# lhn0323/BEVFUSION-3D_object_detection

Hardware: AMD Instinct MI355X
Metric: nuScenes frames/sec (6-cam+LiDAR BEVFusion fwd+bwd) (higher is better)
Workload: dtype bf16; 1 GPU; full: BEVFusion camera+LiDAR (ResNet-50, LSS 6x256x704, hard voxelize 40k pts, sparse encoder, ConvFuser, SECOND/SECONDFPN, TransFusion head + Hungarian targets + focal/L1/gaussian-focal losses) fwd + bwd + clip + AdamW, bf16 autocast, fp32 index paths; global_batch=4, points_per_frame=40000, parallelism=independent frames per rank, execution=eager launches on 2 HIP queues (camera / BEV chain, LiDAR branch), view_transform_conv_dtype=bf16, head_fp32_conv=three bf16 products per multiply, fp32 accumulation (2^-16 relative per product), dense_weight_gradients=one grouped launch per tile shape at the end of the backward pass, backward_pass_thread=caller, trainable_params=37361053

## Files before the change

bevfusion-3d_object_detection_amd/_lib.py:

```python
import ctypes
import os

import torch

_HERE = os.path.dirname(os.path.abspath(__file__))
LIB_PATH = os.path.join(_HERE, "csrc", "libbevfusion_hip.so")

_c_int = ctypes.c_int
_c_vp = ctypes.c_void_p
_c_sz = ctypes.c_size_t

SIGNATURES = {
    "bfhip_abi_version": (_c_int, []),
    "bfhip_last_error": (ctypes.c_char_p, []),
    "bfhip_profile_enable": (None, [_c_int]),
    "bfhip_profile_read": (_c_int, [_c_int, _c_vp, _c_vp, _c_int]),
    "bfhip_bev_pool_fwd": (_c_int, [_c_vp] * 5 + [_c_int] * 7 + [_c_vp, _c_vp]),
    "bfhip_bev_pool_bwd": (_c_int, [_c_vp] * 5 + [_c_int] * 8 + [_c_vp, _c_vp]),
    "bfhip_dynamic_voxelize": (_c_int, [_c_vp, _c_vp, _c_int, _c_int, _c_vp, _c_vp, _c_vp]),
    "bfhip_hard_voxelize_workspace_bytes": (_c_sz, [_c_int, _c_int, _c_int]),
    "bfhip_hard_voxelize": (_c_int, [_c_vp, _c_int, _c_int, _c_vp, _c_vp, _c_vp, _c_vp, _c_vp,
                                     _c_int, _c_int, _c_vp, _c_sz, _c_vp, _c_vp]),
    "bfhip_bev_plan_workspace_bytes": (_c_sz, [ctypes.c_longlong, ctypes.c_longlong]),
    "bfhip_bev_plan": (_c_int, [_c_vp] * 7 + [_c_int] * 4 + [_c_vp] * 3 + [_c_vp] * 11 + [_c_int, _c_vp, _c_sz, _c_vp]),
    "bfhip_lift_splat_fwd": (_c_int, [_c_vp, _c_int, _c_vp, _c_int, _c_int] + [_c_vp] * 6 + [_c_int, _c_int, ctypes.c_longlong,
                                       _c_vp, _c_int, _c_vp]),
    "bfhip_lift_splat_bwd": (_c_int, [_c_vp, _c_int, _c_vp, _c_int, _c_vp, _c_int, _c_int, _c_vp] + [_c_int] * 4 +
                             [_c_vp, _c_int, _c_vp, _c_int, _c_vp]),
    "bfhip_conv_out_shape": (_c_int, [_c_vp] * 6),
    "bfhip_rulebook_subm_workspace_bytes": (_c_sz, [_c_int]),
    "bfhip_rulebook_subm": (_c_int, [_c_vp, _c_int, _c_int, _c_vp, _c_vp, _c_vp, _c_vp, _c_vp, _c_vp, _c_vp, _c_vp, _c_sz,
                                     _c_vp]),
    "bfhip_rulebook_sparse_workspace_bytes": (_c_sz, [_c_int] + [_c_vp] * 5),
    "bfhip_rulebook_sparse_count": (_c_int, [_c_vp, _c_int, _c_vp, _c_int] + [_c_vp] * 5 + [_c_vp, _c_vp, _c_sz, _c_vp]),
    "bfhip_rulebook_sparse_out_indices": (_c_int, [_c_int] + [_c_vp] * 5 + [_c_int, _c_vp, _c_vp, _c_sz, _c_vp]),
    "bfhip_rulebook_sparse_fill": (_c_int, [_c_vp, _c_int, _c_int] + [_c_vp] * 5 + [_c_int] + [_c_vp] * 4 +
                                   [_c_vp] * 4 + [_c_vp, _c_sz] + [_c_vp, _c_sz, _c_vp]),
    "bfhip_spconv_workspace_bytes": (_c_sz, [_c_int] * 3),
    "bfhip_rulebook_sort_rows_workspace_bytes": (_c_sz, [_c_int, _c_int]),
    "bfhip_rulebook_sort_rows": (_c_int, [_c_vp, _c_int, _c_int, _c_int, _c_vp, _c_vp, _c_vp, _c_sz, _c_vp]),
    "bfhip_rulebook_validate_workspace_bytes": (_c_sz, [_c_int]),
    "bfhip_rulebook_validate": (_c_int, [_c_vp, _c_int, _c_int, _c_int, _c_int, _c_vp, _c_vp, _c_vp, _c_vp, _c_sz, _c_vp]),
    "bfhip_spconv_gemm": (_c_int, [_c_vp] * 3 + [_c_int] * 7 + [_c_vp, _c_vp, _c_vp, _c_vp, _c_sz, _c_vp]),
    "bfhip_spconv_gemm_bf16": (_c_int, [_c_vp] * 3 + [_c_int] * 7 + [_c_vp, _c_vp, _c_vp, _c_int, _c_vp, _c_sz, _c_vp]),
    "bfhip_spconv_wgrad_workspace_bytes": (_c_sz, [_c_int] * 4),
    "bfhip_spconv_wgrad": (_c_int, [_c_vp] * 3 + [_c_int] * 5 + [_c_vp, _c_vp, _c_int, _c_vp, _c_sz, _c_vp]),
    "bfhip_sparse_to_bev": (_c_int, [_c_vp, _c_vp] + [_c_int] * 6 + [_c_vp, _c_vp]),
    "bfhip_bev_to_sparse": (_c_int, [_c_vp, _c_vp] + [_c_int] * 6 + [_c_vp, _c_vp]),
    "bfhip_dynamic_scatter_workspace_bytes": (_c_sz, [_c_int]),
    "bfhip_dynamic_scatter_fwd": (_c_int, [_c_vp, _c_vp, _c_int, _c_int, _c_int] + [_c_vp] * 5 + [_c_vp, _c_sz, _c_vp]),
    "bfhip_dynamic_scatter_bwd_workspace_bytes": (_c_sz, [_c_int, _c_int]),
    "bfhip_dynamic_scatter_bwd": (_c_int, [_c_vp] * 6 + [_c_int] * 4 + [_c_vp, _c_sz, _c_vp]),
    "bfhip_voxel_mean": (_c_int, [_c_vp, _c_vp, _c_int, _c_int, _c_int, _c_vp, _c_vp]),
    "bfhip_voxel_compact_mean": (_c_int, [_c_vp] * 4 + [_c_int] * 5 + [_c_vp] * 4),
    "bfhip_depth_lift_bwd_workspace_bytes": (_c_sz, []),
    "bfhip_depth_lift_bwd": (_c_int, [_c_vp, _c_vp, ctypes.c_longlong, _c_vp, _c_vp, _c_sz, _c_vp]),
    "bfhip_rasterise_depth_workspace_bytes": (_c_sz, [_c_int] * 3),
    "bfhip_rasterise_depth": (_c_int, [_c_vp, _c_int, _c_int] + [_c_vp] * 4 + [_c_int] * 3 + [_c_vp, _c_vp] + [_c_int] * 3 +
                              [_c_vp, _c_vp, _c_sz, _c_vp]),
    "bfhip_depth_histogram": (_c_int, [_c_vp] + [_c_int] * 6 + [_c_vp, _c_vp, _c_vp, _c_vp]),
    "bfhip_bn1d_workspace_bytes": (_c_sz, [_c_int, _c_int]),
    "bfhip_bn1d_fwd": (_c_int, [_c_vp] * 4 + [_c_int, _c_int, ctypes.c_float, ctypes.c_float, _c_int] + [_c_vp] * 5 +
                       [_c_vp, _c_sz, _c_vp]),
    "bfhip_bn1d_bwd": (_c_int, [_c_vp] * 5 + [_c_int] * 3 + [_c_vp] * 4 + [_c_vp, _c_sz, _c_vp]),
    "bfhip_sparse_to_bev_nhwc": (_c_int, [_c_vp, _c_vp] + [_c_int] * 7 + [_c_vp, _c_vp]),
    "bfhip_bev_nhwc_to_sparse": (_c_int, [_c_vp, ctypes.c_longlong, ctypes.c_longlong, ctypes.c_longlong, _c_int, _c_vp, _c_int,
                                          _c_int, _c_int, _c_vp, _c_vp]),
    "bfhip_bn2d_supported": (_c_int, [ctypes.c_longlong, _c_int, _c_int]),
    "bfhip_bn2d_workspace_bytes": (_c_sz, [ctypes.c_longlong, _c_int, _c_int]),
    "bfhip_colsum": (_c_int, [_c_vp, ctypes.c_longlong, _c_int, _c_int, _c_vp, _c_vp, _c_sz, _c_vp]),
    "bfhip_bn2d_fwd": (_c_int, [_c_vp] * 4 + [ctypes.c_longlong, _c_int, _c_int, ctypes.c_float, ctypes.c_float, _c_int] +
                       [_c_vp] * 5 + [_c_vp, _c_sz, _c_vp]),
    "bfhip_bn2d_bwd": (_c_int, [_c_vp] * 5 + [ctypes.c_longlong, _c_int, _c_int, _c_int] + [_c_vp] * 4 + [_c_vp, _c_sz, _c_vp]),
    "bfhip_xty_workspace_bytes": (_c_sz, [ctypes.c_longlong, _c_int, _c_int]),
    "bfhip_xty": (_c_int, [_c_vp, _c_vp, ctypes.c_longlong, _c_int, _c_int, _c_int, _c_vp, _c_vp, _c_sz, _c_vp]),
    "bfhip_attn_max_queries": (_c_int, []),
    "bfhip_attn_workspace_bytes": (_c_sz, [_c_int] * 4),
    "bfhip_attn_fwd": (_c_int, [_c_vp] * 3 + [_c_int] * 4 + [ctypes.c_float, ctypes.c_float, ctypes.c_ulonglong, _c_vp, _c_vp,
                                                             _c_vp, _c_vp, _c_sz, _c_vp]),
    "bfhip_attn_bwd": (_c_int, [_c_vp] * 6 + [_c_int] * 4 + [ctypes.c_float, ctypes.c_float, ctypes.c_ulonglong] + [_c_vp] * 4 +
                       [_c_vp, _c_sz, _c_vp]),
    "bfhip_attn_dropout_mask": (_c_int, [_c_int] * 4 + [ctypes.c_float, ctypes.c_ulonglong, _c_vp, _c_vp, _c_vp]),
    "bfhip_upsample2x_nhwc": (_c_int, [_c_vp, _c_vp] + [_c_int] * 6 + [_c_vp]),
    "bfhip_maxpool3x3s2_fwd": (_c_int, [_c_vp] + [_c_int] * 4 + [_c_vp, _c_vp, _c_vp]),
    "bfhip_maxpool3x3s2_bwd": (_c_int, [_c_vp, _c_vp] + [_c_int] * 4 + [_c_vp, _c_vp]),
    "bfhip_circle_nms": (_c_int, [_c_vp, _c_int, ctypes.c_float, _c_int, _c_vp, _c_vp, _c_vp]),
    "bfhip_rotate_nms_workspace_bytes": (_c_sz, [_c_int, _c_int]),
    "bfhip_rotate_nms": (_c_int, [_c_vp, _c_vp, _c_int, ctypes.c_float, _c_int, _c_int, _c_vp, _c_vp, _c_vp, _c_sz, _c_vp]),
    "bfhip_decode_boxes": (_c_int, [_c_vp] * 5 + [_c_int] * 4 + [_c_vp, _c_vp, _c_vp]),
    "bfhip_predict_compact": (_c_int, [_c_vp] * 3 + [_c_int] * 3 + [_c_vp, _c_int, ctypes.c_float] + [_c_vp] * 5),
    "bfhip_assign_cost": (_c_int, [_c_vp, _c_int, _c_vp, _c_int, _c_int, _c_int, _c_vp, _c_int, _c_vp, _c_vp] + [_c_int] * 3 +
                          [_c_vp] * 4),
    "bfhip_hungarian": (_c_int, [_c_vp, _c_vp, _c_int, _c_int, _c_int, _c_vp, _c_vp, _c_vp]),
    "bfhip_assign_targets": (_c_int, [_c_vp, _c_vp, _c_vp, _c_int, _c_vp] + [_c_int] * 5 + [_c_vp] * 7),
    "bfhip_draw_heatmap": (_c_int, [_c_vp, _c_int, _c_vp, _c_vp] + [_c_int] * 5 + [_c_vp, ctypes.c_double, _c_int, _c_vp, _c_vp]),
    "bfhip_gaussian_focal_loss_workspace_bytes": (_c_sz, [ctypes.c_longlong]),
    "bfhip_gaussian_focal_loss": (_c_int, [_c_vp, _c_vp, ctypes.c_longlong, ctypes.c_float, _c_vp, _c_vp, _c_vp, _c_sz, _c_vp]),
    "bfhip_conv2d_supported": (_c_int, [_c_int] * 10),
    "bfhip_conv2d_stat_rows": (_c_int, [_c_int] * 3),
    "bfhip_conv2d_fwd": (_c_int, [_c_vp, _c_int, _c_vp, _c_vp, _c_vp, _c_int] + [_c_int] * 11 + [_c_vp, _c_vp]),
    "bfhip_conv2d_dgrad_workspace_bytes": (_c_sz, [_c_int] * 4),
    "bfhip_conv2d_dgrad": (_c_int, [_c_vp, _c_int, _c_vp, _c_vp, _c_int] + [_c_int] * 11 + [_c_vp, _c_sz, _c_vp]),
    "bfhip_conv2d_dgrad_wt": (_c_int, [_c_vp, _c_int, _c_vp, _c_vp, _c_int, _c_vp, _c_int] + [_c_int] * 11 + [_c_vp]),
    "bfhip_conv2d_dgrad_fuses_addend": (_c_int, [_c_int] * 5),
    "bfhip_split_bf16x3": (_c_int, [_c_vp, ctypes.c_longlong, _c_int, _c_vp, _c_int, _c_vp, _c_int, _c_vp]),
    "bfhip_conv2d_wt_segment_bytes": (_c_int, []),
    "bfhip_conv2d_weight_transpose_batched": (_c_int, [_c_vp, _c_int, ctypes.c_longlong, _c_vp]),
    "bfhip_conv2d_launch_choice": (_c_int, [_c_int] * 12 + [_c_vp]),
    "bfhip_conv2d_wgrad_choice": (_c_int, [_c_int] * 10 + [_c_vp]),
    "bfhip_conv2d_wgrad_workspace_bytes": (_c_sz, [_c_int] * 7),
    "bfhip_conv2d_wgrad": (_c_int, [_c_vp, _c_int, _c_vp, _c_int, _c_vp] + [_c_int] * 11 + [_c_vp, _c_sz, _c_vp]),
    "bfhip_conv2d_wgrad_group_table_bytes": (_c_sz, [_c_int]),
    "bfhip_conv2d_wgrad_groupable": (_c_int, [_c_int] * 10),
    "bfhip_conv2d_wgrad_group_plan": (_c_int, [_c_vp, _c_int, _c_int, _c_vp, _c_sz, _c_vp]),
    "bfhip_conv2d_wgrad_group_launch": (_c_int, [_c_vp, _c_vp, _c_vp, _c_sz, _c_vp]),
    "bfhip_bn2d_fwd_partials": (_c_int, [_c_vp] * 4 + [ctypes.c_longlong, _c_int, _c_int, ctypes.c_float, ctypes.c_float, _c_int] +
                                [_c_vp] * 4 + [_c_vp, _c_int, _c_vp, _c_vp]),
    "bfhip_bn2d_fwd_partials_mask": (_c_int, [_c_vp] * 4 + [ctypes.c_longlong, _c_int, _c_int, ctypes.c_float, ctypes.c_float, _c_int] +
                                     [_c_vp] * 4 + [_c_vp, _c_int, _c_vp, _c_vp, _c_vp]),
    "bfhip_bn2d_bwd_mask": (_c_int, [_c_vp] * 5 + [ctypes.c_longlong, _c_int, _c_int] + [_c_vp] * 4 + [_c_vp, _c_sz, _c_vp]),
    "bfhip_adamw_segment_bytes": (_c_int, []),
    "bfhip_adamw_chunk_elems": (_c_int, []),
    "bfhip_adamw_step": (_c_int, [_c_vp, _c_vp, _c_vp, _c_int, _c_vp, _c_vp] + [ctypes.c_float] * 6 + [_c_vp]),
    "bfhip_adamw_step_groups": (_c_int, [_c_vp, _c_vp, _c_vp, _c_int, _c_vp, _c_vp, _c_vp, _c_vp, _c_int, ctypes.c_float, _c_vp]),
    "bfhip_query_losses": (_c_int, [_c_vp] * 7 + [_c_int] * 6 + [ctypes.c_float, ctypes.c_float] + [_c_vp] * 4),
    "bfhip_swin_attn_supported": (_c_int, [_c_int] * 7),
    "bfhip_swin_attn_parts": (_c_int, [_c_int] * 4),
    "bfhip_swin_attn_fwd": (_c_int, [_c_vp, ctypes.c_longlong, _c_vp] + [_c_int] * 5 + [ctypes.c_float, _c_vp, _c_vp, _c_vp]),
    "bfhip_swin_attn_bwd": (_c_int, [_c_vp, ctypes.c_longlong, _c_vp, _c_vp, _c_vp, _c_vp] + [_c_int] * 5 +
                            [ctypes.c_float, _c_vp, _c_vp, _c_int, _c_vp]),
    "bfhip_layernorm_supported": (_c_int, [ctypes.c_longlong, _c_int, _c_int, _c_int]),
    "bfhip_layernorm_parts": (_c_int, [ctypes.c_longlong, _c_int]),
    "bfhip_layernorm_fwd": (_c_int, [_c_vp, _c_vp, _c_vp, ctypes.c_longlong, _c_vp, _c_vp, ctypes.c_longlong, _c_int, ctypes.c_float] +
                            [_c_int] * 3 + [_c_vp] * 4),
    "bfhip_layernorm_bwd": (_c_int, [_c_vp] * 6 + [ctypes.c_longlong, ctypes.c_longlong] + [_c_int] * 4 + [_c_vp] * 3 + [_c_int] +
                            [_c_vp] * 3),
    "bfhip_bn_eval_supported": (_c_int, [ctypes.c_longlong, _c_int, _c_int]),
    "bfhip_bn_eval_parts": (_c_int, [ctypes.c_longlong, _c_int, _c_int]),
    "bfhip_bn_eval_fwd": (_c_int, [_c_vp] * 6 + [ctypes.c_longlong, _c_int, _c_int, ctypes.c_float, _c_int, _c_vp, _c_vp]),
    "bfhip_bn_eval_bwd": (_c_int, [_c_vp] * 6 + [ctypes.c_longlong, _c_int, _c_int, ctypes.c_float, _c_int] + [_c_vp] * 5),
    "bfhip_bn_eval_rows_fwd": (_c_int, [_c_vp] * 6 + [ctypes.c_longlong, _c_int, _c_int, ctypes.c_float, _c_int, _c_vp, _c_vp,
                                         _c_vp]),
    "bfhip_bn_eval_rows_bwd": (_c_int, [_c_vp] * 6 + [ctypes.c_longlong, _c_int, _c_int, ctypes.c_float, _c_int] + [_c_vp] * 6),
    "bfhip_img_preprocess_max_samples": (_c_int, []),
    "bfhip_img_preprocess": (_c_int, [_c_vp] + [_c_int] * 5 + [_c_vp, _c_vp, ctypes.c_float, _c_int, _c_int, _c_int, _c_int,
                                      _c_vp, _c_vp]),
    "bfhip_image_aug_max_taps": (_c_int, []),
    "bfhip_image_aug_max_cams": (_c_int, []),
    "bfhip_image_aug_supported": (_c_int, [_c_int] * 8),
    "bfhip_image_aug": (_c_int, [_c_vp, _c_int, _c_int, _c_vp, _c_vp, ctypes.c_longlong, _c_int, _c_int, _c_vp, _c_int, _c_int,
                                 _c_vp, _c_vp, ctypes.c_float] + [_c_int] * 4 + [_c_vp, _c_vp]),
    "bfhip_image_aug_masked": (_c_int, [_c_vp, _c_vp, _c_int, _c_int, _c_vp, _c_vp, ctypes.c_longlong, _c_int, _c_int, _c_vp, _c_int,
                                        _c_int, _c_vp, _c_vp, ctypes.c_float] + [_c_int] * 4 + [_c_vp, _c_vp]),
    "bfhip_points_aug_block": (_c_int, []),
    "bfhip_points_aug_workspace_bytes": (_c_sz, [ctypes.c_longlong, _c_int]),
    "bfhip_points_aug": (_c_int, [_c_vp, _c_int, _c_int, _c_vp, _c_vp, _c_vp, _c_sz, _c_vp]),
    "bfhip_points_aug_max_boxes": (_c_int, []),
    "bfhip_points_aug_paste": (_c_int, [_c_vp, _c_vp, _c_int, _c_int, _c_vp, _c_vp, _c_vp, _c_sz, _c_vp]),
    "bfhip_points_aug_max_sweeps": (_c_int, []),
    "bfhip_points_aug_sweeps": (_c_int, [_c_vp, _c_vp, _c_vp, _c_int, _c_int, _c_vp, _c_vp, _c_vp, _c_sz, _c_vp]),
    "bfhip_query_init_supported": (_c_int, [_c_int] * 8),
    "bfhip_query_init_workspace_bytes": (_c_sz, [_c_int] * 4),
    "bfhip_query_init_fwd": (_c_int, [_c_vp] + [ctypes.c_longlong] * 4 + [_c_int] * 4 + [ctypes.c_uint, _c_vp, ctypes.c_longlong,
                                      ctypes.c_longlong] + [_c_int] * 4 + [_c_vp] * 6 + [_c_sz, _c_vp]),
    "bfhip_query_init_bwd": (_c_int, [_c_vp, _c_vp, _c_int, _c_int, _c_int, ctypes.c_longlong, _c_int, _c_vp, _c_vp]),
    "bfhip_jpeg_parse": (_c_int, [_c_vp, _c_sz, _c_vp]),
    "bfhip_jpeg_entropy_decode": (_c_int, [_c_vp, _c_sz, _c_vp, _c_vp, _c_sz]),
    "bfhip_jpeg_decode": (_c_int, [_c_vp, _c_vp, _c_int, _c_vp, _c_sz, _c_vp, _c_sz, _c_vp, _c_sz, _c_vp]),
    "bfhip_jpeg_entropy_encode": (_c_int, [_c_vp, _c_vp, _c_sz, _c_int, _c_vp, _c_sz, _c_vp]),
    "bfhip_jpeg_encode_supported": (_c_int, [_c_int] * 4),
    "bfhip_jpeg_encode_workspace_bytes": (_c_sz, [_c_int] * 4),
    "bfhip_jpeg_encode_max_frames": (_c_int, []),
    "bfhip_jpeg_forward": (_c_int, [_c_vp, _c_vp, _c_int, _c_vp, _c_sz, _c_vp, _c_sz, _c_vp]),
    "bfhip_jpeg_entropy_encode_device": (_c_int, [_c_vp, _c_vp, _c_int, _c_vp, _c_sz, _c_vp, _c_sz, _c_vp, _c_sz, _c_vp, _c_vp]),
    "bfhip_jpeg_encode": (_c_int, [_c_vp, _c_vp, _c_int, _c_vp, _c_sz, _c_vp, _c_sz, _c_vp, _c_sz, _c_vp, _c_sz, _c_vp, _c_vp]),
    "bfhip_png_encode_supported": (_c_int, [_c_int] * 3),
    "bfhip_png_encode_max_frames": (_c_int, []),
    "bfhip_png_workspace_bytes": (_c_sz, [ctypes.c_int64, ctypes.c_int64, _c_int]),
    "bfhip_png_capacity": (_c_sz, [ctypes.c_int64, ctypes.c_int64]),
    "bfhip_png_result_words": (_c_sz, [ctypes.c_int64, ctypes.c_int64]),
    "bfhip_png_encode": (_c_int, [_c_vp, _c_vp, _c_int, _c_vp, _c_sz, _c_vp, _c_sz, _c_vp, _c_sz, _c_vp, _c_sz, _c_vp]),
    "bfhip_png_deflate": (_c_int, [_c_vp, _c_vp, _c_int, _c_vp, _c_sz, _c_vp, _c_sz, _c_vp, _c_sz, _c_vp, _c_sz, _c_vp]),
    "bfhip_png_filter_host": (_c_int, [_c_vp, _c_int, _c_int, _c_vp, _c_sz]),
    "bfhip_png_huffman_lengths": (_c_int, [_c_vp, _c_int, _c_int, _c_vp]),
    "bfhip_png_deflate_host": (_c_int, [_c_vp, _c_sz, _c_sz, _c_vp, _c_sz, _c_vp, _c_sz, _c_vp]),
    "bfhip_points_in_boxes_block": (_c_int, []),
    "bfhip_points_in_boxes_max_boxes": (_c_int, []),
    "bfhip_points_in_boxes_workspace_bytes": (_c_sz, [ctypes.c_longlong, _c_int]),
    "bfhip_points_in_boxes_count": (_c_int, [_c_vp, ctypes.c_longlong, _c_int, _c_vp, _c_int, _c_vp, _c_vp, _c_vp, _c_sz, _c_vp]),
    "bfhip_points_in_boxes_gather": (_c_int, [_c_vp, ctypes.c_longlong, _c_int, _c_vp, _c_int, _c_vp, _c_vp, ctypes.c_longlong,
                                              _c_vp, ctypes.c_longlong, _c_vp, _c_sz, _c_vp]),
    "bfhip_detection_eval_max_preds": (_c_int, []),
    "bfhip_detection_eval_max_gt": (_c_int, []),
    "bfhip_detection_eval_max_thresholds": (_c_int, []),
    "bfhip_detection_eval_max_classes": (_c_int, []),
    "bfhip_detection_match": (_c_int, [_c_vp] * 4 + [ctypes.c_longlong] + [_c_vp] * 3 + [ctypes.c_longlong, _c_int, _c_int, _c_vp,
                                       _c_int, _c_int, ctypes.c_uint64, ctypes.c_uint64, _c_vp, _c_vp, _c_vp]),
    "bfhip_detection_curves_workspace_bytes": (_c_sz, [ctypes.c_longlong, _c_int]),
    "bfhip_detection_curves": (_c_int, [_c_vp] * 5 + [ctypes.c_longlong, _c_int, _c_int, _c_int, _c_vp, _c_vp, ctypes.c_double,
                                        _c_int, ctypes.c_uint64] + [_c_vp] * 6 + [_c_vp, _c_sz, _c_vp]),
    "bfhip_vis_max_dim": (_c_int, []),
    "bfhip_vis_max_thickness": (_c_int, []),
    "bfhip_vis_max_scale": (_c_int, []),
    "bfhip_vis_workspace_bytes": (_c_sz, [_c_int, _c_int, _c_int]),
    "bfhip_vis_camera_segments": (_c_int, [_c_vp, _c_int, _c_vp, _c_vp, _c_int, ctypes.c_float, _c_int, _c_int, _c_int, _c_vp, _c_sz,
                                           _c_vp]),
    "bfhip_vis_bev_segments": (_c_int, [_c_vp, _c_int, ctypes.c_float, ctypes.c_float, ctypes.c_float, _c_int, _c_int, _c_int, _c_vp,
                                        _c_sz, _c_vp]),
    "bfhip_vis_composite": (_c_int, [_c_vp, _c_int, _c_int, _c_int, _c_vp, _c_sz, _c_int, _c_int, _c_vp, _c_vp, _c_int, _c_int, _c_int,
                                     _c_vp, _c_vp]),
    "bfhip_vis_bev_points": (_c_int, [_c_vp, ctypes.c_longlong, _c_int, ctypes.c_float, ctypes.c_float, ctypes.c_float, _c_int, _c_vp,
                                      _c_int, _c_int, _c_vp]),
}


class ImgDesc(ctypes.Structure):
    _fields_ = [("data", _c_vp), ("h", _c_int), ("w", _c_int)]

_lib = None


def load():
    global _lib
    if _lib is None:
        if not os.path.exists(LIB_PATH):
            raise RuntimeError(
                "libbevfusion_hip.so not found at %s: build it with "
                "`python -c 'import __graft_entry__ as g; g.build()'` (hipcc, gfx950). "
                "There is no CPU fallback." % LIB_PATH)
        lib = ctypes.CDLL(LIB_PATH)
        for name, (res, args) in SIGNATURES.items():
            fn = getattr(lib, name)
            fn.restype = res
            fn.argtypes = args
        _lib = lib
    return _lib


_torch_ext = False


def torch_ext():
    global _torch_ext
    if _torch_ext is False:
        _torch_ext = None
        path = os.path.join(_HERE, "csrc", "bfhip_torch_ext.so")
        if os.environ.get("BFHIP_TORCH_EXT", "1") == "1" and os.path.exists(path):
            import importlib.util
            load()
            try:
                spec = importlib.util.spec_from_file_location("bfhip_torch_ext", path)
                mod = importlib.util.module_from_spec(spec)
                spec.loader.exec_module(mod)
                if mod.abi_version() == load().bfhip_abi_version():
                    _torch_ext = mod
            except (ImportError, OSError) as e:
                import warnings
                warnings.warn("bfhip_torch_ext not usable (%s); using the ctypes binding" % e)
    return _torch_ext


def check(rc, what):
    if rc != 0:
        msg = load().bfhip_last_error().decode("utf-8", "replace")
        raise RuntimeError("%s failed (rc=%d): %s" % (what, rc, msg))


_fn_cache = {}


def call(name, *args):
    fn = _fn_cache.get(name)
    if fn is None:
        fn = _fn_cache[name] = getattr(load(), name)
    rc = fn(*args)
    if rc != 0:
        check(rc, name)


def call_size(name, *args):
    return int(getattr(load(), name)(*args))


def ptr(t):
    return None if t is None else t.data_ptr()


_raw_stream = getattr(torch._C, "_cuda_getCurrentRawStream", None)


def stream_of(t):
    if _raw_stream is not None:
        return _raw_stream(t.device.index if t.device.index is not None else torch.cuda.current_device())
    return ctypes.c_void_p(torch.cuda.current_stream(t.device).cuda_stream)


def host_i32(values):
    return (ctypes.c_int32 * len(values))(*[int(v) for v in values])


def host_f32(values):
    arr = (ctypes.c_float * len(values))(*[float(v) for v in values])
    return arr


def require_cuda(t, name):
    if not t.is_cuda:
        raise RuntimeError("%s must be a CUDA(HIP) tensor; this build has no CPU path" % name)
    if not t.is_contiguous():
        raise RuntimeError("%s must be contiguous" % name)


OPS = dict(bev_pool_fwd=0, bev_pool_bwd=1, hard_voxelize=2, dynamic_voxelize=3, lift_splat_fwd=4, lift_splat_bwd=5,
           spconv_fwd=6, spconv_bwd=7, rulebook=8, bev_aux=9, scatter_fwd=10, scatter_bwd=11, spconv_wgrad=12, raster=13,
           spconv_wgrad_main=14, conv2d_fwd=15, conv2d_dgrad=16, conv2d_wgrad=17, bn2d_fwd=18, bn2d_bwd=19,
           conv2d_pw_fwd=20, conv2d_pw_dgrad=21)


def profile_enable(on=True):
    load().bfhip_profile_enable(int(on))


def profile_read(op, reset=True):
    s = ctypes.c_double(0.0)
    c = ctypes.c_longlong(0)
    check(load().bfhip_profile_read(OPS[op] if isinstance(op, str) else op, ctypes.byref(s), ctypes.byref(c),
                                    1 if reset else 0), "profile_read")
    return s.value, c.value
```

bevfusion-3d_object_detection_amd/conv2d.py:

```python
import os

import torch
import torch.nn.functional as F
from torch import nn

from . import _lib

ENABLED = os.environ.get("BFHIP_CONV2D", "1") == "1"
CONV_EXT = os.environ.get("BFHIP_CONV_EXT", "1") == "1"


def _conv_ext():
    if not CONV_EXT or WGRAD_SIDE_STREAM:
        return None
    ext = _lib.torch_ext()
    if ext is None or not hasattr(ext, "conv2d"):
        return None
    ext.set_wgrad_grouped(bool(WGRAD_GROUPED))
    return ext


def _cached_wt(weight):
    cached = getattr(weight, "_bfhip_wt", None)
    if cached is not None and cached[1] == weight._version and cached[2] == weight.data_ptr():
        return cached[0]
    return None
MIN_PIXELS = int(os.environ.get("BFHIP_CONV2D_MIN_PIXELS", "2048"))
MIN_CIN = int(os.environ.get("BFHIP_CONV2D_MIN_CIN", "16"))
FORK = os.environ.get("BFHIP_CONV_FORK", "1") == "1"
_WS = {}

WGRAD_SIDE_STREAM = os.environ.get("BFHIP_WGRAD_SIDE_STREAM", "0") == "1"
_SIDE = {}
_KEEP = []


def _wgrad_stream(device):
    s = _SIDE.get(device)
    if s is None:
        s = _SIDE[device] = torch.cuda.Stream(device=device)
    return s


def wgrad_join():
    for dev, side in _SIDE.items():
        torch.cuda.current_stream(dev).wait_stream(side)
    _KEEP.clear()


WGRAD_GROUPED = os.environ.get("BFHIP_WGRAD_GROUPED", "1") == "1"
_PENDING = {}
_GROUPABLE = {}
_GROUP_STATE = {}
_LAYER_DT = None


class _WgradGroupState:

    def __init__(self, device):
        self.device = device
        self.host = [None, None]
        self.dev = None
        self.slab = None
        self.flip = 0

    def tables(self, nbytes):
        if self.dev is None or self.dev.numel() < nbytes:
            cap = max(int(nbytes) * 2, 1 << 16)
            self.host = [torch.empty(cap, dtype=torch.uint8).pin_memory() for _ in range(2)]
            self.dev = torch.empty(cap, dtype=torch.uint8, device=self.device)
        self.flip ^= 1
        return self.host[self.flip], self.dev

    def slabs(self, nbytes):
        if self.slab is None or self.slab.numel() < nbytes:
            self.slab = None
            self.slab = torch.empty(int(nbytes * 1.25) + 256, dtype=torch.uint8, device=self.device)
        return self.slab


def _layer_dtype():
    global _LAYER_DT
    if _LAYER_DT is None:
        import numpy as np
        _LAYER_DT = np.dtype([("x", "<u8"), ("dy", "<u8"), ("dw", "<u8")] + [(k, "<i4") for k in (
            "ldx", "ldg", "N", "H", "W", "Cin", "Cout", "KH", "KW", "stride", "pad", "dil", "dw_bf16", "reserved")])
        assert _LAYER_DT.itemsize == 80
    return _LAYER_DT


def _defer_wgrad(x, dy, weight, stride, pad, dil):
    N, Cin, H, W = x.shape
    Cout, _, KH, KW = weight.shape
    key = (N, H, W, Cin, Cout, KH, KW, stride, pad, dil)
    ok = _GROUPABLE.get(key)
    if ok is None:
        ok = _GROUPABLE[key] = bool(_lib.load().bfhip_conv2d_wgrad_groupable(*key))
    if (not ok or not weight.is_leaf or weight._backward_hooks or weight.dtype not in (torch.bfloat16, torch.float32)
            or torch.cuda.is_current_stream_capturing()):
        return False
    ldx, ldg = _nhwc_view(x), _nhwc_view(dy)
    if ldx is None or ldg is None:
        return False
    ext = _conv_ext()
    if ext is not None:
        return bool(ext.defer_wgrad(x, dy, weight, stride, pad, dil))
    tid = torch._C._current_graph_task_id()
    pend = _PENDING.get(tid)
    if pend is None:
        if tid < 0:
            return False
        try:
            torch.autograd.Variable._execution_engine.queue_callback(lambda: _flush_wgrads(tid))
        except RuntimeError:
            return False
        for old in [k for k in _PENDING if k < tid - 8]:
            del _PENDING[old]
        pend = _PENDING[tid] = []
    row = (x.data_ptr(), dy.data_ptr(), 0, ldx, ldg, N, H, W, Cin, Cout, KH, KW, stride, pad, dil,
           1 if weight.dtype == torch.bfloat16 else 0, 0)
    pend.append((x, dy, weight, row, _lib.stream_of(x)))
    return True


def _flush_wgrads(tid):
    import ctypes

    import numpy as np
    pend = _PENDING.pop(tid, None)
    if not pend:
        return
    by_dev = {}
    for e in pend:
        by_dev.setdefault(e[0].device, []).append(e)
    lib = _lib.load()
    with torch.no_grad():
        for dev, entries in by_dev.items():
            st = _GROUP_STATE.get(dev)
            if st is None:
                st = _GROUP_STATE[dev] = _WgradGroupState(dev)
            cur = torch.cuda.current_stream(dev)
            raw = cur.cuda_stream
            n = len(entries)
            dws = []
            for x, dy, weight, row, s in entries:
                if s != raw:
                    x.record_stream(cur)
                    dy.record_stream(cur)
                Cout, Cin, KH, KW = weight.shape
                dws.append(torch.empty((Cout, KH, KW, Cin), dtype=weight.dtype, device=dev).permute(0, 3, 1, 2))
            layers = np.array([e[3] for e in entries], dtype=_layer_dtype())
            layers["dw"] = [d.data_ptr() for d in dws]
            nbytes = int(lib.bfhip_conv2d_wgrad_group_table_bytes(n))
            host, table = st.tables(nbytes)
            slab_bytes = ctypes.c_size_t(0)
            _lib.call("bfhip_conv2d_wgrad_group_plan", layers.ctypes.data, n, 0, host.data_ptr(), nbytes, ctypes.byref(slab_bytes))
            slab = st.slabs(slab_bytes.value)
            with torch.cuda.device(dev):
                table[:nbytes].copy_(host[:nbytes], non_blocking=True)
                _lib.call("bfhip_conv2d_wgrad_group_launch", host.data_ptr(), table.data_ptr(), slab.data_ptr(), slab.numel(), raw)
            for (x, dy, weight, row, s), dw in zip(entries, dws):
                if weight.grad is None:
                    weight.grad = dw
                else:
                    weight.grad.add_(dw)


def _launch_wgrad(x, dy, weight, stride, pad, dil):
    N, Cin, H, W = x.shape
    Cout, _, KH, KW = weight.shape
    OH, OW = dy.shape[2], dy.shape[3]
    if WGRAD_GROUPED and not WGRAD_SIDE_STREAM and _defer_wgrad(x, dy, weight, stride, pad, dil):
        return None, None
    lib = _lib.load()
    out_bf16 = weight.dtype == torch.bfloat16
    side = None
    if WGRAD_SIDE_STREAM and getattr(weight, "grad", None) is None:
        main = torch.cuda.current_stream(x.device)
        side = _wgrad_stream(x.device)
        side.wait_stream(main)
        _KEEP.append((x, dy))
    with torch.cuda.stream(side) if side is not None else _NullCtx():
        stream = _lib.stream_of(x)
        dw = torch.empty((Cout, KH, KW, Cin), dtype=weight.dtype if out_bf16 else torch.float32, device=x.device).permute(0, 3, 1, 2)
        ws = _workspace(x.device, lib.bfhip_conv2d_wgrad_workspace_bytes(N, OH, OW, Cin, Cout, KH, KW), stream)
        _lib.call("bfhip_conv2d_wgrad", x.data_ptr(), _nhwc_view(x), dy.data_ptr(), _nhwc_view(dy), dw.data_ptr(), N, H, W, Cin,
                  Cout, KH, KW, stride, pad, dil, 1 if out_bf16 else 0, ws.data_ptr(), ws.numel(), stream)
        if dw.dtype != weight.dtype:
            dw = dw.to(weight.dtype)
    return dw, side


class _NullCtx:
    def __enter__(self):
        return None

    def __exit__(self, *a):
        return False


def _workspace(device, nbytes, stream):
    key = (device, stream)
    buf = _WS.get(key)
    if buf is None or buf.numel() < nbytes:
        buf = _WS[key] = torch.empty(max(int(nbytes), 1 << 24), dtype=torch.uint8, device=device)
    return buf


def _nhwc_view(t):
    N, C, H, W = t.shape
    sn, sc, sh, sw = t.stride()
    if sc == 1 and sw >= C and sh == W * sw and (sn == H * W * sw or N == 1) and sw % 8 == 0 and t.data_ptr() % 16 == 0:
        return sw
    return None


def _as_nhwc_bf16(t):
    if t.dtype != torch.bfloat16:
        t = t.to(torch.bfloat16)
    if _nhwc_view(t) is None:
        t = t.contiguous(memory_format=torch.channels_last)
        if _nhwc_view(t) is None:
            t = t.permute(0, 2, 3, 1).contiguous().permute(0, 3, 1, 2)
    return t


def _weight_ohwi(w):
    if w.dtype != torch.bfloat16:
        w = w.to(torch.bfloat16)
    p = w.permute(0, 2, 3, 1)
    return p if p.is_contiguous() else p.contiguous()


class _Conv2dFunction(torch.autograd.Function):
    @staticmethod
    def forward(ctx, x, weight, bias, stride, pad, dil, emit_stats, dgrad_lib=False, fork=False):
        ctx.set_materialize_grads(False)
        x = _as_nhwc_bf16(x)
        N, Cin, H, W = x.shape
        Cout, _, KH, KW = weight.shape
        OH = (H + 2 * pad - dil * (KH - 1) - 1) // stride + 1
        OW = (W + 2 * pad - dil * (KW - 1) - 1) // stride + 1
        w = _weight_ohwi(weight)
        y = torch.empty((N, OH, OW, Cout), dtype=torch.bfloat16, device=x.device).permute(0, 3, 1, 2)
        partial = None
        if emit_stats:
            rows = _lib.load().bfhip_conv2d_stat_rows(N, OH, OW)
            partial = torch.empty((rows, 2, Cout), dtype=torch.float32, device=x.device)
        b32 = None
        if bias is not None:
            b32 = bias if bias.dtype == torch.float32 else bias.float()
        _lib.call("bfhip_conv2d_fwd", x.data_ptr(), _nhwc_view(x), w.data_ptr(), _lib.ptr(b32), y.data_ptr(), Cout, N, H, W, Cin,
                  Cout, KH, KW, stride, pad, dil, 0, _lib.ptr(partial), _lib.stream_of(x))
        ctx.save_for_backward(x, weight)
        ctx.geom = (stride, pad, dil)
        ctx.dgrad_lib = dgrad_lib
        ctx.bias_dtype = bias.dtype if bias is not None else None
        if partial is not None:
            ctx.mark_non_differentiable(partial)
        ctx.fork = int(fork)
        if fork == 2:
            return y, partial, x[:, :, ::2, ::2].contiguous(memory_format=torch.channels_last)
        if fork:
            return y, partial, x.view_as(x)
        return y, partial

    @staticmethod
    def backward(ctx, dy, _dpartial, d_alias=None):
        x, weight = ctx.saved_tensors
        if dy is None:
            if d_alias is not None and ctx.fork == 2:
                full = torch.zeros_like(x)
                full[:, :, ::2, ::2] = d_alias
                d_alias = full
            return d_alias, None, None, None, None, None, None, None, None
        stride, pad, dil = ctx.geom
        N, Cin, H, W = x.shape
        Cout, _, KH, KW = weight.shape
        dy = _as_nhwc_bf16(dy)
        OH, OW = dy.shape[2], dy.shape[3]
        stream = _lib.stream_of(x)
        lib = _lib.load()
        dx = dw = db = None
        if ctx.needs_input_grad[0]:
            if ctx.dgrad_lib:
                dx = _add_grad(_lib_dgrad(dy, x, weight, stride, pad, dil), d_alias, ctx.fork)
            else:
                dx = _hip_dgrad(dy, x, weight, stride, pad, dil, d_alias, 2 if ctx.fork == 2 else 1)
        side = None
        if ctx.needs_input_grad[1]:
            dw, side = _launch_wgrad(x, dy, weight, stride, pad, dil)
        if ctx.bias_dtype is not None and ctx.needs_input_grad[2]:
            if side is not None:
                with torch.cuda.stream(side):
                    db = _bias_grad(dy).to(ctx.bias_dtype)
            else:
                db = _bias_grad(dy).to(ctx.bias_dtype)
        return dx, dw, db, None, None, None, None, None, None


def _add_grad(dx, addend, fork):
    if addend is None:
        return dx
    if fork == 2:
        dx[:, :, ::2, ::2] += addend
        return dx
    return dx + addend


def _bias_grad(dy):
    N, C, H, W = dy.shape
    if _nhwc_view(dy) == C:
        from .bn2d import colsum
        return colsum(dy.permute(0, 2, 3, 1).reshape(N * H * W, C))
    return dy.sum(dim=(0, 2, 3), dtype=torch.float32)


def _hip_dgrad(dy, x, weight, stride, pad, dil, addend=None, addend_stride=1):
    N, Cin, H, W = x.shape
    Cout, _, KH, KW = weight.shape
    stream = _lib.stream_of(x)
    dx = torch.empty((N, H, W, Cin), dtype=torch.bfloat16, device=x.device).permute(0, 3, 1, 2)
    cached = getattr(weight, "_bfhip_wt", None)
    if cached is not None and cached[1] == weight._version and cached[2] == weight.data_ptr():
        want = (N, Cin, (H + 1) // 2, (W + 1) // 2) if addend_stride == 2 else (N, Cin, H, W)
        fuse = (addend is not None and addend.dtype == torch.bfloat16 and tuple(addend.shape) == want
                and addend.is_contiguous(memory_format=torch.channels_last) and addend.data_ptr() % 16 == 0
                and _lib.load().bfhip_conv2d_dgrad_fuses_addend(KH, KW, stride, pad, 0))
        _lib.call("bfhip_conv2d_dgrad_wt", dy.data_ptr(), _nhwc_view(dy), cached[0].data_ptr(), _lib.ptr(addend) if fuse else None,
                  addend_stride, dx.data_ptr(), Cin, N, H, W, Cin, Cout, KH, KW, stride, pad, dil, 0, stream)
        return dx if fuse else _add_grad(dx, addend, addend_stride)
    ws = _workspace(x.device, _lib.load().bfhip_conv2d_dgrad_workspace_bytes(Cin, Cout, KH, KW), stream)
    _lib.call("bfhip_conv2d_dgrad", dy.data_ptr(), _nhwc_view(dy), _weight_ohwi(weight).data_ptr(), dx.data_ptr(), Cin, N, H,
              W, Cin, Cout, KH, KW, stride, pad, dil, 0, ws.data_ptr(), ws.numel(), stream)
    return _add_grad(dx, addend, addend_stride)


def _lib_dgrad(dy, x, weight, stride, pad, dil):
    w = weight if weight.dtype == torch.bfloat16 else weight.to(torch.bfloat16)
    return torch.ops.aten.convolution_backward(dy, x, w, None, [stride] * 2, [pad] * 2, [dil] * 2, False, [0, 0], 1,
                                               [True, False, False])[0]


class _FixedOrderBiasGrad(torch.autograd.Function):

    @staticmethod
    def forward(ctx, y, bias):
        ctx.bias_dtype = bias.dtype
        ctx.mark_dirty(y)
        return y

    @staticmethod
    def backward(ctx, dy):
        db = dy.sum(dim=(0, 2, 3), dtype=torch.float32).to(ctx.bias_dtype) if ctx.needs_input_grad[1] else None
        return dy, db


class _LibConvHipWgradFunction(torch.autograd.Function):

    @staticmethod
    def forward(ctx, x, weight, stride, pad, dil, dgrad_hip=False):
        x = _as_nhwc_bf16(x)
        w = weight if weight.dtype == torch.bfloat16 else weight.to(torch.bfloat16)
        with torch.autocast("cuda", enabled=False):
            y = F.conv2d(x, w, None, stride, pad, dil)
        ctx.save_for_backward(x, weight)
        ctx.geom = (stride, pad, dil)
        ctx.dgrad_hip = dgrad_hip
        return y

    @staticmethod
    def backward(ctx, dy):
        x, weight = ctx.saved_tensors
        stride, pad, dil = ctx.geom
        N, Cin, H, W = x.shape
        Cout, _, KH, KW = weight.shape
        dy = _as_nhwc_bf16(dy)
        OH, OW = dy.shape[2], dy.shape[3]
        dx = dw = None
        if ctx.needs_input_grad[0]:
            dx = _hip_dgrad(dy, x, weight, stride, pad, dil) if ctx.dgrad_hip else _lib_dgrad(dy, x, weight, stride, pad, dil)
        if ctx.needs_input_grad[1]:
            dw, _ = _launch_wgrad(x, dy, weight, stride, pad, dil)
        return dx, dw, None, None, None, None


FP32_SPLIT = os.environ.get("BFHIP_FP32_CONV", "split") == "split"
_SPLIT_SCOPE = [0]


class fp32_island:

    def __init__(self, mixed):
        self.mixed = bool(mixed)

    def __enter__(self):
        _SPLIT_SCOPE[0] += self.mixed
        return self

    def __exit__(self, *a):
        _SPLIT_SCOPE[0] -= self.mixed
        return False


def _split3(t_nhwc, P, C, chan_order=None, batch_order=None):
    chan = torch.empty((P, 3 * C), dtype=torch.bfloat16, device=t_nhwc.device) if chan_order is not None else None
    batch = torch.empty((3, P, C), dtype=torch.bfloat16, device=t_nhwc.device) if batch_order is not None else None
    _lib.call("bfhip_split_bf16x3", t_nhwc.data_ptr(), P, C, _lib.ptr(chan), chan_order or 0, _lib.ptr(batch), batch_order or 0,
              _lib.stream_of(t_nhwc))
    return chan, batch


_HHL, _HLH = 0b100, 0b010


class _Conv2dSplitFunction(torch.autograd.Function):

    @staticmethod
    def forward(ctx, x, weight, bias, stride, pad, dil, emit_stats):
        ctx.set_materialize_grads(False)
        N, Cin, H, W = x.shape
        Cout, _, KH, KW = weight.shape
        OH = (H + 2 * pad - dil * (KH - 1) - 1) // stride + 1
        OW = (W + 2 * pad - dil * (KW - 1) - 1) // stride + 1
        xn = x.permute(0, 2, 3, 1)
        if not xn.is_contiguous():
            xn = xn.contiguous()
        need_w = ctx.needs_input_grad[1]
        x_chan, x_batch = _split3(xn, N * H * W, Cin, _HHL, _HLH if need_w else None)
        wn = weight.detach().permute(0, 2, 3, 1).contiguous().view(Cout * KH * KW, Cin)
        w_chan, _ = _split3(wn, Cout * KH * KW, Cin, _HLH)
        y = torch.empty((N, OH, OW, Cout), dtype=torch.float32, device=x.device).permute(0, 3, 1, 2)
        partial = None
        if emit_stats:
            partial = torch.empty((_lib.load().bfhip_conv2d_stat_rows(N, OH, OW), 2, Cout), dtype=torch.float32, device=x.device)
        b32 = None if bias is None else (bias if bias.dtype == torch.float32 else bias.float())
        _lib.call("bfhip_conv2d_fwd", x_chan.data_ptr(), 3 * Cin, w_chan.data_ptr(), _lib.ptr(b32), y.data_ptr(), Cout, N, H, W, 3 * Cin,
                  Cout, KH, KW, stride, pad, dil, 1, _lib.ptr(partial), _lib.stream_of(x))
        ctx.save_for_backward(x_batch, weight)
        ctx.geom = (stride, pad, dil, N, Cin, H, W)
        ctx.has_bias = bias is not None
        if partial is not None:
            ctx.mark_non_differentiable(partial)
        return y, partial

    @staticmethod
    def backward(ctx, dy, _dpartial):
        x_batch, weight = ctx.saved_tensors
        if dy is None:
            return None, None, None, None, None, None, None
        stride, pad, dil, N, Cin, H, W = ctx.geom
        Cout, _, KH, KW = weight.shape
        OH, OW = dy.shape[2], dy.shape[3]
        lib = _lib.load()
        gn = dy.float().permute(0, 2, 3, 1)
        if not gn.is_contiguous():
            gn = gn.contiguous()
        stream = _lib.stream_of(gn)
        need_x, need_w = ctx.needs_input_grad[0], ctx.needs_input_grad[1]
        g_chan, g_batch = _split3(gn, N * OH * OW, Cout, _HHL if need_x else None, 0b100 if need_w else None)
        dx = dw = db = None
        if need_x:
            wn = weight.detach().permute(0, 2, 3, 1).contiguous().view(Cout * KH * KW, Cin)
            _, w_stack = _split3(wn, Cout * KH * KW, Cin, None, _HLH)
            dx = torch.empty((N, H, W, Cin), dtype=torch.float32, device=gn.device).permute(0, 3, 1, 2)
            ws = _workspace(gn.device, lib.bfhip_conv2d_dgrad_workspace_bytes(Cin, 3 * Cout, KH, KW), stream)
            _lib.call("bfhip_conv2d_dgrad", g_chan.data_ptr(), 3 * Cout, w_stack.data_ptr(), dx.data_ptr(), Cin, N, H, W, Cin, 3 * Cout,
                      KH, KW, stride, pad, dil, 1, ws.data_ptr(), ws.numel(), stream)
        if need_w:
            dw = torch.empty((Cout, KH, KW, Cin), dtype=torch.float32, device=gn.device).permute(0, 3, 1, 2)
            ws = _workspace(gn.device, lib.bfhip_conv2d_wgrad_workspace_bytes(3 * N, OH, OW, Cin, Cout, KH, KW), stream)
            _lib.call("bfhip_conv2d_wgrad", x_batch.data_ptr(), Cin, g_batch.data_ptr(), Cout, dw.data_ptr(), 3 * N, H, W, Cin, Cout, KH,
                      KW, stride, pad, dil, 0, ws.data_ptr(), ws.numel(), stream)
            if dw.dtype != weight.dtype:
                dw = dw.to(weight.dtype)
        if ctx.has_bias and ctx.needs_input_grad[2]:
            db = gn.sum(dim=(0, 1, 2))
        return dx, dw, db, None, None, None, None


class TransposedWeights:

    def __init__(self, modules):
        import numpy as np
        self.items = []
        recs = []
        blk = 0
        seg_bytes = _lib.load().bfhip_conv2d_wt_segment_bytes()
        assert seg_bytes == 40, seg_bytes
        for m in modules:
            if not isinstance(m, Conv2d) or m.groups != 1 or not m.weight.is_cuda:
                continue
            if isinstance(m, Conv2dHipWgrad) and m.dgrad != "hip" and not m.cache_wt:
                continue
            w = m.weight
            if w.dtype not in (torch.bfloat16, torch.float32) or not w.permute(0, 2, 3, 1).is_contiguous():
                continue
            Cout, Cin, KH, KW = w.shape
            wt = torch.empty(Cin * KH * KW * Cout, dtype=torch.bfloat16, device=w.device)
            self.items.append((w, wt))
            recs.append((w.data_ptr(), wt.data_ptr(), Cout, KH * KW, Cin, 1 if w.dtype == torch.float32 else 0, blk))
            blk += -(-Cin // 32) * -(-Cout // 32) * KH * KW
        self.blocks = blk
        self.table = None
        if recs:
            dt = np.dtype([("src", "<u8"), ("dst", "<u8"), ("Cout", "<i4"), ("taps", "<i4"), ("Cin", "<i4"), ("f32", "<i4"), ("blk0", "<i8")])
            arr = np.array(recs, dtype=dt)
            self.table = torch.from_numpy(arr.view(np.uint8).copy()).to(self.items[0][0].device)
            self._ptrs = [r[0] for r in recs]
        self.refresh()

    def refresh(self):
        if self.table is None:
            return
        if any(w.data_ptr() != p for (w, _), p in zip(self.items, self._ptrs)):
            for w, _ in self.items:
                w._bfhip_wt = None
            self.table = None
            return
        _lib.call("bfhip_conv2d_weight_transpose_batched", self.table.data_ptr(), len(self.items), self.blocks,
                  _lib.stream_of(self.table))
        for w, wt in self.items:
            w._bfhip_wt = (wt, w._version, w.data_ptr())


def _one(v):
    if isinstance(v, (tuple, list)):
        return v[0] if all(a == v[0] for a in v) else None
    return v


def conv2d(x, weight, bias=None, stride=1, padding=0, dilation=1, emit_stats=False, dgrad_lib=False, fork=False):
    ext = _conv_ext() if x.is_cuda and x.dim() == 4 and not weight._backward_hooks else None
    if ext is not None:
        out = ext.conv2d(x, weight, bias, int(stride), int(padding), int(dilation), bool(emit_stats), bool(dgrad_lib), int(fork),
                         None if dgrad_lib else _cached_wt(weight))
        partial = out[1] if emit_stats else None
        return (out[0], partial, out[2]) if fork else (out[0], partial)
    return _Conv2dFunction.apply(x, weight, bias, int(stride), int(padding), int(dilation), bool(emit_stats), bool(dgrad_lib),
                                 int(fork))


def lib_conv2d(x, weight, stride, padding, dilation, dgrad_hip=False):
    ext = _conv_ext() if x.is_cuda and x.dim() == 4 and not weight._backward_hooks else None
    if ext is not None:
        return ext.lib_conv2d(x, weight, int(stride), int(padding), int(dilation), bool(dgrad_hip),
                              _cached_wt(weight) if dgrad_hip else None)
    return _LibConvHipWgradFunction.apply(x, weight, stride, padding, dilation, dgrad_hip)


class Conv2d(nn.Conv2d):

    def _hip_domain(self, x):
        if not (ENABLED and x.is_cuda and x.dim() == 4 and self.groups == 1 and self.padding_mode == "zeros"
                and not isinstance(self.padding, str)):
            return False
        low = x.dtype == torch.bfloat16 or (torch.is_autocast_enabled("cuda") and torch.get_autocast_dtype("cuda") == torch.bfloat16
                                            and x.dtype in (torch.float32, torch.bfloat16))
        if not low or self.weight.dtype not in (torch.bfloat16, torch.float32):
            return False
        s, p, d = _one(self.stride), _one(self.padding), _one(self.dilation)
        if s is None or p is None or d is None:
            return False
        N, Cin, H, W = x.shape
        return N * H * W >= MIN_PIXELS and Cin >= MIN_CIN

    def hip_eligible(self, x):
        if not self._hip_domain(x):
            return False
        s, p, d = _one(self.stride), _one(self.padding), _one(self.dilation)
        N, Cin, H, W = x.shape
        return bool(_lib.load().bfhip_conv2d_supported(N, H, W, Cin, self.out_channels, self.kernel_size[0], self.kernel_size[1],
                                                       s, p, d))

    def split_eligible(self, x):
        if not (FP32_SPLIT and _SPLIT_SCOPE[0] > 0 and ENABLED and x.is_cuda and x.dim() == 4 and x.dtype == torch.float32 and self.weight.dtype == torch.float32
                and not torch.is_autocast_enabled("cuda") and self.groups == 1 and self.padding_mode == "zeros"
                and not isinstance(self.padding, str)):
            return False
        s, p, d = _one(self.stride), _one(self.padding), _one(self.dilation)
        if s is None or p is None or d is None:
            return False
        N, Cin, H, W = x.shape
        Cout, KH, KW = self.out_channels, self.kernel_size[0], self.kernel_size[1]
        if N * H * W < MIN_PIXELS or Cin % 8 or Cout % 8 or x.numel() * 3 >= (1 << 31):
            return False
        sup = _lib.load().bfhip_conv2d_supported
        return bool(sup(N, H, W, 3 * Cin, Cout, KH, KW, s, p, d) and sup(N, H, W, Cin, 3 * Cout, KH, KW, s, p, d)
                    and sup(3 * N, H, W, Cin, Cout, KH, KW, s, p, d))

    def forward(self, x):
        if not self.hip_eligible(x):
            if self.split_eligible(x):
                emit = self.training and self.bias is None and torch.is_grad_enabled()
                y, partial = _Conv2dSplitFunction.apply(x, self.weight, self.bias, _one(self.stride), _one(self.padding),
                                                        _one(self.dilation), emit)
                if partial is not None:
                    y._bfhip_stat_partial = (partial, y.data_ptr(), y._version)
                return y
            if self.bias is not None and self.bias.requires_grad and torch.is_grad_enabled() and self._hip_domain(x):
                return _FixedOrderBiasGrad.apply(self._conv_forward(x, self.weight, self.bias.detach()), self.bias)
            return super().forward(x)
        emit = self.training and self.bias is None and torch.is_grad_enabled()
        y, partial = conv2d(x, self.weight, self.bias, _one(self.stride), _one(self.padding), _one(self.dilation), emit)
        if partial is not None:
            y._bfhip_stat_partial = (partial, y.data_ptr(), y._version)
        return y


class Conv2dHipWgrad(Conv2d):

    fwd = "lib"
    dgrad = "lib"
    cache_wt = False

    def forward(self, x):
        if self.bias is not None or not self.training or not self.hip_eligible(x):
            return nn.Conv2d.forward(self, x)
        s, p, d = _one(self.stride), _one(self.padding), _one(self.dilation)
        if self.fwd == "hip":
            y, partial = conv2d(x, self.weight, None, s, p, d, torch.is_grad_enabled(), self.dgrad != "hip")
            if partial is not None:
                y._bfhip_stat_partial = (partial, y.data_ptr(), y._version)
            return y
        return lib_conv2d(x, self.weight, s, p, d, self.dgrad == "hip")

    def forward_fork(self, x, subsample=1):
        if (FORK and self.fwd == "hip" and self.dgrad == "hip" and self.bias is None and self.training and torch.is_grad_enabled()
                and x.requires_grad and x.dtype == torch.bfloat16 and x.dim() == 4 and _nhwc_view(x) is not None
                and self.hip_eligible(x)):
            s, p, d = _one(self.stride), _one(self.padding), _one(self.dilation)
            y, partial, alias = conv2d(x, self.weight, None, s, p, d, True, False, 2 if subsample == 2 else 1)
            y._bfhip_stat_partial = (partial, y.data_ptr(), y._version)
            return y, alias
        return self(x), (x if subsample == 1 else None)

    def forward_unstrided(self, x_sub):
        assert self.kernel_size == (1, 1) and _one(self.padding) == 0 and self.bias is None
        y, partial = conv2d(x_sub, self.weight, None, 1, 0, 1, torch.is_grad_enabled())
        if partial is not None:
            y._bfhip_stat_partial = (partial, y.data_ptr(), y._version)
        return y
```

bevfusion-3d_object_detection_amd/csrc/conv2d.hip:

```cpp
#include "conv_common.h"

namespace bfhip {
namespace {

template <bool TR>
__device__ __forceinline__ const bf16_t *piece_src(const bf16_t *x, const ConvGeom &g, bool row_ok, int nb, int hb, int wb,
                                                   unsigned info, const bf16_t *zsrc) {
  const int dh = info >> 24, dw = (info >> 16) & 0xff, ci = info & 0xffff;
  int ih, iw;
  bool ok = row_ok;
  if (!TR) {
    ih = hb + dh;
    iw = wb + dw;
  } else {
    const int th = hb - dh, tw = wb - dw;
    ok = ok && ((th | tw) >= 0) && (((th | tw) & g.smask) == 0);
    ih = th >> g.sshift;
    iw = tw >> g.sshift;
  }
  ok = ok && (unsigned)ih < (unsigned)g.H && (unsigned)iw < (unsigned)g.W;
  const unsigned off = (unsigned)(nb + ih * g.W + iw) * (unsigned)g.ldx + (unsigned)ci;
  return ok ? x + off : zsrc;
}

struct RowIdentity {
  __device__ __forceinline__ long long operator()(long long m) const { return m; }
};
struct RowParityClass {
  int Hc, Wc, H, W, h0, w0, stride;
  __device__ __forceinline__ long long operator()(long long m) const {
    const unsigned mu = (unsigned)m, hw = (unsigned)(Hc * Wc);
    const unsigned n = mu / hw, rem = mu - n * hw;
    const unsigned i = rem / (unsigned)Wc, j = rem - i * (unsigned)Wc;
    return (long long)((n * (unsigned)H + h0 + i * stride) * (unsigned)W + w0 + j * stride);
  }
};

struct Addend {
  const bf16_t *p;
  int sub, ld, H, W;
};

template <int WGM, int WGN, int MI, int NI, bool OUT_F32, typename RowMap = RowIdentity>
__device__ __forceinline__ void igemm_epilogue(f32x16 (&acc)[MI][NI], unsigned char *smem, int tm, long long m0, int n0,
                                               long long M, int Kout, int ldy, const float *__restrict__ bias,
                                               void *__restrict__ y, float *__restrict__ stat_partial,
                                               RowMap row_map = RowMap(), Addend add = Addend{nullptr, 0, 0, 0, 0}) {
  constexpr int NTHREADS = WGM * WGN * 64;
  constexpr int BN = WGN * NI * 32, BM = WGM * MI * 32;
  constexpr int PR = BM / 128;
  constexpr int G = WGM / PR;
  static_assert(BM % 128 == 0 && G * PR == WGM, "tile rows must be whole 128-row statistic groups");
  const int tid = threadIdx.x, lane = tid & 63, w = tid >> 6;
  const int wm = w / WGN, wn = w % WGN;
  const int l31 = lane & 31, lh = lane >> 5;
  __syncthreads();

  if (stat_partial) {
    float *sred = (float *)(smem);
#pragma unroll
    for (int ni = 0; ni < NI; ++ni) {
      float s = 0.f, s2 = 0.f;
#pragma unroll
      for (int mi = 0; mi < MI; ++mi)
#pragma unroll
        for (int r = 0; r < 16; ++r) { float v = acc[mi][ni][r]; s += v; s2 += v * v; }
      s += __shfl_xor(s, 32);
      s2 += __shfl_xor(s2, 32);
      if (lh == 0) {
        int col = wn * (NI * 32) + ni * 32 + l31;
        sred[(wm * BN + col) * 2 + 0] = s;
        sred[(wm * BN + col) * 2 + 1] = s2;
      }
    }
    __syncthreads();
    const int total_rows = (int)((M + 127) / 128);
    for (int e = tid; e < PR * BN; e += NTHREADS) {
      const int pr = e / BN, col = e - pr * BN;
      const int prow = tm * PR + pr;
      if (n0 + col < Kout && prow < total_rows) {
        float t0 = 0.f, t1 = 0.f;
#pragma unroll
        for (int gi = 0; gi < G; ++gi) {
          const float *q = sred + ((pr * G + gi) * BN + col) * 2;
          t0 += q[0];
          t1 += q[1];
        }
        stat_partial[((size_t)prow * 2 + 0) * Kout + n0 + col] = t0;
        stat_partial[((size_t)prow * 2 + 1) * Kout + n0 + col] = t1;
      }
    }
    __syncthreads();
  }

  constexpr int ESZ = OUT_F32 ? 4 : 2;
  constexpr int ROWB = BN * ESZ;
#pragma unroll
  for (int ni = 0; ni < NI; ++ni) {
    const int col = wn * (NI * 32) + ni * 32 + l31;
    const float bv = (bias && n0 + col < Kout) ? bias[n0 + col] : 0.f;
#pragma unroll
    for (int mi = 0; mi < MI; ++mi)
#pragma unroll
      for (int r = 0; r < 16; ++r) {
        const int row = wm * (MI * 32) + mi * 32 + (r & 3) + 8 * (r >> 2) + 4 * lh;
        const float v = acc[mi][ni][r] + bv;
        if (OUT_F32) *(float *)(smem + row * ROWB + col * 4) = v;
        else *(bf16_t *)(smem + row * ROWB + col * 2) = (bf16_t)bf16_rne(v);
      }
  }
  __syncthreads();
  constexpr int CPR = ROWB / 16;
  constexpr int EPC = 16 / ESZ;
  for (int idx = tid; idx < BM * CPR; idx += NTHREADS) {
    const int row = idx / CPR, c = idx - row * CPR;
    const long long m = m0 + row;
    const int col = n0 + c * EPC;
    if (m >= M || col >= Kout) continue;
    unsigned char *dst = (unsigned char *)y + ((size_t)row_map(m) * ldy + col) * ESZ;
    const unsigned char *src = smem + row * ROWB + c * 16;
    const bf16_t *rs = nullptr;
    if (!OUT_F32 && add.p) {
      if (add.sub == 2) {
        const unsigned mu = (unsigned)row_map(m), hw = (unsigned)(add.H * add.W);
        const unsigned n = mu / hw, rem = mu - n * hw;
        const unsigned h = rem / (unsigned)add.W, w = rem - h * (unsigned)add.W;
        if (((h | w) & 1u) == 0)
          rs = add.p + ((size_t)((n * (unsigned)((add.H + 1) >> 1) + (h >> 1)) * (unsigned)((add.W + 1) >> 1) + (w >> 1)) * add.ld + col);
      } else {
        rs = add.p + ((size_t)row_map(m) * add.ld + col);
      }
    }
    if (rs) {
      bf16_t *d16 = (bf16_t *)dst;
      const bf16_t *s16 = (const bf16_t *)src;
      if (col + EPC <= Kout && ((((uintptr_t)dst) | ((uintptr_t)rs)) & 15) == 0) {
        const uint4 a4 = *(const uint4 *)src, b4 = *(const uint4 *)rs;
        const unsigned a[4] = {a4.x, a4.y, a4.z, a4.w}, b[4] = {b4.x, b4.y, b4.z, b4.w};
        unsigned o[4];
#pragma unroll
        for (int q = 0; q < 4; ++q) {
          const float lo = __uint_as_float(a[q] << 16) + __uint_as_float(b[q] << 16);
          const float hi = __uint_as_float(a[q] & 0xffff0000u) + __uint_as_float(b[q] & 0xffff0000u);
          o[q] = bf16_rne(lo) | (bf16_rne(hi) << 16);
        }
        *(uint4 *)dst = make_uint4(o[0], o[1], o[2], o[3]);
        continue;
      }
      for (int e = 0; e < EPC && col + e < Kout; e += 2) {
        if (col + e + 1 < Kout && ((((uintptr_t)(d16 + e)) | ((uintptr_t)(rs + e))) & 3) == 0) {
          const unsigned a = *(const unsigned *)(s16 + e), b = *(const unsigned *)(rs + e);
          const float lo = __uint_as_float(a << 16) + __uint_as_float(b << 16);
          const float hi = __uint_as_float(a & 0xffff0000u) + __uint_as_float(b & 0xffff0000u);
          *(unsigned *)(d16 + e) = bf16_rne(lo) | (bf16_rne(hi) << 16);
        } else {
          for (int q = e; q < e + 2 && col + q < Kout; ++q)
            d16[q] = (bf16_t)bf16_rne(__uint_as_float((unsigned)s16[q] << 16) + __uint_as_float((unsigned)rs[q] << 16));
        }
      }
      continue;
    }
    if (col + EPC <= Kout && (((uintptr_t)dst) & 15) == 0) *(uint4 *)dst = *(const uint4 *)src;
    else
      for (int e = 0; e < EPC && col + e < Kout; ++e) {
        if (OUT_F32) ((float *)dst)[e] = ((const float *)src)[e];
        else ((bf16_t *)dst)[e] = ((const bf16_t *)src)[e];
      }
  }
}

template <int WGM, int WGN, int MI, int NI, int STAGES, bool OUT_F32, int MODE>
__global__ __launch_bounds__(WGM * WGN * 64, (STAGES == 1 ? 4 : (WGM * WGN > 4 ? 1 : 2))) void conv_igemm_kernel(
    const bf16_t *__restrict__ x, const bf16_t *__restrict__ wt, const float *__restrict__ bias, void *__restrict__ y,
    float *__restrict__ stat_partial, ConvGeom g, int tiles_m, int tiles_n) {
  constexpr bool TR = MODE != 0;
  constexpr int NWAVES = WGM * WGN, NTHREADS = NWAVES * 64;
  constexpr int BN = WGN * NI * 32, BM = WGM * MI * 32, BK = 64;
  constexpr int A_BYTES = BM * BK * 2, B_BYTES = BN * BK * 2, S_BYTES = A_BYTES + B_BYTES;
  constexpr int NA = (BM / 8) / NWAVES;
  constexpr int NB = (BN / 8) / NWAVES;
  constexpr int GL = NA + NB;
  static_assert(NA >= 1 && NA * 8 * NWAVES == BM && NB >= 1 && NB * 8 * NWAVES == BN, "tiles must split into whole DMA instructions");
  extern __shared__ __attribute__((aligned(1024))) unsigned char smem[];
  unsigned *taps = (unsigned *)(smem + STAGES * S_BYTES);
  const int tid = threadIdx.x, lane = tid & 63, w = tid >> 6;
  const long long lb = xcd_chunked_block(blockIdx.x, (long long)tiles_m * tiles_n);
  const int tn = (int)(lb % tiles_n);
  int tm = (int)(lb / tiles_n);
  long long M = g.M;
  int nq = g.nq;
  ConvGeom::ParityClass pc = {};
  if (MODE == 2) {
    int c = 0;
    while (c + 1 < g.ncls && tm >= g.cls[c + 1].tile0) ++c;
    pc = g.cls[c];
    tm -= pc.tile0;
    M = (long long)g.N * pc.Hc * pc.Wc;
    nq = pc.nkh * pc.nkw * (g.C >> 3);
  }
  const long long m0 = (long long)tm * BM;
  const int n0 = tn * BN;

  if (MODE == 2 && nq == 0) {
    constexpr int ESZ = OUT_F32 ? 4 : 2, EPC = 16 / ESZ, CPR = BN / EPC;
    const RowParityClass rm{pc.Hc, pc.Wc, g.OH, g.OW, pc.h0, pc.w0, g.stride};
    for (int idx = tid; idx < BM * CPR; idx += NTHREADS) {
      const int row = idx / CPR, c = idx - row * CPR;
      const long long m = m0 + row;
      const int col = n0 + c * EPC;
      if (m >= M || col >= g.Kout) continue;
      unsigned char *dst = (unsigned char *)y + ((size_t)rm(m) * g.ldy + col) * ESZ;
      if (col + EPC <= g.Kout && (((uintptr_t)dst) & 15) == 0) *(uint4 *)dst = make_uint4(0u, 0u, 0u, 0u);
      else
        for (int e = 0; e < EPC && col + e < g.Kout; ++e) {
          if (OUT_F32) ((float *)dst)[e] = 0.f;
          else ((bf16_t *)dst)[e] = 0;
        }
    }
    return;
  }

  for (int q = tid; q < nq; q += NTHREADS) {
    int k = q * 8;
    int tap = k / g.C, ci = k - tap * g.C;
    int kh, kw;
    if (MODE == 2) {
      const int a = tap / pc.nkw;
      kh = pc.kh0 + a * g.stride;
      kw = pc.kw0 + (tap - a * pc.nkw) * g.stride;
    } else {
      kh = tap / g.KW;
      kw = tap - kh * g.KW;
    }
    taps[q] = ((unsigned)(kh * g.dil) << 24) | ((unsigned)(kw * g.dil) << 16) | (unsigned)ci;
  }

  const int lrow = lane >> 3, lpos = lane & 7;
  int nb[NA], hb[NA], wb[NA];
  bool rok[NA];
#pragma unroll
  for (int i = 0; i < NA; ++i) {
    long long m = m0 + w * (NA * 8) + i * 8 + lrow;
    rok[i] = m < M;
    long long mm = rok[i] ? m : 0;
    int n, oh, ow;
    const unsigned mu = (unsigned)mm;
    if (MODE == 2) {
      const unsigned hw = (unsigned)(pc.Hc * pc.Wc);
      const unsigned nn = mu / hw, rem = mu - nn * hw;
      const unsigned ci_ = rem / (unsigned)pc.Wc;
      n = (int)nn;
      oh = pc.h0 + (int)ci_ * g.stride;
      ow = pc.w0 + (int)(rem - ci_ * (unsigned)pc.Wc) * g.stride;
    } else {
      const unsigned hw = (unsigned)(g.OH * g.OW);
      const unsigned nn = mu / hw, rem = mu - nn * hw;
      n = (int)nn;
      oh = (int)(rem / (unsigned)g.OW);
      ow = (int)(rem - (unsigned)oh * (unsigned)g.OW);
    }
    nb[i] = n * g.H * g.W;
    hb[i] = TR ? oh + g.pad : oh * g.stride - g.pad;
    wb[i] = TR ? ow + g.pad : ow * g.stride - g.pad;
  }
  const bf16_t *wrow[NB];
#pragma unroll
  for (int i = 0; i < NB; ++i) {
    int co = n0 + w * (NB * 8) + i * 8 + lrow;
    wrow[i] = co < g.Kout ? wt + (size_t)co * g.ldw : nullptr;
  }
  __syncthreads();

  const int nt = (nq + 7) >> 3;
  const bf16_t *zsrc = zero_src();
  auto stage = [&](int t, int buf) {
    unsigned char *dA = smem + buf * S_BYTES + (w * (NA * 8)) * 128;
    unsigned char *dB = smem + buf * S_BYTES + A_BYTES + (w * (NB * 8)) * 128;
#pragma unroll
    for (int i = 0; i < NA; ++i) {
      const int swz = ((w * (NA * 8) + i * 8 + lrow) >> 1) & 7;
      const int q = t * 8 + (lpos ^ swz);
      const bf16_t *src = q < nq ? piece_src<TR>(x, g, rok[i], nb[i], hb[i], wb[i], taps[q], zsrc) : zsrc;
      glds16(src, dA + i * 1024);
    }
#pragma unroll
    for (int i = 0; i < NB; ++i) {
      const int swz = ((w * (NB * 8) + i * 8 + lrow) >> 1) & 7;
      const int q = t * 8 + (lpos ^ swz);
      const bf16_t *src = zsrc;
      if (wrow[i] && q < nq) {
        if (MODE == 2) {
          const unsigned info = taps[q];
          src = wrow[i] + ((size_t)((info >> 24) * g.KW + ((info >> 16) & 0xff)) * g.C + (info & 0xffff));
        } else {
          src = wrow[i] + (size_t)q * 8;
        }
      }
      glds16(src, dB + i * 1024);
    }
  };

  f32x16 acc[MI][NI];
#pragma unroll
  for (int mi = 0; mi < MI; ++mi)
#pragma unroll
    for (int ni = 0; ni < NI; ++ni)
#pragma unroll
      for (int r = 0; r < 16; ++r) acc[mi][ni][r] = 0.f;

  const int wm = w / WGN, wn = w % WGN;
  const int l31 = lane & 31, lh = lane >> 5, rswz = (lane >> 1) & 7;
  const int aoff = (wm * (MI * 32) + l31) * 128, boff = A_BYTES + (wn * (NI * 32) + l31) * 128;

#pragma unroll
  for (int s0 = 0; s0 < STAGES - 1; ++s0)
    if (s0 < nt) stage(s0, s0);
  int buf = 0, nbuf = STAGES - 1;
  for (int t = 0; t < nt; ++t) {
    if (STAGES == 1) {
      if (t) __syncthreads();
      stage(t, 0);
    }
    if (STAGES <= 2 || nt - 1 - t == 0) wait_vmcnt<0>();
    else if (STAGES == 3 || nt - 1 - t == 1) wait_vmcnt<GL>();
    else wait_vmcnt<2 * GL>();
    __builtin_amdgcn_s_barrier();
    const unsigned char *pA = smem + buf * S_BYTES + aoff, *pB = smem + buf * S_BYTES + boff;
    if (STAGES > 1 && t + STAGES - 1 < nt) stage(t + STAGES - 1, nbuf);
#pragma unroll
    for (int ks = 0; ks < 4; ++ks) {
      const int pos = ((2 * ks + lh) ^ rswz) << 4;
      bf16x8 a[MI], b[NI];
#pragma unroll
      for (int mi = 0; mi < MI; ++mi) a[mi] = *(const bf16x8 *)(pA + mi * 32 * 128 + pos);
#pragma unroll
      for (int ni = 0; ni < NI; ++ni) b[ni] = *(const bf16x8 *)(pB + ni * 32 * 128 + pos);
#pragma unroll
      for (int mi = 0; mi < MI; ++mi)
#pragma unroll
        for (int ni = 0; ni < NI; ++ni) acc[mi][ni] = __builtin_amdgcn_mfma_f32_32x32x16_bf16(a[mi], b[ni], acc[mi][ni], 0, 0, 0);
    }
    buf = buf + 1 == STAGES ? 0 : buf + 1;
    nbuf = nbuf + 1 == STAGES ? 0 : nbuf + 1;
  }
  if (MODE == 2)
    igemm_epilogue<WGM, WGN, MI, NI, OUT_F32, RowParityClass>(acc, smem, tm, m0, n0, M, g.Kout, g.ldy, bias, y, stat_partial,
                                                              RowParityClass{pc.Hc, pc.Wc, g.OH, g.OW, pc.h0, pc.w0, g.stride});
  else
    igemm_epilogue<WGM, WGN, MI, NI, OUT_F32>(acc, smem, tm, m0, n0, M, g.Kout, g.ldy, bias, y, stat_partial);
}

template <int NI, bool OUT_F32, int DIR>
__global__ __launch_bounds__(256, 4) void conv_pw_kernel(const bf16_t *__restrict__ x, const bf16_t *__restrict__ wt,
                                                         const float *__restrict__ bias, void *__restrict__ y,
                                                         float *__restrict__ stat_partial, long long M, int C, int ldx, int Kout,
                                                         int ldw, int ldy, int tiles_m, int tiles_n, Addend add) {
  constexpr int WGN = 2, MI = 2;
  constexpr int BM = 128, BN = NI * 64;
  constexpr int A_BYTES = BM * 128;
  constexpr int NA = 4, NB = BN / 32;
  extern __shared__ __attribute__((aligned(1024))) unsigned char smem[];
  const int tid = threadIdx.x, lane = tid & 63, w = tid >> 6;
  const long long lb = xcd_chunked_block(blockIdx.x, (long long)tiles_m * tiles_n);
  const int tn = (int)(lb % tiles_n), tm = (int)(lb / tiles_n);
  const long long m0 = (long long)tm * BM;
  const int n0 = tn * BN;
  const int nq = C >> 3, nt = (nq + 7) >> 3;
  const int lrow = lane >> 3, lpos = lane & 7;
  const bf16_t *zsrc = zero_src();
  const bf16_t *arow[NA], *brow[NB];
#pragma unroll
  for (int i = 0; i < NA; ++i) {
    const long long m = m0 + w * 32 + i * 8 + lrow;
    arow[i] = m < M ? x + (unsigned)m * (unsigned)ldx : nullptr;
  }
#pragma unroll
  for (int i = 0; i < NB; ++i) {
    const int co = n0 + w * (NB * 8) + i * 8 + lrow;
    brow[i] = co < Kout ? wt + (size_t)co * ldw : nullptr;
  }
  f32x16 acc[MI][NI];
#pragma unroll
  for (int mi = 0; mi < MI; ++mi)
#pragma unroll
    for (int ni = 0; ni < NI; ++ni)
#pragma unroll
      for (int r = 0; r < 16; ++r) acc[mi][ni][r] = 0.f;
  const int wm = w / WGN, wn = w % WGN;
  const int l31 = lane & 31, lh = lane >> 5, rswz = (lane >> 1) & 7;
  const unsigned char *pA = smem + (wm * 64 + l31) * 128, *pB = smem + A_BYTES + (wn * (NI * 32) + l31) * 128;
  unsigned char *dA = smem + (w * 32) * 128, *dB = smem + A_BYTES + (w * (NB * 8)) * 128;
  for (int t = 0; t < nt; ++t) {
    if (t) __syncthreads();
#pragma unroll
    for (int i = 0; i < NA; ++i) {
      const int q = t * 8 + (lpos ^ (((w * 32 + i * 8 + lrow) >> 1) & 7));
      glds16(arow[i] && q < nq ? arow[i] + q * 8 : zsrc, dA + i * 1024);
    }
#pragma unroll
    for (int i = 0; i < NB; ++i) {
      const int q = t * 8 + (lpos ^ (((w * (NB * 8) + i * 8 + lrow) >> 1) & 7));
      glds16(brow[i] && q < nq ? brow[i] + q * 8 : zsrc, dB + i * 1024);
    }
    wait_vmcnt<0>();
    __builtin_amdgcn_s_barrier();
#pragma unroll
    for (int ks = 0; ks < 4; ++ks) {
      const int pos = ((2 * ks + lh) ^ rswz) << 4;
      bf16x8 a[MI], b[NI];
#pragma unroll
      for (int mi = 0; mi < MI; ++mi) a[mi] = *(const bf16x8 *)(pA + mi * 32 * 128 + pos);
#pragma unroll
      for (int ni = 0; ni < NI; ++ni) b[ni] = *(const bf16x8 *)(pB + ni * 32 * 128 + pos);
#pragma unroll
      for (int mi = 0; mi < MI; ++mi)
#pragma unroll
        for (int ni = 0; ni < NI; ++ni) acc[mi][ni] = __builtin_amdgcn_mfma_f32_32x32x16_bf16(a[mi], b[ni], acc[mi][ni], 0, 0, 0);
    }
  }
  igemm_epilogue<2, WGN, MI, NI, OUT_F32>(acc, smem, tm, m0, n0, M, Kout, ldy, bias, y, stat_partial, RowIdentity(), add);
}

__global__ __launch_bounds__(256) void conv_weight_transpose_kernel(const bf16_t *__restrict__ w, bf16_t *__restrict__ wt,
                                                                    int Cout, int taps, int Cin) {
  __shared__ bf16_t tile[32][33];
  const int tap = blockIdx.z, c0 = blockIdx.x * 32, o0 = blockIdx.y * 32;
  const int tx = threadIdx.x & 31, ty = threadIdx.x >> 5;
  for (int r = ty; r < 32; r += 8) {
    int co = o0 + r, ci = c0 + tx;
    tile[r][tx] = (co < Cout && ci < Cin) ? w[((size_t)co * taps + tap) * Cin + ci] : (bf16_t)0;
  }
  __syncthreads();
  for (int r = ty; r < 32; r += 8) {
    int ci = c0 + r, co = o0 + tx;
    if (ci < Cin && co < Cout) wt[((size_t)ci * taps + tap) * Cout + co] = tile[tx][r];
  }
}

struct WtSeg {
  const void *src;
  bf16_t *dst;
  int Cout, taps, Cin, src_f32;
  long long blk0;
};
__global__ __launch_bounds__(256) void conv_weight_transpose_batched_kernel(const WtSeg *__restrict__ segs, int nseg) {
  __shared__ bf16_t tile[32][33];
  const long long b = blockIdx.x;
  int lo = 0, hi = nseg - 1;
  while (lo < hi) {
    const int mid = (lo + hi + 1) >> 1;
    if (segs[mid].blk0 <= b) lo = mid; else hi = mid - 1;
  }
  const WtSeg sg = segs[lo];
  const int nx = (sg.Cin + 31) >> 5, ny = (sg.Cout + 31) >> 5;
  int local = (int)(b - sg.blk0);
  const int bx = local % nx; local /= nx;
  const int by = local % ny;
  const int tap = local / ny;
  if (tap >= sg.taps) return;
  const int c0 = bx * 32, o0 = by * 32;
  const int tx = threadIdx.x & 31, ty = threadIdx.x >> 5;
  for (int r = ty; r < 32; r += 8) {
    const int co = o0 + r, ci = c0 + tx;
    bf16_t v = 0;
    if (co < sg.Cout && ci < sg.Cin) {
      const size_t i = ((size_t)co * sg.taps + tap) * sg.Cin + ci;
      v = sg.src_f32 ? (bf16_t)bf16_rne(((const float *)sg.src)[i]) : ((const bf16_t *)sg.src)[i];
    }
    tile[r][tx] = v;
  }
  __syncthreads();
  for (int r = ty; r < 32; r += 8) {
    const int ci = c0 + r, co = o0 + tx;
    if (ci < sg.Cin && co < sg.Cout) sg.dst[((size_t)ci * sg.taps + tap) * sg.Cout + co] = tile[tx][r];
  }
}

__global__ __launch_bounds__(256) void split_bf16x3_kernel(const float *__restrict__ src, long long P, int C, bf16_t *__restrict__ chan,
                                                           int order_chan, bf16_t *__restrict__ batch, int order_batch) {
  const int cv = C >> 3;
  const long long t = (long long)blockIdx.x * blockDim.x + threadIdx.x;
  if (t >= P * cv) return;
  const long long p = t / cv;
  const int c = (int)(t - p * cv) << 3;
  const float4 a = *(const float4 *)(src + p * C + c), b = *(const float4 *)(src + p * C + c + 4);
  const float v[8] = {a.x, a.y, a.z, a.w, b.x, b.y, b.z, b.w};
  unsigned hi[8], lo[8];
#pragma unroll
  for (int j = 0; j < 8; ++j) {
    hi[j] = bf16_rne(v[j]);
    lo[j] = bf16_rne(v[j] - __uint_as_float(hi[j] << 16));
  }
  const uint4 H4 = make_uint4(hi[0] | (hi[1] << 16), hi[2] | (hi[3] << 16), hi[4] | (hi[5] << 16), hi[6] | (hi[7] << 16));
  const uint4 L4 = make_uint4(lo[0] | (lo[1] << 16), lo[2] | (lo[3] << 16), lo[4] | (lo[5] << 16), lo[6] | (lo[7] << 16));
#pragma unroll
  for (int k = 0; k < 3; ++k) {
    if (chan) *(uint4 *)(chan + p * (3LL * C) + (long long)k * C + c) = ((order_chan >> k) & 1) ? L4 : H4;
    if (batch) *(uint4 *)(batch + ((long long)k * P + p) * C + c) = ((order_batch >> k) & 1) ? L4 : H4;
  }
}

bool takes_pointwise(const ConvGeom &g) {
  static const int max_c = env_int("BFHIP_CONV_PW_MAXC", 4096);
  return g.KH == 1 && g.KW == 1 && g.stride == 1 && g.pad == 0 && g.transposed != 2 && g.C <= max_c;
}

struct IgemmChoice {
  bool pointwise;
  int shape, stages, BM, BN, tiles_m, tiles_n;
  size_t lds;
  int tile0[17];
};

IgemmChoice choose_igemm(const ConvGeom &g, int out_f32, int cus) {
  IgemmChoice c = {};
  if (takes_pointwise(g)) {
    c.pointwise = true;
    c.stages = 1; c.BM = 128; c.BN = g.Kout > 64 ? 128 : 64;
    c.tiles_m = ceil_div(g.M, 128);
    c.tiles_n = ceil_div(g.Kout, c.BN);
    const size_t stage = (size_t)(128 + c.BN) * 128, epi = (size_t)128 * c.BN * (out_f32 ? 4 : 2);
    c.lds = stage > epi ? stage : epi;
    return c;
  }
  static const int tile256 = env_int("BFHIP_CONV_TILE256", 1);
  static const int tile256_min = env_int("BFHIP_CONV_TILE256_MIN", 384);
  int shape = g.Kout > 64 ? 1 : 0;
  const long long t256 = (long long)ceil_div(g.M, 256) * ceil_div(g.Kout, 256);
  const bool fits256 = t256 >= tile256_min && (long long)ceil_div(g.Kout, 256) * 256 * 8 <= (long long)g.Kout * 9;
  if (tile256 && !out_f32 && g.Kout > 128 && (fits256 || tile256 == 2)) shape = 2;
  static const int quant = env_int("BFHIP_CONV_QUANT", 1);
  if (quant && shape == 1) {
    const long long t = (long long)ceil_div(g.M, 128) * ceil_div(g.Kout, 128);
    const double rounds = (double)t / (2.0 * cus);
    if (rounds > 1.0 && rounds < 4.0 && rounds - (long long)rounds < 0.15) shape = 0;
  }
  static const int small_grid = env_int("BFHIP_CONV_SMALL_GRID", 1);
  if (small_grid && shape == 1 && g.transposed != 2 && (long long)ceil_div(g.M, 128) * ceil_div(g.Kout, 128) < cus) shape = 0;
  static const int single = env_int("BFHIP_CONV_SINGLE_STAGE", 1);
  const long long tiles128 = (long long)ceil_div(g.M, 128) * ceil_div(g.Kout, shape == 0 ? 64 : 128);
  const bool one_stage = shape <= 1 && single && (single == 2 || g.transposed == 2 || tiles128 >= 3LL * cus || (g.nq + 7) / 8 <= 18);
  c.shape = shape; c.stages = one_stage ? 1 : 2;
  c.BM = shape == 2 ? 256 : 128; c.BN = shape == 2 ? 256 : (shape == 0 ? 64 : 128);
  c.tiles_m = ceil_div(g.M, c.BM);
  c.tiles_n = ceil_div(g.Kout, c.BN);
  if (g.transposed == 2) {
    c.tiles_m = 0;
    for (int k = 0; k < g.ncls; ++k) {
      c.tile0[k] = c.tiles_m;
      c.tiles_m += ceil_div((long long)g.N * g.cls[k].Hc * g.cls[k].Wc, c.BM);
    }
    c.tile0[g.ncls] = c.tiles_m;
  }
  c.lds = (size_t)c.stages * (c.BM + c.BN) * 128 + (size_t)g.nq * 4;
  if (c.stages == 1) {
    const size_t epi = (size_t)c.BM * c.BN * (out_f32 ? 4 : 2);
    if (c.lds < epi) c.lds = epi;
  }
  return c;
}

struct IgemmArgs { const bf16_t *x, *wt; const float *bias; void *y; float *stat_partial; ConvGeom g; hipStream_t s; Addend add; };

template <int NI, bool F32, int DIR>
void launch_pw(const IgemmArgs &a, const IgemmChoice &c) {
  launch_big_lds<conv_pw_kernel<NI, F32, DIR>>(64 * 1024, dim3((unsigned)((long long)c.tiles_m * c.tiles_n)), dim3(256), c.lds, a.s, a.x, a.wt,
                                               a.bias, a.y, a.stat_partial, a.g.M, a.g.C, a.g.ldx, a.g.Kout, a.g.ldw, a.g.ldy, c.tiles_m, c.tiles_n, a.add);
}
template <int NI, bool F32>
void launch_pw(const IgemmArgs &a, const IgemmChoice &c) { a.g.transposed ? launch_pw<NI, F32, 1>(a, c) : launch_pw<NI, F32, 0>(a, c); }

template <int WGM, int WGN, int MI, int NI, int ST, bool F32, int MODE>
void launch_ig(const IgemmArgs &a, const IgemmChoice &c) {
  launch_big_lds<conv_igemm_kernel<WGM, WGN, MI, NI, ST, F32, MODE>>(
      (WGM * WGN > 4) ? 159 * 1024 : 80 * 1024, dim3((unsigned)((long long)c.tiles_m * c.tiles_n)), dim3(WGM * WGN * 64), c.lds, a.s, a.x, a.wt,
      a.bias, a.y, a.stat_partial, a.g, c.tiles_m, c.tiles_n);
}
template <int WGM, int WGN, int MI, int NI, int ST, bool F32>
void launch_ig(const IgemmArgs &a, const IgemmChoice &c) {
  const int m = a.g.transposed;
  m == 2 ? launch_ig<WGM, WGN, MI, NI, ST, F32, 2>(a, c) : m ? launch_ig<WGM, WGN, MI, NI, ST, F32, 1>(a, c) : launch_ig<WGM, WGN, MI, NI, ST, F32, 0>(a, c);
}
template <int NI, int ST>
void launch_ig128(const IgemmArgs &a, const IgemmChoice &c, int f32) { f32 ? launch_ig<2, 2, 2, NI, ST, true>(a, c) : launch_ig<2, 2, 2, NI, ST, false>(a, c); }

int launch_igemm(const void *x, const void *wt, const float *bias, void *y, float *stat_partial, const ConvGeom &g, int out_f32,
                 hipStream_t s, const char *what, Addend add = Addend{nullptr, 0, 0, 0, 0}) {
  BFHIP_REQUIRE(!add.p || (takes_pointwise(g) && !out_f32),
                "%s: an addend is only fused into the pointwise kernel (1x1, stride 1, no padding, bf16 output)", what);
  const IgemmChoice c = choose_igemm(g, out_f32, device_cus());
  IgemmArgs a = {(const bf16_t *)x, (const bf16_t *)wt, bias, y, stat_partial, g, s, add};
  for (int k = 0; g.transposed == 2 && k <= g.ncls; ++k) a.g.cls[k].tile0 = c.tile0[k];
  if (c.pointwise && c.BN == 128) out_f32 ? launch_pw<2, true>(a, c) : launch_pw<2, false>(a, c);
  else if (c.pointwise) out_f32 ? launch_pw<1, true>(a, c) : launch_pw<1, false>(a, c);
  else if (c.shape == 2) launch_ig<2, 4, 4, 2, 2, false>(a, c);
  else if (c.shape == 1) c.stages == 1 ? launch_ig128<2, 1>(a, c, out_f32) : launch_ig128<2, 2>(a, c, out_f32);
  else c.stages == 1 ? launch_ig128<1, 1>(a, c, out_f32) : launch_ig128<1, 2>(a, c, out_f32);
  return check_launch(what);
}

ConvGeom dgrad_geom(int N, int H, int W, int Cin, int ldx, int Cout, int ldg, int KH, int KW, int stride, int pad, int dil) {
  static const int parity = env_int("BFHIP_CONV_DGRAD_PARITY", 1);
  return conv_geom_dgrad(N, H, W, Cin, ldx, Cout, ldg, KH, KW, stride, pad, dil, parity != 0);
}

}
}

using namespace bfhip;

BFHIP_EXPORT int bfhip_conv2d_supported(int N, int H, int W, int Cin, int Cout, int KH, int KW, int stride, int pad, int dil) {
  return geom_ok(N, H, W, Cin, KH, KW, stride, pad, dil) && geom_ok(N, H, W, Cout, KH, KW, stride, pad, dil) ? 1 : 0;
}

BFHIP_EXPORT int bfhip_conv2d_stat_rows(int N, int OH, int OW) { return ceil_div((long long)N * OH * OW, 128); }

BFHIP_EXPORT int bfhip_conv2d_fwd(const void *x, int ldx, const void *w, const float *bias, void *y, int ldy, int N, int H, int W,
                                  int Cin, int Cout, int KH, int KW, int stride, int pad, int dil, int out_f32,
                                  float *stat_partial, void *stream_) {
  BFHIP_REQUIRE(bfhip_conv2d_supported(N, H, W, Cin, Cout, KH, KW, stride, pad, dil), "conv2d_fwd: unsupported geometry");
  BFHIP_REQUIRE(x && w && y, "conv2d_fwd: null pointer");
  BFHIP_REQUIRE(dma_operand_ok(x, ldx, Cin) && ((uintptr_t)w % 16) == 0 && ldy >= Cout, kOperandMsg, "conv2d_fwd");
  const ConvGeom g = conv_geom_fwd(N, H, W, Cin, ldx, Cout, KH, KW, stride, pad, dil, ldy);
  BFHIP_REQUIRE(g.OH > 0 && g.OW > 0, "conv2d_fwd: empty output");
  BFHIP_REQUIRE((long long)N * H * W * ldx < (1LL << 31), "conv2d_fwd: tensors of 2^31 elements or more are not supported");
  ProfScope ps;
  prof_begin(takes_pointwise(g) ? BFHIP_OP_CONV2D_PW_FWD : BFHIP_OP_CONV2D_FWD, (hipStream_t)stream_, &ps);
  const int rc = launch_igemm(x, w, bias, y, stat_partial, g, out_f32, (hipStream_t)stream_, "conv2d_fwd");
  prof_end(&ps);
  return rc;
}

BFHIP_EXPORT int bfhip_conv2d_launch_choice(int dir, int N, int H, int W, int Cin, int Cout, int KH, int KW, int stride, int pad,
                                            int dil, int out_f32, int32_t *out_host) {
  BFHIP_REQUIRE(out_host && (dir == 0 || dir == 1), "conv2d_launch_choice: bad arguments");
  BFHIP_REQUIRE(bfhip_conv2d_supported(N, H, W, Cin, Cout, KH, KW, stride, pad, dil), "conv2d_launch_choice: unsupported geometry");
  const ConvGeom g = dir ? dgrad_geom(N, H, W, Cin, Cin, Cout, Cout, KH, KW, stride, pad, dil)
                         : conv_geom_fwd(N, H, W, Cin, Cin, Cout, KH, KW, stride, pad, dil, Cout);
  BFHIP_REQUIRE((dir ? g.H > 0 && g.W > 0 : g.OH > 0 && g.OW > 0), "conv2d_launch_choice: empty output");
  const IgemmChoice c = choose_igemm(g, out_f32, device_cus());
  const int32_t v[8] = {c.pointwise ? 1 : 0, c.pointwise ? c.BN : c.shape, c.stages, g.transposed, c.BM, c.BN, c.tiles_m, c.tiles_n};
  for (int i = 0; i < 8; ++i) out_host[i] = v[i];
  return BFHIP_OK;
}

BFHIP_EXPORT size_t bfhip_conv2d_dgrad_workspace_bytes(int Cin, int Cout, int KH, int KW) {
  return align_up((size_t)Cin * KH * KW * Cout * 2, 256);
}

static int conv2d_dgrad_impl(const void *dy, int ldg, const void *w, void *dx, int ldx, int N, int H, int W, int Cin, int Cout,
                             int KH, int KW, int stride, int pad, int dil, int out_f32, void *workspace, size_t workspace_bytes,
                             hipStream_t s, const void *addend = nullptr, int addend_stride = 1) {
  BFHIP_REQUIRE(bfhip_conv2d_supported(N, H, W, Cin, Cout, KH, KW, stride, pad, dil), "conv2d_dgrad: unsupported geometry");
  BFHIP_REQUIRE(dy && dx && workspace, "conv2d_dgrad: null pointer");
  BFHIP_REQUIRE(workspace_bytes >= bfhip_conv2d_dgrad_workspace_bytes(Cin, Cout, KH, KW), "conv2d_dgrad: workspace too small");
  BFHIP_REQUIRE(dma_operand_ok(dy, ldg, Cout) && ((uintptr_t)workspace % 16) == 0 && ldx >= Cin, kOperandMsg, "conv2d_dgrad");
  const ConvGeom g = dgrad_geom(N, H, W, Cin, ldx, Cout, ldg, KH, KW, stride, pad, dil);
  BFHIP_REQUIRE((long long)N * g.H * g.W * ldg < (1LL << 31), "conv2d_dgrad: tensors of 2^31 elements or more are not supported");
  BFHIP_REQUIRE(((uintptr_t)addend % 4) == 0 && (addend_stride == 1 || addend_stride == 2), "conv2d_dgrad: bad addend");
  ProfScope ps;
  prof_begin(takes_pointwise(g) ? BFHIP_OP_CONV2D_PW_DGRAD : BFHIP_OP_CONV2D_DGRAD, s, &ps);
  if (w)
    hipLaunchKernelGGL(conv_weight_transpose_kernel, dim3(ceil_div(Cin, 32), ceil_div(Cout, 32), KH * KW), dim3(256), 0, s,
                       (const bf16_t *)w, (bf16_t *)workspace, Cout, KH * KW, Cin);
  const int rc = launch_igemm(dy, workspace, nullptr, dx, nullptr, g, out_f32, s, "conv2d_dgrad",
                              Addend{(const bf16_t *)addend, addend ? addend_stride : 0, Cin, H, W});
  prof_end(&ps);
  return rc;
}

BFHIP_EXPORT int bfhip_conv2d_dgrad(const void *dy, int ldg, const void *w, void *dx, int ldx, int N, int H, int W, int Cin,
                                    int Cout, int KH, int KW, int stride, int pad, int dil, int out_f32, void *workspace,
                                    size_t workspace_bytes, void *stream_) {
  BFHIP_REQUIRE(w, "conv2d_dgrad: null pointer");
  return conv2d_dgrad_impl(dy, ldg, w, dx, ldx, N, H, W, Cin, Cout, KH, KW, stride, pad, dil, out_f32, workspace, workspace_bytes,
                           (hipStream_t)stream_);
}

BFHIP_EXPORT int bfhip_conv2d_dgrad_wt(const void *dy, int ldg, const void *wt, const void *addend, int addend_stride, void *dx,
                                       int ldx, int N, int H, int W, int Cin, int Cout, int KH, int KW, int stride, int pad, int dil,
                                       int out_f32, void *stream_) {
  return conv2d_dgrad_impl(dy, ldg, nullptr, dx, ldx, N, H, W, Cin, Cout, KH, KW, stride, pad, dil, out_f32, (void *)wt,
                           bfhip_conv2d_dgrad_workspace_bytes(Cin, Cout, KH, KW), (hipStream_t)stream_, addend, addend_stride);
}

BFHIP_EXPORT int bfhip_conv2d_dgrad_fuses_addend(int KH, int KW, int stride, int pad, int out_f32) {
  return KH == 1 && KW == 1 && stride == 1 && pad == 0 && !out_f32 ? 1 : 0;
}

BFHIP_EXPORT int bfhip_split_bf16x3(const float *src, long long P, int C, void *chan, int order_chan, void *batch, int order_batch,
                                    void *stream_) {
  BFHIP_REQUIRE(src && (chan || batch) && P > 0 && C > 0 && C % 8 == 0, "split_bf16x3: bad arguments");
  BFHIP_REQUIRE(((uintptr_t)src % 16) == 0 && ((uintptr_t)chan % 16) == 0 && ((uintptr_t)batch % 16) == 0, "split_bf16x3: misaligned tensor");
  const long long total = P * (C / 8);
  BFHIP_REQUIRE(total < (1LL << 31) * 256, "split_bf16x3: tensor too large");
  hipLaunchKernelGGL(split_bf16x3_kernel, dim3((unsigned)ceil_div(total, 256)), dim3(256), 0, (hipStream_t)stream_, src, P, C,
                     (bf16_t *)chan, order_chan, (bf16_t *)batch, order_batch);
  return check_launch("split_bf16x3");
}

BFHIP_EXPORT int bfhip_conv2d_wt_segment_bytes(void) { return (int)sizeof(WtSeg); }

BFHIP_EXPORT int bfhip_conv2d_weight_transpose_batched(const void *segs_dev, int nseg, long long total_blocks, void *stream_) {
  BFHIP_REQUIRE(segs_dev && nseg > 0 && total_blocks > 0 && total_blocks < (1LL << 31), "conv2d_weight_transpose_batched: bad table");
  hipLaunchKernelGGL(conv_weight_transpose_batched_kernel, dim3((unsigned)total_blocks), dim3(256), 0, (hipStream_t)stream_,
                     (const WtSeg *)segs_dev, nseg);
  return check_launch("conv2d_weight_transpose_batched");
}
```

bevfusion-3d_object_detection_amd/csrc/torch_binding.cpp:

```cpp
#include <torch/extension.h>
#include <torch/csrc/autograd/engine.h>
#include <torch/csrc/autograd/graph_task.h>
#include <c10/hip/HIPStream.h>
#include <c10/hip/HIPGuard.h>
#include <ATen/hip/impl/HIPStreamMasqueradingAsCUDA.h>
#include <hip/hip_runtime_api.h>

#include <map>
#include <mutex>
#include <vector>

#include "../../include/bevfusion_hip.h"

namespace {

using torch::Tensor;
using torch::autograd::AutogradContext;
using torch::autograd::tensor_list;

inline void *cur_stream(const Tensor &t) { return (void *)c10::hip::getCurrentHIPStream(t.get_device()).stream(); }
inline int dt_code(const Tensor &t) { return t.scalar_type() == at::kBFloat16 ? 1 : 0; }
inline void check(int rc, const char *what) {
  TORCH_CHECK(rc == 0, what, " failed (rc=", rc, "): ", bfhip_last_error());
}

class BN2dFn : public torch::autograd::Function<BN2dFn> {
 public:
  static Tensor forward(AutogradContext *ctx, const Tensor &x, const c10::optional<Tensor> &residual, const Tensor &weight,
                        const Tensor &bias, const Tensor &running_mean, const Tensor &running_var, double eps,
                        double momentum, bool relu, const c10::optional<Tensor> &partial, bool relu_bits) {
    const int64_t C = x.size(1), M = x.numel() / C;
    const int dt = dt_code(x);
    Tensor res;
    if (residual.has_value() && residual->defined()) {
      res = residual->scalar_type() == x.scalar_type() ? *residual : residual->to(x.scalar_type());
      res = res.contiguous(at::MemoryFormat::ChannelsLast);
    }
    Tensor y = at::empty_like(x);
    Tensor stats = at::empty({4 * C}, x.options().dtype(at::kFloat));
    Tensor mask;
    if (partial.has_value() && partial->defined()) {
      const Tensor &pt = *partial;
      if (relu_bits && relu && res.defined() && dt == 1 && C % 8 == 0) {
        mask = at::empty({M, C / 8}, x.options().dtype(at::kByte));
        check(bfhip_bn2d_fwd_partials_mask(x.data_ptr(), res.data_ptr(), weight.data_ptr<float>(), bias.data_ptr<float>(), M, (int)C, dt,
                                           (float)eps, (float)momentum, 1, running_mean.data_ptr<float>(),
                                           running_var.data_ptr<float>(), stats.data_ptr<float>(), y.data_ptr(),
                                           pt.data_ptr<float>(), (int)pt.size(0), nullptr, mask.data_ptr<uint8_t>(), cur_stream(x)),
              "bn2d_fwd_partials_mask");
      } else {
        check(bfhip_bn2d_fwd_partials(x.data_ptr(), res.defined() ? res.data_ptr() : nullptr, weight.data_ptr<float>(),
                                      bias.data_ptr<float>(), M, (int)C, dt, (float)eps, (float)momentum, relu ? 1 : 0,
                                      running_mean.data_ptr<float>(), running_var.data_ptr<float>(), stats.data_ptr<float>(),
                                      y.data_ptr(), pt.data_ptr<float>(), (int)pt.size(0), nullptr, cur_stream(x)),
              "bn2d_fwd_partials");
      }
    } else {
      const size_t wsb = bfhip_bn2d_workspace_bytes(M, (int)C, dt);
      Tensor ws = at::empty({(int64_t)wsb}, x.options().dtype(at::kByte));
      check(bfhip_bn2d_fwd(x.data_ptr(), res.defined() ? res.data_ptr() : nullptr, weight.data_ptr<float>(),
                           bias.data_ptr<float>(), M, (int)C, dt, (float)eps, (float)momentum, relu ? 1 : 0,
                           running_mean.data_ptr<float>(), running_var.data_ptr<float>(), stats.data_ptr<float>(), y.data_ptr(),
                           nullptr, ws.data_ptr(), wsb, cur_stream(x)),
            "bn2d_fwd");
    }
    const bool keep_y = relu && res.defined() && !mask.defined();
    ctx->save_for_backward({x, keep_y ? y : Tensor(), stats, weight, mask});
    ctx->saved_data["relu"] = relu;
    ctx->saved_data["has_res"] = res.defined();
    if (res.defined()) ctx->saved_data["res_dtype"] = (int64_t)residual->scalar_type();
    return y;
  }

  static tensor_list backward(AutogradContext *ctx, tensor_list grads) {
    auto saved = ctx->get_saved_variables();
    const Tensor &x = saved[0], &y = saved[1], &stats = saved[2], &weight = saved[3], &mask = saved[4];
    const bool relu = ctx->saved_data["relu"].toBool(), has_res = ctx->saved_data["has_res"].toBool();
    const int64_t C = x.size(1), M = x.numel() / C;
    const int dt = dt_code(x);
    Tensor dy = grads[0];
    if (dy.scalar_type() != x.scalar_type()) dy = dy.to(x.scalar_type());
    dy = dy.contiguous(at::MemoryFormat::ChannelsLast);
    Tensor dx = at::empty_like(x);
    Tensor dres = has_res ? at::empty_like(x) : Tensor();
    Tensor dgb = at::empty({2 * C}, x.options().dtype(at::kFloat));
    const size_t wsb = bfhip_bn2d_workspace_bytes(M, (int)C, dt);
    Tensor ws = at::empty({(int64_t)wsb}, x.options().dtype(at::kByte));
    if (mask.defined())
      check(bfhip_bn2d_bwd_mask(dy.data_ptr(), x.data_ptr(), mask.data_ptr<uint8_t>(), stats.data_ptr<float>(),
                                weight.data_ptr<float>(), M, (int)C, dt, dx.data_ptr(), dres.defined() ? dres.data_ptr() : nullptr,
                                dgb.data_ptr<float>(), nullptr, ws.data_ptr(), wsb, cur_stream(x)),
            "bn2d_bwd_mask");
    else
      check(bfhip_bn2d_bwd(dy.data_ptr(), x.data_ptr(), y.defined() ? y.data_ptr() : nullptr, stats.data_ptr<float>(),
                           weight.data_ptr<float>(), M, (int)C, dt, relu ? 1 : 0, dx.data_ptr(),
                           dres.defined() ? dres.data_ptr() : nullptr, dgb.data_ptr<float>(), nullptr, ws.data_ptr(), wsb, cur_stream(x)),
            "bn2d_bwd");
    if (has_res) {
      auto rdt = (at::ScalarType)ctx->saved_data["res_dtype"].toInt();
      if (rdt != dres.scalar_type()) dres = dres.to(rdt);
    }
    return {dx, dres, dgb.slice(0, 0, C), dgb.slice(0, C, 2 * C), Tensor(), Tensor(), Tensor(), Tensor(), Tensor(), Tensor(), Tensor()};
  }
};

Tensor bn2d(const Tensor &x, const c10::optional<Tensor> &residual, const Tensor &weight, const Tensor &bias,
            const Tensor &running_mean, const Tensor &running_var, double eps, double momentum, bool relu,
            const c10::optional<Tensor> &partial, bool relu_bits) {
  return BN2dFn::apply(x, residual, weight, bias, running_mean, running_var, eps, momentum, relu, partial, relu_bits);
}

class BN1dFn : public torch::autograd::Function<BN1dFn> {
 public:
  static Tensor forward(AutogradContext *ctx, const Tensor &x_, const c10::optional<Tensor> &residual, const Tensor &weight,
                        const Tensor &bias, const Tensor &running_mean, const Tensor &running_var, double eps,
                        double momentum, bool relu) {
    Tensor x = x_.contiguous();
    const int64_t N = x.size(0), C = x.size(1);
    Tensor res;
    if (residual.has_value() && residual->defined()) res = residual->contiguous();
    Tensor y = at::empty_like(x);
    Tensor stats = at::empty({2 * C}, x.options());
    const size_t wsb = bfhip_bn1d_workspace_bytes((int)N, (int)C);
    Tensor ws = at::empty({(int64_t)wsb}, x.options().dtype(at::kByte));
    check(bfhip_bn1d_fwd(x.data_ptr<float>(), res.defined() ? res.data_ptr<float>() : nullptr, weight.data_ptr<float>(),
                         bias.data_ptr<float>(), (int)N, (int)C, (float)eps, (float)momentum, relu ? 1 : 0,
                         running_mean.data_ptr<float>(), running_var.data_ptr<float>(), stats.data_ptr<float>(),
                         y.data_ptr<float>(), nullptr, ws.data_ptr(), wsb, cur_stream(x)),
          "bn1d_fwd");
    ctx->save_for_backward({x, y, stats, weight});
    ctx->saved_data["relu"] = relu;
    ctx->saved_data["has_res"] = res.defined();
    return y;
  }

  static tensor_list backward(AutogradContext *ctx, tensor_list grads) {
    auto saved = ctx->get_saved_variables();
    const Tensor &x = saved[0], &y = saved[1], &stats = saved[2], &weight = saved[3];
    const bool relu = ctx->saved_data["relu"].toBool(), has_res = ctx->saved_data["has_res"].toBool();
    const int64_t N = x.size(0), C = x.size(1);
    Tensor dy = grads[0].contiguous();
    Tensor dx = at::empty_like(x);
    Tensor dres = has_res ? at::empty_like(x) : Tensor();
    Tensor dgb = at::empty({2 * C}, x.options());
    const size_t wsb = bfhip_bn1d_workspace_bytes((int)N, (int)C);
    Tensor ws = at::empty({(int64_t)wsb}, x.options().dtype(at::kByte));
    check(bfhip_bn1d_bwd(dy.data_ptr<float>(), y.data_ptr<float>(), x.data_ptr<float>(), stats.data_ptr<float>(),
                         weight.data_ptr<float>(), (int)N, (int)C, relu ? 1 : 0, dx.data_ptr<float>(),
                         dres.defined() ? dres.data_ptr<float>() : nullptr, dgb.data_ptr<float>(), nullptr, ws.data_ptr(), wsb,
                         cur_stream(x)),
          "bn1d_bwd");
    return {dx, dres, dgb.slice(0, 0, C), dgb.slice(0, C, 2 * C), Tensor(), Tensor(), Tensor(), Tensor(), Tensor()};
  }
};

Tensor bn1d(const Tensor &x, const c10::optional<Tensor> &residual, const Tensor &weight, const Tensor &bias,
            const Tensor &running_mean, const Tensor &running_var, double eps, double momentum, bool relu) {
  return BN1dFn::apply(x, residual, weight, bias, running_mean, running_var, eps, momentum, relu);
}



inline int64_t nhwc_pitch(const Tensor &t) {
  const auto sz = t.sizes();
  const auto st = t.strides();
  const int64_t N = sz[0], C = sz[1], H = sz[2], W = sz[3], sn = st[0], sc = st[1], sh = st[2], sw = st[3];
  if (sc == 1 && sw >= C && sh == W * sw && (sn == H * W * sw || N == 1) && sw % 8 == 0 && ((uintptr_t)t.data_ptr()) % 16 == 0) return sw;
  return 0;
}

inline Tensor as_nhwc_bf16(Tensor t) {
  if (t.scalar_type() != at::kBFloat16) t = t.to(at::kBFloat16);
  if (!nhwc_pitch(t)) {
    t = t.contiguous(at::MemoryFormat::ChannelsLast);
    if (!nhwc_pitch(t)) t = t.permute({0, 2, 3, 1}).contiguous().permute({0, 3, 1, 2});
  }
  return t;
}

inline Tensor weight_ohwi(const Tensor &w_) {
  Tensor w = w_.scalar_type() == at::kBFloat16 ? w_ : w_.to(at::kBFloat16);
  Tensor p = w.permute({0, 2, 3, 1});
  return p.is_contiguous() ? p : p.contiguous();
}

inline Tensor empty_nhwc(int64_t N, int64_t C, int64_t H, int64_t W, const at::TensorOptions &opt) {
  return at::empty({N, H, W, C}, opt).permute({0, 3, 1, 2});
}

struct PendingWgrad {
  Tensor x, dy, weight;
  bfhip_wgrad_layer row;
  void *stream;
};
struct GroupState {
  Tensor host[2], dev, slab;
  int flip = 0;
};
std::mutex g_mu;
std::map<int, std::vector<PendingWgrad>> &g_pending = *new std::map<int, std::vector<PendingWgrad>>();
std::map<int, GroupState> &g_group = *new std::map<int, GroupState>();
bool g_grouped = true;

void flush_wgrads(int tid) {
  std::vector<PendingWgrad> pend;
  {
    std::lock_guard<std::mutex> lock(g_mu);
    auto it = g_pending.find(tid);
    if (it == g_pending.end()) return;
    pend = std::move(it->second);
    g_pending.erase(it);
  }
  if (pend.empty()) return;
  static std::mutex flush_mu;
  std::lock_guard<std::mutex> one_at_a_time(flush_mu);
  at::NoGradGuard no_grad;
  std::map<int, std::vector<size_t>> by_dev;
  for (size_t i = 0; i < pend.size(); ++i) by_dev[pend[i].x.get_device()].push_back(i);
  for (auto &kv : by_dev) {
    const int dev = kv.first;
    const auto &idx = kv.second;
    const int n = (int)idx.size();
    c10::hip::HIPGuard guard((c10::DeviceIndex)dev);
    auto cur = c10::hip::getCurrentHIPStreamMasqueradingAsCUDA((c10::DeviceIndex)dev);
    void *raw = (void *)cur.stream();
    GroupState &st = g_group[dev];
    std::vector<bfhip_wgrad_layer> rows((size_t)n);
    std::vector<Tensor> dws((size_t)n);
    for (int k = 0; k < n; ++k) {
      PendingWgrad &e = pend[idx[k]];
      if (e.stream != raw) {
        e.x.record_stream(cur);
        e.dy.record_stream(cur);
      }
      const auto ws = e.weight.sizes();
      dws[k] = empty_nhwc(ws[0], ws[1], ws[2], ws[3], e.weight.options());
      rows[k] = e.row;
      rows[k].dw = dws[k].data_ptr();
    }
    const size_t nbytes = bfhip_conv2d_wgrad_group_table_bytes(n);
    if (!st.dev.defined() || (size_t)st.dev.numel() < nbytes) {
      const int64_t cap = std::max<int64_t>((int64_t)nbytes * 2, 1 << 16);
      for (auto &h : st.host) h = at::empty({cap}, at::TensorOptions().dtype(at::kByte).pinned_memory(true));
      st.dev = at::empty({cap}, at::TensorOptions().dtype(at::kByte).device(at::kCUDA, dev));
    }
    st.flip ^= 1;
    Tensor &host = st.host[st.flip];
    size_t slab_bytes = 0;
    check(bfhip_conv2d_wgrad_group_plan(rows.data(), n, 0, host.data_ptr(), nbytes, &slab_bytes), "conv2d_wgrad_group_plan");
    if (!st.slab.defined() || (size_t)st.slab.numel() < slab_bytes) {
      st.slab = Tensor();
      st.slab = at::empty({(int64_t)(slab_bytes + slab_bytes / 4) + 256}, at::TensorOptions().dtype(at::kByte).device(at::kCUDA, dev));
    }
    st.dev.narrow(0, 0, (int64_t)nbytes).copy_(host.narrow(0, 0, (int64_t)nbytes), true);
    check(bfhip_conv2d_wgrad_group_launch(host.data_ptr(), st.dev.data_ptr(), st.slab.data_ptr(), (size_t)st.slab.numel(), raw),
          "conv2d_wgrad_group_launch");
    for (int k = 0; k < n; ++k) {
      Tensor &w = pend[idx[k]].weight;
      if (!w.grad().defined()) w.mutable_grad() = dws[k];
      else w.mutable_grad().add_(dws[k]);
    }
  }
}

bool defer_wgrad(const Tensor &x, const Tensor &dy, const Tensor &weight, int64_t stride, int64_t pad, int64_t dil) {
  if (!g_grouped) return false;
  const int64_t N = x.size(0), Cin = x.size(1), H = x.size(2), W = x.size(3);
  const int64_t Cout = weight.size(0), KH = weight.size(2), KW = weight.size(3);
  if (!weight.is_leaf() || !weight.requires_grad()) return false;
  if (weight.scalar_type() != at::kBFloat16 && weight.scalar_type() != at::kFloat) return false;
  if (!bfhip_conv2d_wgrad_groupable((int)N, (int)H, (int)W, (int)Cin, (int)Cout, (int)KH, (int)KW, (int)stride, (int)pad, (int)dil)) return false;
  const int64_t ldx = nhwc_pitch(x), ldg = nhwc_pitch(dy);
  if (!ldx || !ldg) return false;
  void *stream = cur_stream(x);
  hipStreamCaptureStatus cap = hipStreamCaptureStatusNone;
  if (hipStreamIsCapturing((hipStream_t)stream, &cap) != hipSuccess) { (void)hipGetLastError(); return false; }
  if (cap != hipStreamCaptureStatusNone) return false;
  const int tid = torch::autograd::get_current_graph_task_id();
  if (tid < 0) return false;
  const auto *plan = torch::autograd::get_current_graph_task_exec_info();
  if (plan && !plan->empty()) return false;
  PendingWgrad e;
  e.x = x; e.dy = dy; e.weight = weight; e.stream = stream;
  e.row = bfhip_wgrad_layer{x.data_ptr(), dy.data_ptr(), nullptr, (int32_t)ldx, (int32_t)ldg, (int32_t)N, (int32_t)H, (int32_t)W,
                            (int32_t)Cin, (int32_t)Cout, (int32_t)KH, (int32_t)KW, (int32_t)stride, (int32_t)pad, (int32_t)dil,
                            weight.scalar_type() == at::kBFloat16 ? 1 : 0, 0};
  std::lock_guard<std::mutex> lock(g_mu);
  auto it = g_pending.find(tid);
  if (it == g_pending.end()) {
    torch::autograd::Engine::get_default_engine().queue_callback([tid]() { flush_wgrads(tid); });
    for (auto old = g_pending.begin(); old != g_pending.end();) old = old->first < tid - 8 ? g_pending.erase(old) : std::next(old);
    it = g_pending.emplace(tid, std::vector<PendingWgrad>()).first;
  }
  it->second.push_back(std::move(e));
  return true;
}

int64_t pending_wgrads() {
  std::lock_guard<std::mutex> lock(g_mu);
  int64_t n = 0;
  for (auto &kv : g_pending) n += (int64_t)kv.second.size();
  return n;
}

Tensor launch_wgrad(const Tensor &x, const Tensor &dy, const Tensor &weight, int64_t stride, int64_t pad, int64_t dil) {
  if (defer_wgrad(x, dy, weight, stride, pad, dil)) return Tensor();
  const int64_t N = x.size(0), Cin = x.size(1), H = x.size(2), W = x.size(3);
  const int64_t Cout = weight.size(0), KH = weight.size(2), KW = weight.size(3), OH = dy.size(2), OW = dy.size(3);
  const bool out_bf16 = weight.scalar_type() == at::kBFloat16;
  Tensor dw = empty_nhwc(Cout, Cin, KH, KW, x.options().dtype(out_bf16 ? at::kBFloat16 : at::kFloat));
  const size_t wsb = bfhip_conv2d_wgrad_workspace_bytes((int)N, (int)OH, (int)OW, (int)Cin, (int)Cout, (int)KH, (int)KW);
  Tensor ws = at::empty({(int64_t)std::max<size_t>(wsb, 256)}, x.options().dtype(at::kByte));
  check(bfhip_conv2d_wgrad(x.data_ptr(), (int)nhwc_pitch(x), dy.data_ptr(), (int)nhwc_pitch(dy), dw.data_ptr(), (int)N, (int)H, (int)W,
                           (int)Cin, (int)Cout, (int)KH, (int)KW, (int)stride, (int)pad, (int)dil, out_bf16 ? 1 : 0, ws.data_ptr(),
                           (size_t)ws.numel(), cur_stream(x)),
        "conv2d_wgrad");
  return dw.scalar_type() == weight.scalar_type() ? dw : dw.to(weight.scalar_type());
}

inline Tensor add_grad(Tensor dx, const Tensor &addend, int fork) {
  if (!addend.defined()) return dx;
  if (fork == 2) {
    using torch::indexing::Slice;
    dx.index({Slice(), Slice(), Slice(0, c10::nullopt, 2), Slice(0, c10::nullopt, 2)}).add_(addend);
    return dx;
  }
  return dx + addend;
}

Tensor hip_dgrad(const Tensor &dy, const Tensor &x, const Tensor &weight, const Tensor &wt, int64_t stride, int64_t pad, int64_t dil,
                 const Tensor &addend, int addend_stride) {
  const int64_t N = x.size(0), Cin = x.size(1), H = x.size(2), W = x.size(3);
  const int64_t Cout = weight.size(0), KH = weight.size(2), KW = weight.size(3);
  Tensor dx = empty_nhwc(N, Cin, H, W, x.options().dtype(at::kBFloat16));
  if (wt.defined()) {
    bool fuse = false;
    if (addend.defined() && addend.scalar_type() == at::kBFloat16 && addend.dim() == 4 && addend.size(0) == N && addend.size(1) == Cin &&
        addend.size(2) == (addend_stride == 2 ? (H + 1) / 2 : H) && addend.size(3) == (addend_stride == 2 ? (W + 1) / 2 : W) &&
        addend.is_contiguous(at::MemoryFormat::ChannelsLast) && ((uintptr_t)addend.data_ptr()) % 16 == 0)
      fuse = bfhip_conv2d_dgrad_fuses_addend((int)KH, (int)KW, (int)stride, (int)pad, 0) != 0;
    check(bfhip_conv2d_dgrad_wt(dy.data_ptr(), (int)nhwc_pitch(dy), wt.data_ptr(), fuse ? addend.data_ptr() : nullptr, addend_stride,
                                dx.data_ptr(), (int)Cin, (int)N, (int)H, (int)W, (int)Cin, (int)Cout, (int)KH, (int)KW, (int)stride,
                                (int)pad, (int)dil, 0, cur_stream(x)),
          "conv2d_dgrad_wt");
    return fuse ? dx : add_grad(dx, addend, addend_stride);
  }
  const size_t wsb = bfhip_conv2d_dgrad_workspace_bytes((int)Cin, (int)Cout, (int)KH, (int)KW);
  Tensor ws = at::empty({(int64_t)std::max<size_t>(wsb, 256)}, x.options().dtype(at::kByte));
  Tensor w = weight_ohwi(weight);
  check(bfhip_conv2d_dgrad(dy.data_ptr(), (int)nhwc_pitch(dy), w.data_ptr(), dx.data_ptr(), (int)Cin, (int)N, (int)H, (int)W, (int)Cin,
                           (int)Cout, (int)KH, (int)KW, (int)stride, (int)pad, (int)dil, 0, ws.data_ptr(), (size_t)ws.numel(), cur_stream(x)),
        "conv2d_dgrad");
  return add_grad(dx, addend, addend_stride);
}

inline Tensor lib_dgrad(const Tensor &dy, const Tensor &x, const Tensor &weight, int64_t stride, int64_t pad, int64_t dil) {
  Tensor w = weight.scalar_type() == at::kBFloat16 ? weight : weight.to(at::kBFloat16);
  return std::get<0>(at::convolution_backward(dy, x, w, c10::nullopt, {stride, stride}, {pad, pad}, {dil, dil}, false, {0, 0}, 1,
                                              {true, false, false}));
}

inline Tensor bias_grad(const Tensor &dy) {
  const int64_t N = dy.size(0), C = dy.size(1), H = dy.size(2), W = dy.size(3), M = N * H * W;
  if (nhwc_pitch(dy) == C && M >= 4096 && bfhip_bn2d_supported(M, (int)C, 1)) {
    const size_t wsb = bfhip_bn2d_workspace_bytes(M, (int)C, 1);
    if (wsb > 0) {
      Tensor out = at::empty({C}, dy.options().dtype(at::kFloat));
      Tensor ws = at::empty({(int64_t)wsb}, dy.options().dtype(at::kByte));
      check(bfhip_colsum(dy.data_ptr(), M, (int)C, 1, out.data_ptr<float>(), ws.data_ptr(), wsb, cur_stream(dy)), "colsum");
      return out;
    }
  }
  return dy.sum({0, 2, 3}, false, at::kFloat);
}

class ConvFn : public torch::autograd::Function<ConvFn> {
 public:
  static tensor_list forward(AutogradContext *ctx, const Tensor &x_, const Tensor &weight, const c10::optional<Tensor> &bias,
                             int64_t stride, int64_t pad, int64_t dil, bool emit_stats, bool dgrad_lib, int64_t fork,
                             const c10::optional<Tensor> &wt) {
    ctx->set_materialize_grads(false);
    Tensor x = as_nhwc_bf16(x_);
    const int64_t N = x.size(0), Cin = x.size(1), H = x.size(2), W = x.size(3);
    const int64_t Cout = weight.size(0), KH = weight.size(2), KW = weight.size(3);
    const int64_t OH = (H + 2 * pad - dil * (KH - 1) - 1) / stride + 1, OW = (W + 2 * pad - dil * (KW - 1) - 1) / stride + 1;
    Tensor w = weight_ohwi(weight);
    Tensor y = empty_nhwc(N, Cout, OH, OW, x.options());
    Tensor partial = emit_stats ? at::empty({(int64_t)bfhip_conv2d_stat_rows((int)N, (int)OH, (int)OW), 2, Cout}, x.options().dtype(at::kFloat))
                                : at::empty({0}, x.options().dtype(at::kFloat));
    Tensor b32;
    const bool has_bias = bias.has_value() && bias->defined();
    if (has_bias) b32 = bias->scalar_type() == at::kFloat ? *bias : bias->to(at::kFloat);
    check(bfhip_conv2d_fwd(x.data_ptr(), (int)nhwc_pitch(x), w.data_ptr(), has_bias ? b32.data_ptr<float>() : nullptr, y.data_ptr(),
                           (int)Cout, (int)N, (int)H, (int)W, (int)Cin, (int)Cout, (int)KH, (int)KW, (int)stride, (int)pad, (int)dil, 0,
                           emit_stats ? partial.data_ptr<float>() : nullptr, cur_stream(x)),
          "conv2d_fwd");
    ctx->save_for_backward({x, weight, (wt.has_value() && wt->defined()) ? *wt : Tensor()});
    ctx->saved_data["geom"] = std::vector<int64_t>{stride, pad, dil, fork, dgrad_lib ? 1 : 0, has_bias ? 1 : 0,
                                                   has_bias ? (int64_t)bias->scalar_type() : 0};
    ctx->mark_non_differentiable({partial});
    if (fork == 2) {
      using torch::indexing::Slice;
      return {y, partial, x.index({Slice(), Slice(), Slice(0, c10::nullopt, 2), Slice(0, c10::nullopt, 2)}).contiguous(at::MemoryFormat::ChannelsLast)};
    }
    if (fork) return {y, partial, x.view_as(x)};
    return {y, partial};
  }

  static tensor_list backward(AutogradContext *ctx, tensor_list grads) {
    auto saved = ctx->get_saved_variables();
    const Tensor &x = saved[0], &weight = saved[1], &wt = saved[2];
    const auto g = ctx->saved_data["geom"].toIntVector();
    const int64_t stride = g[0], pad = g[1], dil = g[2];
    const int fork = (int)g[3];
    const bool dgrad_lib = g[4] != 0, has_bias = g[5] != 0;
    Tensor dy = grads[0];
    Tensor d_alias = grads.size() > 2 ? grads[2] : Tensor();
    tensor_list out(10);
    if (!dy.defined()) {
      if (d_alias.defined() && fork == 2) {
        using torch::indexing::Slice;
        Tensor full = at::zeros_like(x);
        full.index_put_({Slice(), Slice(), Slice(0, c10::nullopt, 2), Slice(0, c10::nullopt, 2)}, d_alias);
        d_alias = full;
      }
      out[0] = d_alias;
      return out;
    }
    dy = as_nhwc_bf16(dy);
    if (ctx->needs_input_grad(0)) {
      if (dgrad_lib) out[0] = add_grad(lib_dgrad(dy, x, weight, stride, pad, dil), d_alias, fork);
      else out[0] = hip_dgrad(dy, x, weight, wt, stride, pad, dil, d_alias, fork == 2 ? 2 : 1);
    }
    if (ctx->needs_input_grad(1)) out[1] = launch_wgrad(x, dy, weight, stride, pad, dil);
    if (has_bias && ctx->needs_input_grad(2)) out[2] = bias_grad(dy).to((at::ScalarType)g[6]);
    return out;
  }
};

tensor_list conv2d(const Tensor &x, const Tensor &weight, const c10::optional<Tensor> &bias, int64_t stride, int64_t pad, int64_t dil,
                   bool emit_stats, bool dgrad_lib, int64_t fork, const c10::optional<Tensor> &wt) {
  return ConvFn::apply(x, weight, bias, stride, pad, dil, emit_stats, dgrad_lib, fork, wt);
}

class LibConvFn : public torch::autograd::Function<LibConvFn> {
 public:
  static Tensor forward(AutogradContext *ctx, const Tensor &x_, const Tensor &weight, int64_t stride, int64_t pad, int64_t dil,
                        bool dgrad_hip, const c10::optional<Tensor> &wt) {
    Tensor x = as_nhwc_bf16(x_);
    Tensor w = weight.scalar_type() == at::kBFloat16 ? weight : weight.to(at::kBFloat16);
    Tensor y;
    {
      c10::impl::ExcludeDispatchKeyGuard no_autocast(c10::DispatchKey::AutocastCUDA);
      y = at::conv2d(x, w, {}, {stride, stride}, {pad, pad}, {dil, dil});
    }
    ctx->save_for_backward({x, weight, (wt.has_value() && wt->defined()) ? *wt : Tensor()});
    ctx->saved_data["geom"] = std::vector<int64_t>{stride, pad, dil, dgrad_hip ? 1 : 0};
    return y;
  }

  static tensor_list backward(AutogradContext *ctx, tensor_list grads) {
    auto saved = ctx->get_saved_variables();
    const Tensor &x = saved[0], &weight = saved[1], &wt = saved[2];
    const auto g = ctx->saved_data["geom"].toIntVector();
    const int64_t stride = g[0], pad = g[1], dil = g[2];
    tensor_list out(7);
    if (!grads[0].defined()) return out;
    Tensor dy = as_nhwc_bf16(grads[0]);
    if (ctx->needs_input_grad(0))
      out[0] = g[3] ? hip_dgrad(dy, x, weight, wt, stride, pad, dil, Tensor(), 1) : lib_dgrad(dy, x, weight, stride, pad, dil);
    if (ctx->needs_input_grad(1)) out[1] = launch_wgrad(x, dy, weight, stride, pad, dil);
    return out;
  }
};

Tensor lib_conv2d(const Tensor &x, const Tensor &weight, int64_t stride, int64_t pad, int64_t dil, bool dgrad_hip,
                  const c10::optional<Tensor> &wt) {
  return LibConvFn::apply(x, weight, stride, pad, dil, dgrad_hip, wt);
}

}

PYBIND11_MODULE(TORCH_EXTENSION_NAME, m) {
  m.doc() = "C++ autograd front-ends over libbevfusion_hip.so (include/bevfusion_hip.h)";
  m.def("bn2d", &bn2d, "fused BatchNorm2d(+residual)(+ReLU), channels-last, training mode; optional statistics partials of the producing conv",
        pybind11::arg("x"), pybind11::arg("residual"), pybind11::arg("weight"), pybind11::arg("bias"), pybind11::arg("running_mean"),
        pybind11::arg("running_var"), pybind11::arg("eps"), pybind11::arg("momentum"), pybind11::arg("relu"),
        pybind11::arg("partial") = c10::optional<Tensor>(), pybind11::arg("relu_bits") = false);
  m.def("bn1d", &bn1d, "fused BatchNorm1d(+residual)(+ReLU) on f32[N, C], training mode");
  m.def("conv2d", &conv2d, "dense convolution on csrc/conv2d.hip (conv2d.py::_Conv2dFunction): [y, partial (empty without statistics)[, x']]",
        pybind11::arg("x"), pybind11::arg("weight"), pybind11::arg("bias"), pybind11::arg("stride"), pybind11::arg("pad"), pybind11::arg("dil"),
        pybind11::arg("emit_stats"), pybind11::arg("dgrad_lib"), pybind11::arg("fork"), pybind11::arg("wt"));
  m.def("lib_conv2d", &lib_conv2d, "library forward, HIP weight gradient (conv2d.py::_LibConvHipWgradFunction)", pybind11::arg("x"),
        pybind11::arg("weight"), pybind11::arg("stride"), pybind11::arg("pad"), pybind11::arg("dil"), pybind11::arg("dgrad_hip"), pybind11::arg("wt"));
  m.def("defer_wgrad", &defer_wgrad, "queue a layer's weight gradient for the grouped launch at the end of the running backward pass");
  m.def("set_wgrad_grouped", [](bool on) { g_grouped = on; });
  m.def("pending_wgrads", &pending_wgrads);
  m.def("abi_version", []() { return bfhip_abi_version(); });
}
```

include/bevfusion_hip.h:

```cpp
#ifndef BEVFUSION_HIP_H_
#define BEVFUSION_HIP_H_

#include <stddef.h>
#include <stdint.h>

#ifdef __cplusplus
extern "C" {
#endif

#define BFHIP_OK 0
#define BFHIP_E_INVALID (-1)
#define BFHIP_E_WORKSPACE (-2)
#define BFHIP_E_LAUNCH (-3)

#define BFHIP_REDUCE_SUM 0
#define BFHIP_REDUCE_MEAN 1
#define BFHIP_REDUCE_MAX 2

#define BFHIP_OP_BEV_POOL_FWD 0
#define BFHIP_OP_BEV_POOL_BWD 1
#define BFHIP_OP_HARD_VOXELIZE 2
#define BFHIP_OP_DYNAMIC_VOXELIZE 3
#define BFHIP_OP_LIFT_SPLAT_FWD 4
#define BFHIP_OP_LIFT_SPLAT_BWD 5
#define BFHIP_OP_SPCONV_FWD 6
#define BFHIP_OP_SPCONV_BWD 7
#define BFHIP_OP_RULEBOOK 8
#define BFHIP_OP_BEV_AUX 9
#define BFHIP_OP_SCATTER_FWD 10
#define BFHIP_OP_SCATTER_BWD 11
#define BFHIP_OP_SPCONV_WGRAD 12
#define BFHIP_OP_RASTER 13
#define BFHIP_OP_SPCONV_WGRAD_MAIN 14
#define BFHIP_OP_CONV2D_FWD 15
#define BFHIP_OP_CONV2D_DGRAD 16
#define BFHIP_OP_CONV2D_WGRAD 17
#define BFHIP_OP_BN2D_FWD 18
#define BFHIP_OP_BN2D_BWD 19
#define BFHIP_OP_CONV2D_PW_FWD 20
#define BFHIP_OP_CONV2D_PW_DGRAD 21
#define BFHIP_OP_COUNT 24

int bfhip_abi_version(void);
const char *bfhip_last_error(void);

void bfhip_profile_enable(int on);
int bfhip_profile_read(int op, double *sum_ms_host, long long *count_host, int reset);

int bfhip_bev_pool_fwd(const float *x, const int32_t *geom, const int32_t *starts,
                       const int32_t *lengths, float *out, int n, int c, int m, int b, int d,
                       int h, int w, const int32_t *m_dev, void *stream);
int bfhip_bev_pool_bwd(const float *out_grad, const int32_t *geom, const int32_t *starts,
                       const int32_t *lengths, float *x_grad, int n, int c, int m, int b, int d,
                       int h, int w, int intervals_cover_all_rows, const int32_t *m_dev,
                       void *stream);

int bfhip_dynamic_voxelize(const float *points, int32_t *coors, int n, int f,
                           const float *voxel_size_host, const float *coors_range_host,
                           void *stream);
size_t bfhip_hard_voxelize_workspace_bytes(int n, int max_points, int max_voxels);
int bfhip_hard_voxelize(const float *points, int n, int f, float *voxels, int32_t *coors,
                        int32_t *num_points_per_voxel, const float *voxel_size_host,
                        const float *coors_range_host, int max_points, int max_voxels,
                        void *workspace, size_t workspace_bytes, int32_t *voxel_num_dev,
                        void *stream);

size_t bfhip_dynamic_scatter_workspace_bytes(int N);
int bfhip_dynamic_scatter_fwd(const float *feats, const int32_t *coors, int N, int C, int reduce_type,
                              float *voxel_feats, int32_t *voxel_coors, int32_t *point2voxel,
                              int32_t *voxel_count, int32_t *counts_dev, void *workspace,
                              size_t workspace_bytes, void *stream);
size_t bfhip_dynamic_scatter_bwd_workspace_bytes(int M, int C);
int bfhip_dynamic_scatter_bwd(float *grad_feats, const float *grad_voxel_feats, const float *feats,
                              const float *voxel_feats, const int32_t *point2voxel,
                              const int32_t *voxel_count, int N, int M, int C, int reduce_type,
                              void *workspace, size_t workspace_bytes, void *stream);
int bfhip_voxel_mean(const float *voxels, const int32_t *num_points, int M, int P, int F, float *out,
                     void *stream);

size_t bfhip_bev_plan_workspace_bytes(long long nprime, long long ncells_times_b);
int bfhip_bev_plan(const float *frustum, const float *post_trans, const float *post_rots_inv,
                   const float *combine, const float *c2l_trans, const float *extra_rots,
                   const float *extra_trans, int B, int N, int D, int HW,
                   const float *origin_host, const float *dx_host, const int32_t *nx_host,
                   uint32_t *sorted_pd, int32_t *starts, int32_t *lengths,
                   int32_t *cell_of_interval, int32_t *interval_order, int32_t *counts_dev, int32_t *cell_of_point,
                   int32_t *geom_sorted, int64_t *ranks_sorted, uint8_t *kept, float *geom_xyz,
                   int mmax, void *workspace, size_t workspace_bytes, void *stream);

int bfhip_lift_splat_fwd(const float *depth, int depth_pitch, const void *feat, int feat_bf16, int feat_pitch,
                         const uint32_t *sorted_pd, const int32_t *starts, const int32_t *lengths,
                         const int32_t *cell_of_interval, const int32_t *interval_order ,
                         const int32_t *counts_dev, int mmax, int C, long long out_cells, void *out, int out_bf16,
                         void *stream);
int bfhip_lift_splat_bwd(const void *out_grad, int grad_bf16 , const float *depth,
                         int depth_pitch,
                         const void *feat, int feat_bf16, int feat_pitch, const int32_t *cell_of_point,
                         int num_cams, int D, int HW, int C, float *d_depth, int d_depth_pitch,
                         void *d_feat, int d_feat_pitch, void *stream);

int bfhip_conv_out_shape(const int *in_shape, const int *ksize, const int *stride,
                         const int *padding, const int *dilation, int *out_shape);
size_t bfhip_rulebook_subm_workspace_bytes(int N);
int bfhip_rulebook_subm(const int32_t *indices, int N, int B, const int *in_shape, const int *ksize,
                        const int *dilation, int32_t *pair_fwd, int32_t *n_pairs_dev, uint32_t *row_mask,
                        int32_t *perm, void *workspace, size_t workspace_bytes, void *stream);
size_t bfhip_rulebook_sparse_workspace_bytes(int B, const int *in_shape, const int *ksize,
                                             const int *stride, const int *padding,
                                             const int *dilation);
int bfhip_rulebook_sparse_count(const int32_t *indices, int N, const int32_t *n_in_dev, int B, const int *in_shape,
                                const int *ksize, const int *stride, const int *padding, const int *dilation,
                                int32_t *counts_dev, void *workspace, size_t workspace_bytes, void *stream);
int bfhip_rulebook_sparse_out_indices(int B, const int *in_shape, const int *ksize, const int *stride,
                                      const int *padding, const int *dilation, int cap, int32_t *out_indices,
                                      void *workspace, size_t workspace_bytes, void *stream);
int bfhip_rulebook_sparse_fill(const int32_t *indices, int N, int B, const int *in_shape,
                               const int *ksize, const int *stride, const int *padding,
                               const int *dilation, int n_out, int32_t *out_indices,
                               int32_t *pair_fwd, int32_t *pair_bwd, int32_t *counts_dev,
                               uint32_t *mask_fwd, int32_t *perm_fwd, uint32_t *mask_bwd, int32_t *perm_bwd,
                               void *sort_workspace, size_t sort_workspace_bytes,
                               void *workspace, size_t workspace_bytes, void *stream);
size_t bfhip_rulebook_sort_rows_workspace_bytes(int n_rows, int KV);
int bfhip_rulebook_sort_rows(const int32_t *pairs, int ld, int KV, int n_rows, uint32_t *row_mask,
                             int32_t *perm, void *workspace, size_t workspace_bytes, void *stream);
size_t bfhip_rulebook_validate_workspace_bytes(int n_rows);
int bfhip_rulebook_validate(const int32_t *pairs, int ld, int KV, int n_rows, int n_src, const int32_t *perm,
                            const uint32_t *row_mask, int32_t *status_dev, void *workspace, size_t workspace_bytes,
                            void *stream);
size_t bfhip_spconv_workspace_bytes(int KV, int Cin, int Cout);
int bfhip_spconv_gemm(const float *in, const float *W, const int32_t *pairs, int ld, int KV,
                      int n_rows, int Cin, int Cout, int transpose, int flip, const int32_t *perm,
                      const uint32_t *row_mask, float *out, void *workspace, size_t workspace_bytes,
                      void *stream);
int bfhip_spconv_gemm_bf16(const void *in, const float *W, const int32_t *pairs, int ld, int KV,
                           int n_rows, int Cin, int Cout, int transpose, int flip, const int32_t *perm,
                           const uint32_t *row_mask, void *out, int io_bf16, void *workspace, size_t workspace_bytes,
                           void *stream);
size_t bfhip_spconv_wgrad_workspace_bytes(int KV, int Cin, int Cout, int n_rows);
int bfhip_spconv_wgrad(const void *in, const void *dout, const int32_t *pairs, int ld, int KV,
                       int n_rows, int Cin, int Cout, const int32_t *perm, float *dW, int io_bf16, void *workspace,
                       size_t workspace_bytes, void *stream);
int bfhip_sparse_to_bev(const float *feats, const int32_t *indices, int N, int C, int B, int X,
                        int Y, int Z, float *out, void *stream);
int bfhip_bev_to_sparse(const float *grad_out, const int32_t *indices, int N, int C, int B, int X,
                        int Y, int Z, float *grad_feats, void *stream);
int bfhip_sparse_to_bev_nhwc(const float *feats, const int32_t *indices, int N, int C, int B, int X, int Y, int Z,
                             int dtype, void *out, void *stream);
int bfhip_bev_nhwc_to_sparse(const void *grad_out, long long stride_b, long long stride_x, long long stride_y,
                             int dtype, const int32_t *indices, int N, int C, int Z, float *grad_feats, void *stream);

size_t bfhip_depth_lift_bwd_workspace_bytes(void);
int bfhip_depth_lift_bwd(const void *dy, const void *d, long long M, float *out, void *workspace, size_t workspace_bytes, void *stream);
size_t bfhip_rasterise_depth_workspace_bytes(int ncam, int iH, int iW);
int bfhip_rasterise_depth(const float *points, int n, int f, const float *inv_rot, const float *aug_trans,
                          const float *lidar2image, const float *img_aug, int ncam, int iH, int iW,
                          float *depth, float *counts, int fH, int fW, int D, const float *dbound_host,
                          void *workspace, size_t workspace_bytes, void *stream);
int bfhip_depth_histogram(const float *depth, int BN, int iH, int iW, int fH, int fW, int D,
                          const float *dbound_host, float *counts, float *distr, void *stream);

size_t bfhip_bn1d_workspace_bytes(int N, int C);
int bfhip_bn1d_fwd(const float *x, const float *residual, const float *gamma, const float *beta, int N, int C,
                   float eps, float momentum, int relu, float *running_mean, float *running_var, float *stats,
                   float *y, const int32_t *n_rows_dev, void *workspace, size_t workspace_bytes, void *stream);
int bfhip_bn1d_bwd(const float *dy, const float *y, const float *x, const float *stats, const float *gamma, int N,
                   int C, int relu, float *dx, float *dres, float *dgb, const int32_t *n_rows_dev, void *workspace,
                   size_t workspace_bytes, void *stream);

int bfhip_bn2d_supported(long long M, int C, int dtype);
int bfhip_colsum(const void *x, long long M, int C, int dtype, float *out, void *workspace, size_t workspace_bytes, void *stream);
size_t bfhip_bn2d_workspace_bytes(long long M, int C, int dtype);
int bfhip_bn2d_fwd(const void *x, const void *residual, const float *gamma, const float *beta, long long M, int C,
                   int dtype, float eps, float momentum, int relu, float *running_mean, float *running_var,
                   float *stats, void *y, const int32_t *m_dev, void *workspace, size_t workspace_bytes, void *stream);
int bfhip_bn2d_bwd(const void *dy, const void *x, const void *y, const float *stats, const float *gamma, long long M,
                   int C, int dtype, int relu, void *dx, void *dres, float *dgb, const int32_t *m_dev, void *workspace,
                   size_t workspace_bytes, void *stream);

size_t bfhip_xty_workspace_bytes(long long K, int M, int N);
int bfhip_xty(const void *X, const void *Y, long long K, int M, int N, int dtype, float *out, void *workspace,
              size_t workspace_bytes, void *stream);

int bfhip_attn_max_queries(void);
size_t bfhip_attn_workspace_bytes(int B, int H, int Lq, int Lk);
int bfhip_attn_fwd(const void *Q, const void *K, const void *V, int B, int H, int Lq, int Lk, float scale,
                   float dropout_p, unsigned long long seed, const unsigned long long *seed_dev, void *O, float *lse,
                   void *workspace, size_t workspace_bytes, void *stream);
int bfhip_attn_bwd(const void *Q, const void *K, const void *V, const void *O, const void *dO, const float *lse, int B,
                   int H, int Lq, int Lk, float scale, float dropout_p, unsigned long long seed,
                   const unsigned long long *seed_dev, void *dQ, void *dK, void *dV, void *workspace, size_t workspace_bytes,
                   void *stream);
int bfhip_attn_dropout_mask(int B, int H, int Lq, int Lk, float dropout_p, unsigned long long seed,
                            const unsigned long long *seed_dev, unsigned char *mask, void *stream);

int bfhip_upsample2x_nhwc(const void *src, void *dst, int B, int H, int W, int C, int dtype, int dir, void *stream);

int bfhip_maxpool3x3s2_fwd(const void *x, int N, int H, int W, int C, void *y, unsigned char *tap, void *stream);
int bfhip_maxpool3x3s2_bwd(const void *dy, const unsigned char *tap, int N, int H, int W, int C, void *dx, void *stream);

int bfhip_decode_boxes(const float *center, const float *height, const float *dim, const float *rot,
                       const float *vel, int B, int P, int ld, int p_off, const float *cfg_host, float *boxes,
                       void *stream);
int bfhip_predict_compact(const float *boxes, const float *scores, const long long *labels, int B, int P, int W,
                          const float *range_host, int use_threshold, float threshold, float *out_boxes, float *out_scores,
                          int32_t *out_labels, int32_t *counts, void *stream);
int bfhip_assign_cost(const float *boxes, int W, const float *cls_logits, int C, int ld, int p_off,
                      const float *gt_boxes, int Wg, const int32_t *gt_labels, const int32_t *n_gt, int B, int P,
                      int G, const float *cfg_host, float *cost, float *iou, void *stream);
int bfhip_hungarian(const float *cost, const int32_t *n_gt, int B, int P, int G, int32_t *assigned,
                    int32_t *status, void *stream);
int bfhip_assign_targets(const int32_t *assigned, const float *iou, const float *gt_boxes, int Wg,
                         const int32_t *gt_labels, int B, int P, int G, int num_classes, int code_size,
                         const float *cfg_host, int32_t *labels, float *label_weights, float *bbox_targets,
                         float *bbox_weights, float *ious, void *stream);
int bfhip_draw_heatmap(const float *gt_boxes, int Wg, const int32_t *gt_labels, const int32_t *n_gt, int B, int G,
                       int num_classes, int H, int W, const float *cfg_host, double gaussian_overlap,
                       int min_radius, float *heatmap, void *stream);
size_t bfhip_gaussian_focal_loss_workspace_bytes(long long n);
int bfhip_gaussian_focal_loss(const float *logits, const float *target, long long n, float clip_eps,
                              float *loss_sum_npos, float *grad, void *workspace, size_t workspace_bytes,
                              void *stream);
int bfhip_circle_nms(const float *dets, int n, float thresh, int post_max_size, int32_t *keep, int32_t *n_keep,
                     void *stream);
size_t bfhip_rotate_nms_workspace_bytes(int n, int pre_max_size);
int bfhip_rotate_nms(const float *boxes, const float *scores, int n, float thresh, int pre_max_size, int post_max_size,
                     int32_t *keep, int32_t *n_keep, void *workspace, size_t workspace_bytes, void *stream);
int bfhip_query_losses(const float *cls_logits, const int32_t *labels, const float *label_weights,
                       const float *box_pred, const float *bbox_targets, const float *bbox_weights,
                       const float *code_weights, int B, int C, int P, int K, int ld, int p_off, float gamma,
                       float alpha, float *grad_cls, float *grad_box, float *loss_sums, void *stream);

int bfhip_voxel_compact_mean(const float *voxels, const int32_t *coors, const int32_t *num_points, const int32_t *counts_dev,
                             int B, int max_voxels, int P, int F, int cap, float *feats, int32_t *out_coords,
                             int32_t *n_total_dev, void *stream);

int bfhip_conv2d_supported(int N, int H, int W, int Cin, int Cout, int KH, int KW, int stride, int pad, int dil);
int bfhip_conv2d_stat_rows(int N, int OH, int OW);
int bfhip_conv2d_fwd(const void *x, int ldx, const void *w, const float *bias, void *y, int ldy, int N, int H, int W, int Cin,
                     int Cout, int KH, int KW, int stride, int pad, int dil, int out_f32, float *stat_partial, void *stream);
size_t bfhip_conv2d_dgrad_workspace_bytes(int Cin, int Cout, int KH, int KW);
int bfhip_conv2d_dgrad(const void *dy, int ldg, const void *w, void *dx, int ldx, int N, int H, int W, int Cin, int Cout,
                       int KH, int KW, int stride, int pad, int dil, int out_f32, void *workspace, size_t workspace_bytes,
                       void *stream);
int bfhip_conv2d_dgrad_wt(const void *dy, int ldg, const void *wt, const void *addend, int addend_stride, void *dx, int ldx, int N,
                          int H, int W, int Cin, int Cout, int KH, int KW, int stride, int pad, int dil, int out_f32, void *stream);
int bfhip_conv2d_dgrad_fuses_addend(int KH, int KW, int stride, int pad, int out_f32);
int bfhip_conv2d_wt_segment_bytes(void);
int bfhip_conv2d_weight_transpose_batched(const void *segs_dev, int nseg, long long total_blocks, void *stream);
int bfhip_split_bf16x3(const float *src, long long P, int C, void *chan, int order_chan, void *batch, int order_batch, void *stream);
int bfhip_conv2d_launch_choice(int dir, int N, int H, int W, int Cin, int Cout, int KH, int KW, int stride, int pad, int dil,
                               int out_f32, int32_t *out_host);
int bfhip_conv2d_wgrad_choice(int N, int H, int W, int Cin, int Cout, int KH, int KW, int stride, int pad, int dil,
                              int32_t *out_host);
size_t bfhip_conv2d_wgrad_workspace_bytes(int N, int OH, int OW, int Cin, int Cout, int KH, int KW);
int bfhip_conv2d_wgrad(const void *x, int ldx, const void *dy, int ldg, void *dw, int N, int H, int W, int Cin, int Cout,
                       int KH, int KW, int stride, int pad, int dil, int dw_bf16, void *workspace, size_t workspace_bytes,
                       void *stream);
typedef struct bfhip_wgrad_layer {
  const void *x, *dy;
  void *dw;
  int32_t ldx, ldg, N, H, W, Cin, Cout, KH, KW, stride, pad, dil, dw_bf16, reserved;
} bfhip_wgrad_layer;
size_t bfhip_conv2d_wgrad_group_table_bytes(int n_layers);
int bfhip_conv2d_wgrad_groupable(int N, int H, int W, int Cin, int Cout, int KH, int KW, int stride, int pad, int dil);
int bfhip_conv2d_wgrad_group_plan(const void *layers, int n_layers, int target_steps, void *table_host, size_t table_bytes,
                                  size_t *slab_bytes);
int bfhip_conv2d_wgrad_group_launch(const void *table_host, const void *table_dev, void *slab, size_t slab_bytes, void *stream);
int bfhip_bn2d_fwd_partials(const void *x, const void *residual, const float *gamma, const float *beta, long long M, int C,
                            int dtype, float eps, float momentum, int relu, float *running_mean, float *running_var,
                            float *stats, void *y, const float *partial, int nblk, const int32_t *m_dev, void *stream);
int bfhip_bn2d_fwd_partials_mask(const void *x, const void *residual, const float *gamma, const float *beta, long long M, int C,
                                 int dtype, float eps, float momentum, int relu, float *running_mean, float *running_var,
                                 float *stats, void *y, const float *partial, int nblk, const int32_t *m_dev,
                                 unsigned char *relu_mask, void *stream);
int bfhip_bn2d_bwd_mask(const void *dy, const void *x, const unsigned char *relu_mask, const float *stats, const float *gamma,
                        long long M, int C, int dtype, void *dx, void *dres, float *dgb, const int32_t *m_dev, void *workspace,
                        size_t workspace_bytes, void *stream);

int bfhip_adamw_segment_bytes(void);
int bfhip_adamw_chunk_elems(void);
int bfhip_adamw_step(const void *segs_dev, const int64_t *grad_ptrs_dev, const int32_t *chunks_dev, int n_chunks,
                     float *partial_dev, float *scalars_dev, float lr, float beta1, float beta2, float eps,
                     float weight_decay, float max_norm, void *stream);
int bfhip_adamw_step_groups(const void *segs_dev, const int64_t *grad_ptrs_dev, const int32_t *chunks_dev, int n_chunks,
                            float *partial_dev, float *scalars_dev, float *groups_dev, const float *groups_host, int n_groups,
                            float max_norm, void *stream);

int bfhip_swin_attn_supported(int B, int Hp, int Wp, int heads, int window, int head_dim, int shift);
int bfhip_swin_attn_parts(int B, int Hp, int Wp, int heads);
int bfhip_swin_attn_fwd(const void *qkv, long long qkv_pitch, const float *bias, int B, int Hp, int Wp, int heads, int shift,
                        float scale, void *out, float *lse, void *stream);
int bfhip_swin_attn_bwd(const void *qkv, long long qkv_pitch, const float *bias, const void *out, const void *dout,
                        const float *lse, int B, int Hp, int Wp, int heads, int shift, float scale, void *dqkv,
                        float *dbias_partial, int parts, void *stream);

int bfhip_layernorm_supported(long long M, int C, int x_dtype, int y_dtype);
int bfhip_layernorm_parts(long long M, int C);
int bfhip_layernorm_fwd(const void *x, const void *branch, const float *scale, long long rows_per_sample, const float *gamma,
                        const float *beta, long long M, int C, float eps, int x_dtype, int branch_dtype, int y_dtype, void *s,
                        void *y, float *mean_rstd, void *stream);
int bfhip_layernorm_bwd(const void *s, const float *mean_rstd, const float *gamma, const void *dy, const void *dsum,
                        const float *scale, long long rows_per_sample, long long M, int C, int x_dtype, int branch_dtype,
                        int y_dtype, void *dx, void *dbranch, float *partial, int parts, float *dgamma, float *dbeta,
                        void *stream);

int bfhip_bn_eval_supported(long long M, int C, int dtype);
int bfhip_bn_eval_parts(long long M, int C, int dtype);
int bfhip_bn_eval_fwd(const void *x, const void *residual, const float *gamma, const float *beta, const float *running_mean,
                      const float *running_var, long long M, int C, int dtype, float eps, int relu, void *y, void *stream);
int bfhip_bn_eval_bwd(const void *dy, const void *y, const void *x, const float *gamma, const float *running_mean,
                      const float *running_var, long long M, int C, int dtype, float eps, int relu, void *dx, void *dres,
                      float *partial, float *dgb, void *stream);

int bfhip_bn_eval_rows_fwd(const void *x, const void *residual, const float *gamma, const float *beta,
                           const float *running_mean, const float *running_var, long long M, int C, int dtype, float eps,
                           int relu, void *y, const int32_t *rows_dev, void *stream);
int bfhip_bn_eval_rows_bwd(const void *dy, const void *y, const void *x, const float *gamma, const float *running_mean,
                           const float *running_var, long long M, int C, int dtype, float eps, int relu, void *dx, void *dres,
                           float *partial, float *dgb, const int32_t *rows_dev, void *stream);

typedef struct bfhip_img_desc {
  const void *data;
  int h, w;
} bfhip_img_desc;
int bfhip_img_preprocess_max_samples(void);
int bfhip_img_preprocess(const bfhip_img_desc *samples_host, int n_samples, int views, int src_dtype, int swap_rb, int normalise,
                         const float *mean_host, const float *std_host, float pad_value, int Hp, int Wp, int out_dtype,
                         int pixel_major, void *out, void *stream);

typedef struct bfhip_image_aug_cam {
  const void *data;
  int h, w;
  int crop[2];
  int flip, rotates;
  int a[6];
  int h_off, h_taps, h_first, h_count;
  int v_off, v_taps, v_first, v_count;
} bfhip_image_aug_cam;
int bfhip_image_aug_max_taps(void);
int bfhip_image_aug_max_cams(void);
int bfhip_image_aug_supported(int src_h, int src_w, int new_h, int new_w, int fH, int fW, int h_taps, int v_taps);
int bfhip_image_aug(const bfhip_image_aug_cam *cams_host, int n_samples, int views, const int32_t *tables_host,
                    const int32_t *tables_dev, long long table_ints, int fH, int fW, void *mid, int swap_rb, int normalise,
                    const float *mean_host, const float *std_host, float pad_value, int Hp, int Wp, int out_dtype,
                    int pixel_major, void *out, void *stream);

typedef struct bfhip_grid_mask {
  int active;
  int d, length, st_h, st_w;
  int use_h, use_w, mode;
  int hh, ww;
  int crop[2];
  int r, rotates;
  int a[6];
} bfhip_grid_mask;
int bfhip_image_aug_masked(const bfhip_image_aug_cam *cams_host, const bfhip_grid_mask *masks_host, int n_samples, int views,
                           const int32_t *tables_host, const int32_t *tables_dev, long long table_ints, int fH, int fW, void *mid,
                           int swap_rb, int normalise, const float *mean_host, const float *std_host, float pad_value, int Hp,
                           int Wp, int out_dtype, int pixel_major, void *out, void *stream);

#define BFHIP_POINTS_AUG_ROUNDS 6
typedef struct bfhip_points_aug_sample {
  const float *points;
  int n;
  int flags;
  float rot[9];
  float trans[3];
  float scale;
  float range[6];
  uint32_t keys[BFHIP_POINTS_AUG_ROUNDS];
} bfhip_points_aug_sample;
int bfhip_points_aug_block(void);
size_t bfhip_points_aug_workspace_bytes(long long total_rows, int n_samples);
int bfhip_points_aug(const bfhip_points_aug_sample *samples_host, int n_samples, int C, float *out, int32_t *kept,
                     void *workspace, size_t workspace_bytes, void *stream);

typedef struct bfhip_points_aug_paste_desc {
  const float *points;
  int n_points;
  const float *planes;
  int n_boxes;
} bfhip_points_aug_paste_desc;
int bfhip_points_aug_max_boxes(void);
int bfhip_points_aug_paste(const bfhip_points_aug_sample *samples_host, const bfhip_points_aug_paste_desc *pastes_host,
                           int n_samples, int C, float *out, int32_t *kept, void *workspace, size_t workspace_bytes,
                           void *stream);

#define BFHIP_POINTS_AUG_MAX_SEGMENTS 16
typedef struct bfhip_points_aug_segment {
  int first;
  int flags;
  float dt;
  float radius;
  double m[9];
  double t[3];
} bfhip_points_aug_segment;
typedef struct bfhip_points_aug_sweeps_desc {
  const bfhip_points_aug_segment *segments;
  int n_segments;
  int first[BFHIP_POINTS_AUG_MAX_SEGMENTS + 1];
} bfhip_points_aug_sweeps_desc;
int bfhip_points_aug_max_sweeps(void);
int bfhip_points_aug_sweeps(const bfhip_points_aug_sample *samples_host, const bfhip_points_aug_paste_desc *pastes_host,
                            const bfhip_points_aug_sweeps_desc *sweeps_host, int n_samples, int C, float *out, int32_t *kept,
                            void *workspace, size_t workspace_bytes, void *stream);

int bfhip_query_init_supported(int B, int C, int H, int W, int K, int Ch, int nms_kernel_size, int row_dtype);
size_t bfhip_query_init_workspace_bytes(int B, int C, int H, int W);
int bfhip_query_init_fwd(const float *h, long long h_sb, long long h_sc, long long h_sy, long long h_sx, int B, int C, int H, int W,
                         unsigned nms_free_mask, const void *flat, long long flat_sb, long long flat_sr, int Ch, int row_dtype,
                         int K, int pos_w, long long *top_class, long long *top_index, float *query_pos,
                         float *query_heatmap_score, void *rows, void *workspace, size_t workspace_bytes, void *stream);
int bfhip_query_init_bwd(const long long *top_index, const void *d_rows, int B, int K, int Ch, long long HW, int row_dtype,
                         void *d_flat, void *stream);

#define BFHIP_JPEG_R_OK 0
#define BFHIP_JPEG_R_PROGRESSIVE 1
#define BFHIP_JPEG_R_ARITHMETIC 2
#define BFHIP_JPEG_R_PRECISION 3
#define BFHIP_JPEG_R_COMPONENTS 4
#define BFHIP_JPEG_R_MULTI_SCAN 5
#define BFHIP_JPEG_R_QUANT16 6
#define BFHIP_JPEG_R_SAMPLING 7
#define BFHIP_JPEG_R_EXIF_ORIENTATION 8
#define BFHIP_JPEG_R_NOT_BASELINE 9
#define BFHIP_JPEG_R_COLOUR_SPACE 10
typedef struct bfhip_jpeg_header {
  int32_t width, height, ncomp;
  int32_t supported, reason;
  int32_t restart_interval;
  int32_t mcus_x, mcus_y;
  int32_t hs[3], vs[3];
  int32_t block_cols[3], block_rows[3];
  int64_t coef_offset[3];
  int64_t coef_bytes;
  uint16_t quant[3][64];
} bfhip_jpeg_header;
typedef struct bfhip_jpeg_frame {
  int64_t coef_off[3];
  int64_t plane_off[3];
  int64_t rgb_off;
  int32_t width, height;
  int32_t hs, vs;
  int32_t block_cols[3], block_rows[3];
  uint16_t quant[3][64];
} bfhip_jpeg_frame;
int bfhip_jpeg_parse(const uint8_t *bytes, size_t n, bfhip_jpeg_header *header);
int bfhip_jpeg_entropy_decode(const uint8_t *bytes, size_t n, const bfhip_jpeg_header *header, int16_t *coef, size_t coef_bytes);
int bfhip_jpeg_decode(const bfhip_jpeg_frame *frames_host, const bfhip_jpeg_frame *frames_dev, int n_frames,
                      const int16_t *coef_dev, size_t coef_elems, uint8_t *planes_dev, size_t planes_bytes, uint8_t *rgb_dev,
                      size_t rgb_bytes, void *stream);

#define BFHIP_JPEG_ENC_OVERFLOW 1
#define BFHIP_JPEG_ENC_BAD_COEF 2
typedef struct bfhip_jpeg_enc_stats {
  int64_t bytes;
  int64_t stuffed;
  int64_t zrl;
  int64_t eob;
  int32_t max_ac_category, max_dc_category;
} bfhip_jpeg_enc_stats;
typedef struct bfhip_jpeg_enc_frame {
  int64_t rgb_off;
  int64_t coef_off[3];
  int64_t out_off, capacity;
  int64_t ws_off;
  int32_t width, height;
  int32_t hs, vs;
  int32_t block_cols[3], block_rows[3];
  uint16_t quant[3][64];
} bfhip_jpeg_enc_frame;
int bfhip_jpeg_entropy_encode(const bfhip_jpeg_header *header, const int16_t *coef, size_t coef_bytes, int restart_interval,
                              uint8_t *out, size_t capacity, bfhip_jpeg_enc_stats *stats);
int bfhip_jpeg_encode_supported(int width, int height, int hs, int vs);
size_t bfhip_jpeg_encode_workspace_bytes(int width, int height, int hs, int vs);
int bfhip_jpeg_encode_max_frames(void);
int bfhip_jpeg_forward(const bfhip_jpeg_enc_frame *frames_host, const bfhip_jpeg_enc_frame *frames_dev, int n_frames,
                       const uint8_t *rgb_dev, size_t rgb_bytes, int16_t *coef_dev, size_t coef_elems, void *stream);
int bfhip_jpeg_entropy_encode_device(const bfhip_jpeg_enc_frame *frames_host, const bfhip_jpeg_enc_frame *frames_dev, int n_frames,
                                     const int16_t *coef_dev, size_t coef_elems, void *workspace, size_t workspace_bytes,
                                     uint8_t *out_dev, size_t out_bytes, int64_t *result_dev, void *stream);
int bfhip_jpeg_encode(const bfhip_jpeg_enc_frame *frames_host, const bfhip_jpeg_enc_frame *frames_dev, int n_frames,
                      const uint8_t *rgb_dev, size_t rgb_bytes, int16_t *coef_dev, size_t coef_elems, void *workspace,
                      size_t workspace_bytes, uint8_t *out_dev, size_t out_bytes, int64_t *result_dev, void *stream);

#define BFHIP_PNG_OVERFLOW 1
typedef struct bfhip_png_stats {
  int64_t bytes;
  int64_t bands, stored_bands, dynamic_bands;
  int64_t tokens;
  int32_t max_code_length, overflow;
} bfhip_png_stats;
typedef struct bfhip_png_frame {
  int64_t src_off;
  int64_t out_off, capacity;
  int64_t ws_off, res_off;
  int64_t n_bytes, band_bytes;
  int32_t width, height;
} bfhip_png_frame;
int bfhip_png_encode_supported(int width, int height, int band_rows);
int bfhip_png_encode_max_frames(void);
size_t bfhip_png_workspace_bytes(int64_t n_bytes, int64_t band_bytes, int with_filter);
size_t bfhip_png_capacity(int64_t n_bytes, int64_t band_bytes);
size_t bfhip_png_result_words(int64_t n_bytes, int64_t band_bytes);
int bfhip_png_encode(const bfhip_png_frame *frames_host, const bfhip_png_frame *frames_dev, int n_frames, const uint8_t *rgb_dev,
                     size_t rgb_bytes, void *workspace, size_t workspace_bytes, uint8_t *out_dev, size_t out_bytes,
                     uint32_t *result_dev, size_t result_words, void *stream);
int bfhip_png_deflate(const bfhip_png_frame *jobs_host, const bfhip_png_frame *jobs_dev, int n_jobs, const uint8_t *data_dev,
                      size_t data_bytes, void *workspace, size_t workspace_bytes, uint8_t *out_dev, size_t out_bytes,
                      uint32_t *result_dev, size_t result_words, void *stream);
int bfhip_png_filter_host(const uint8_t *rgb, int width, int height, uint8_t *out, size_t out_bytes);
int bfhip_png_huffman_lengths(const uint32_t *hist, int n_symbols, int max_len, uint8_t *lens);
int bfhip_png_deflate_host(const uint8_t *data, size_t n, size_t band_bytes, uint8_t *out, size_t capacity, uint32_t *bands,
                           size_t band_slots, bfhip_png_stats *stats);

int bfhip_points_in_boxes_block(void);
int bfhip_points_in_boxes_max_boxes(void);
size_t bfhip_points_in_boxes_workspace_bytes(long long n, int K);
int bfhip_points_in_boxes_count(const float *points, long long n, int C, const float *planes, int K, int32_t *counts,
                                uint64_t *member, void *workspace, size_t workspace_bytes, void *stream);
int bfhip_points_in_boxes_gather(const float *points, long long n, int C, const float *centers, int K, const int32_t *counts,
                                 const uint64_t *member, long long total, float *out, long long capacity, const void *workspace,
                                 size_t workspace_bytes, void *stream);

int bfhip_detection_eval_max_preds(void);
int bfhip_detection_eval_max_gt(void);
int bfhip_detection_eval_max_thresholds(void);
int bfhip_detection_eval_max_classes(void);
int bfhip_detection_match(const float *pred, const float *score, const int32_t *pred_cls, const int32_t *pred_off, long long n_pred,
                          const float *gt, const int32_t *gt_cls, const int32_t *gt_off, long long n_gt, int n_samples,
                          int n_classes, const double *dist_ths, int n_ths, int tp_index, uint64_t half_period_mask,
                          uint64_t attr_empty_mask, int32_t *match, double *pred_err, void *stream);
size_t bfhip_detection_curves_workspace_bytes(long long n_pred, int n_ths);
int bfhip_detection_curves(const float *score, const int32_t *order, const int32_t *cls_off, const int32_t *match,
                           const double *pred_err, long long n_pred, int n_classes, int n_ths, int tp_index, const int32_t *npos,
                           const double *levels, double min_precision, int first_level, uint64_t attr_empty_mask,
                           double *precision, double *confidence, double *err_curves, double *ap, double *tp_err,
                           int32_t *max_recall_ind, void *workspace, size_t workspace_bytes, void *stream);

int bfhip_vis_max_dim(void);
int bfhip_vis_max_thickness(void);
int bfhip_vis_max_scale(void);
size_t bfhip_vis_workspace_bytes(int n_views, int n_boxes, int edges);
int bfhip_vis_camera_segments(const float *table, int n_boxes, const float *lidar2cam, const float *cam2img, int n_views,
                              float near, int thickness, int H, int W, void *workspace, size_t workspace_bytes, void *stream);
int bfhip_vis_bev_segments(const float *table, int n_boxes, float x0, float y1, float px_per_m, int thickness, int H, int W,
                           void *workspace, size_t workspace_bytes, void *stream);
int bfhip_vis_composite(const uint8_t *src, int n_views, int H, int W, const void *workspace, size_t workspace_bytes, int n_boxes,
                        int edges, const int32_t *colors, const int32_t *cell_view, int rows, int cols, int scale, uint8_t *out,
                        void *stream);
int bfhip_vis_bev_points(const float *points, long long n, int C, float x0, float y0, float px_per_m, int point_size,
                         uint8_t *canvas, int H, int W, void *stream);

#ifdef __cplusplus
}
#endif
#endif
```

Measured before the change: 156.7 frames/s.

## Add split-K path for conv forward and transposed dgrad with fp32 slab workspace

Adds split-K variants of the implicit-GEMM and pointwise conv kernels. When an output grid has too few tiles to fill the GPU, the K loop is spread over several blocks that write fp32 partial slabs, and a reduction combines them into the output. New _ws entry points take a cached per-stream workspace, and both the Python path and the torch extension path call them. This raises occupancy for small-M, large-K layers, at the cost of extra slab traffic, a reduce launch and a 32MB-or-larger workspace.

```diff
diff --git a/bevfusion-3d_object_detection_amd/_lib.py b/bevfusion-3d_object_detection_amd/_lib.py
--- a/bevfusion-3d_object_detection_amd/_lib.py
+++ b/bevfusion-3d_object_detection_amd/_lib.py
@@ -103,6 +103,10 @@
     "bfhip_conv2d_dgrad": (_c_int, [_c_vp, _c_int, _c_vp, _c_vp, _c_int] + [_c_int] * 11 + [_c_vp, _c_sz, _c_vp]),
     "bfhip_conv2d_dgrad_wt": (_c_int, [_c_vp, _c_int, _c_vp, _c_vp, _c_int, _c_vp, _c_int] + [_c_int] * 11 + [_c_vp]),
     "bfhip_conv2d_dgrad_fuses_addend": (_c_int, [_c_int] * 5),
+    "bfhip_conv2d_split_workspace_bytes": (_c_sz, [_c_int] * 12),
+    "bfhip_conv2d_split_choice": (_c_int, [_c_int] * 12 + [_c_vp]),
+    "bfhip_conv2d_fwd_ws": (_c_int, [_c_vp, _c_int, _c_vp, _c_vp, _c_vp, _c_int] + [_c_int] * 11 + [_c_vp, _c_vp, _c_sz, _c_vp]),
+    "bfhip_conv2d_dgrad_wt_ws": (_c_int, [_c_vp, _c_int, _c_vp, _c_vp, _c_int, _c_vp, _c_int] + [_c_int] * 11 + [_c_vp, _c_sz, _c_vp]),
     "bfhip_split_bf16x3": (_c_int, [_c_vp, ctypes.c_longlong, _c_int, _c_vp, _c_int, _c_vp, _c_int, _c_vp]),
     "bfhip_conv2d_wt_segment_bytes": (_c_int, []),
     "bfhip_conv2d_weight_transpose_batched": (_c_int, [_c_vp, _c_int, ctypes.c_longlong, _c_vp]),
diff --git a/bevfusion-3d_object_detection_amd/conv2d.py b/bevfusion-3d_object_detection_amd/conv2d.py
--- a/bevfusion-3d_object_detection_amd/conv2d.py
+++ b/bevfusion-3d_object_detection_amd/conv2d.py
@@ -207,6 +207,26 @@
     return buf
 
 
+_SPLIT_WS = {}
+_SPLIT_BYTES = {}
+
+
+def _split_workspace(direction, device, stream, geom):
+    key = (direction,) + geom
+    need = _SPLIT_BYTES.get(key)
+    if need is None:
+        need = _SPLIT_BYTES[key] = int(_lib.load().bfhip_conv2d_split_workspace_bytes(direction, *geom, 0))
+    if need == 0:
+        return None, 0
+    buf = _SPLIT_WS.get((device, stream))
+    if buf is None or buf.numel() < need:
+        if torch.cuda.is_current_stream_capturing():
+            return None, 0
+        _SPLIT_WS.pop((device, stream), None)
+        buf = _SPLIT_WS[(device, stream)] = torch.empty(max(need, 32 << 20), dtype=torch.uint8, device=device)
+    return buf.data_ptr(), buf.numel()
+
+
 def _nhwc_view(t):
     N, C, H, W = t.shape
     sn, sc, sh, sw = t.stride()
@@ -250,8 +270,10 @@
         b32 = None
         if bias is not None:
             b32 = bias if bias.dtype == torch.float32 else bias.float()
-        _lib.call("bfhip_conv2d_fwd", x.data_ptr(), _nhwc_view(x), w.data_ptr(), _lib.ptr(b32), y.data_ptr(), Cout, N, H, W, Cin,
-                  Cout, KH, KW, stride, pad, dil, 0, _lib.ptr(partial), _lib.stream_of(x))
+        stream = _lib.stream_of(x)
+        ws, ws_bytes = _split_workspace(0, x.device, stream, (N, H, W, Cin, Cout, KH, KW, stride, pad, dil))
+        _lib.call("bfhip_conv2d_fwd_ws", x.data_ptr(), _nhwc_view(x), w.data_ptr(), _lib.ptr(b32), y.data_ptr(), Cout, N, H, W, Cin,
+                  Cout, KH, KW, stride, pad, dil, 0, _lib.ptr(partial), ws, ws_bytes, stream)
         ctx.save_for_backward(x, weight)
         ctx.geom = (stride, pad, dil)
         ctx.dgrad_lib = dgrad_lib
@@ -327,8 +349,9 @@
         fuse = (addend is not None and addend.dtype == torch.bfloat16 and tuple(addend.shape) == want
                 and addend.is_contiguous(memory_format=torch.channels_last) and addend.data_ptr() % 16 == 0
                 and _lib.load().bfhip_conv2d_dgrad_fuses_addend(KH, KW, stride, pad, 0))
-        _lib.call("bfhip_conv2d_dgrad_wt", dy.data_ptr(), _nhwc_view(dy), cached[0].data_ptr(), _lib.ptr(addend) if fuse else None,
-                  addend_stride, dx.data_ptr(), Cin, N, H, W, Cin, Cout, KH, KW, stride, pad, dil, 0, stream)
+        ws, ws_bytes = _split_workspace(1, x.device, stream, (N, H, W, Cin, Cout, KH, KW, stride, pad, dil))
+        _lib.call("bfhip_conv2d_dgrad_wt_ws", dy.data_ptr(), _nhwc_view(dy), cached[0].data_ptr(), _lib.ptr(addend) if fuse else None,
+                  addend_stride, dx.data_ptr(), Cin, N, H, W, Cin, Cout, KH, KW, stride, pad, dil, 0, ws, ws_bytes, stream)
         return dx if fuse else _add_grad(dx, addend, addend_stride)
     ws = _workspace(x.device, _lib.load().bfhip_conv2d_dgrad_workspace_bytes(Cin, Cout, KH, KW), stream)
     _lib.call("bfhip_conv2d_dgrad", dy.data_ptr(), _nhwc_view(dy), _weight_ohwi(weight).data_ptr(), dx.data_ptr(), Cin, N, H,
diff --git a/bevfusion-3d_object_detection_amd/csrc/conv2d.hip b/bevfusion-3d_object_detection_amd/csrc/conv2d.hip
--- a/bevfusion-3d_object_detection_amd/csrc/conv2d.hip
+++ b/bevfusion-3d_object_detection_amd/csrc/conv2d.hip
@@ -169,10 +169,12 @@
   }
 }
 
-template <int WGM, int WGN, int MI, int NI, int STAGES, bool OUT_F32, int MODE>
-__global__ __launch_bounds__(WGM * WGN * 64, (STAGES == 1 ? 4 : (WGM * WGN > 4 ? 1 : 2))) void conv_igemm_kernel(
-    const bf16_t *__restrict__ x, const bf16_t *__restrict__ wt, const float *__restrict__ bias, void *__restrict__ y,
-    float *__restrict__ stat_partial, ConvGeom g, int tiles_m, int tiles_n) {
+template <int WGM, int WGN, int MI, int NI, int STAGES, bool OUT_F32, int MODE, bool SPLIT>
+__device__ __forceinline__ void conv_igemm_body(unsigned char *smem, const bf16_t *__restrict__ x, const bf16_t *__restrict__ wt,
+                                                const float *__restrict__ bias, void *__restrict__ y,
+                                                float *__restrict__ stat_partial, const ConvGeom g, int tiles_m, int tiles_n,
+                                                int splits, int per) {
+  static_assert(!SPLIT || (MODE != 2 && OUT_F32), "split-K: forward / plain transposed gather into fp32 slabs");
   constexpr bool TR = MODE != 0;
   constexpr int NWAVES = WGM * WGN, NTHREADS = NWAVES * 64;
   constexpr int BN = WGN * NI * 32, BM = WGM * MI * 32, BK = 64;
@@ -181,10 +183,14 @@
   constexpr int NB = (BN / 8) / NWAVES;
   constexpr int GL = NA + NB;
   static_assert(NA >= 1 && NA * 8 * NWAVES == BM && NB >= 1 && NB * 8 * NWAVES == BN, "tiles must split into whole DMA instructions");
-  extern __shared__ __attribute__((aligned(1024))) unsigned char smem[];
   unsigned *taps = (unsigned *)(smem + STAGES * S_BYTES);
   const int tid = threadIdx.x, lane = tid & 63, w = tid >> 6;
-  const long long lb = xcd_chunked_block(blockIdx.x, (long long)tiles_m * tiles_n);
+  long long lb = xcd_chunked_block(blockIdx.x, (long long)tiles_m * tiles_n * (SPLIT ? splits : 1));
+  int split = 0;
+  if (SPLIT) {
+    split = (int)(lb % splits);
+    lb /= splits;
+  }
   const int tn = (int)(lb % tiles_n);
   int tm = (int)(lb / tiles_n);
   long long M = g.M;
@@ -312,21 +318,26 @@
   const int l31 = lane & 31, lh = lane >> 5, rswz = (lane >> 1) & 7;
   const int aoff = (wm * (MI * 32) + l31) * 128, boff = A_BYTES + (wn * (NI * 32) + l31) * 128;
 
+  int tb = 0, te = nt;
+  if (SPLIT) {
+    tb = split * per;
+    te = tb + per < nt ? tb + per : nt;
+  }
 #pragma unroll
   for (int s0 = 0; s0 < STAGES - 1; ++s0)
-    if (s0 < nt) stage(s0, s0);
+    if (tb + s0 < te) stage(tb + s0, s0);
   int buf = 0, nbuf = STAGES - 1;
-  for (int t = 0; t < nt; ++t) {
+  for (int t = tb; t < te; ++t) {
     if (STAGES == 1) {
-      if (t) __syncthreads();
+      if (t != tb) __syncthreads();
       stage(t, 0);
     }
-    if (STAGES <= 2 || nt - 1 - t == 0) wait_vmcnt<0>();
-    else if (STAGES == 3 || nt - 1 - t == 1) wait_vmcnt<GL>();
+    if (STAGES <= 2 || te - 1 - t == 0) wait_vmcnt<0>();
+    else if (STAGES == 3 || te - 1 - t == 1) wait_vmcnt<GL>();
     else wait_vmcnt<2 * GL>();
     __builtin_amdgcn_s_barrier();
     const unsigned char *pA = smem + buf * S_BYTES + aoff, *pB = smem + buf * S_BYTES + boff;
-    if (STAGES > 1 && t + STAGES - 1 < nt) stage(t + STAGES - 1, nbuf);
+    if (STAGES > 1 && t + STAGES - 1 < te) stage(t + STAGES - 1, nbuf);
 #pragma unroll
     for (int ks = 0; ks < 4; ++ks) {
       const int pos = ((2 * ks + lh) ^ rswz) << 4;
@@ -343,11 +354,115 @@
     buf = buf + 1 == STAGES ? 0 : buf + 1;
     nbuf = nbuf + 1 == STAGES ? 0 : nbuf + 1;
   }
-  if (MODE == 2)
+  if (SPLIT)
+    igemm_epilogue<WGM, WGN, MI, NI, true>(acc, smem, tm, m0, n0, M, g.Kout, g.Kout, nullptr,
+                                           (float *)y + (size_t)split * (size_t)M * (size_t)g.Kout, nullptr);
+  else if (MODE == 2)
     igemm_epilogue<WGM, WGN, MI, NI, OUT_F32, RowParityClass>(acc, smem, tm, m0, n0, M, g.Kout, g.ldy, bias, y, stat_partial,
                                                               RowParityClass{pc.Hc, pc.Wc, g.OH, g.OW, pc.h0, pc.w0, g.stride});
   else
     igemm_epilogue<WGM, WGN, MI, NI, OUT_F32>(acc, smem, tm, m0, n0, M, g.Kout, g.ldy, bias, y, stat_partial);
+}
+
+template <int WGM, int WGN, int MI, int NI, int STAGES, bool OUT_F32, int MODE>
+__global__ __launch_bounds__(WGM * WGN * 64, (STAGES == 1 ? 4 : (WGM * WGN > 4 ? 1 : 2))) void conv_igemm_kernel(
+    const bf16_t *__restrict__ x, const bf16_t *__restrict__ wt, const float *__restrict__ bias, void *__restrict__ y,
+    float *__restrict__ stat_partial, ConvGeom g, int tiles_m, int tiles_n) {
+  extern __shared__ __attribute__((aligned(1024))) unsigned char smem[];
+  conv_igemm_body<WGM, WGN, MI, NI, STAGES, OUT_F32, MODE, false>(smem, x, wt, bias, y, stat_partial, g, tiles_m, tiles_n, 1, 0);
+}
+
+template <int NI, int STAGES, int MODE>
+__global__ __launch_bounds__(256, (STAGES == 1 ? 4 : 2)) void conv_igemm_splitk_kernel(
+    const bf16_t *__restrict__ x, const bf16_t *__restrict__ wt, float *__restrict__ slabs, ConvGeom g, int tiles_m, int tiles_n,
+    int splits, int per) {
+  extern __shared__ __attribute__((aligned(1024))) unsigned char smem[];
+  conv_igemm_body<2, 2, 2, NI, STAGES, true, MODE, true>(smem, x, wt, nullptr, slabs, nullptr, g, tiles_m, tiles_n, splits, per);
+}
+
+template <int NI, bool OUT_F32, bool SPLIT>
+__device__ __forceinline__ void conv_pw_body(unsigned char *smem, const bf16_t *__restrict__ x, const bf16_t *__restrict__ wt,
+                                             const float *__restrict__ bias, void *__restrict__ y, float *__restrict__ stat_partial,
+                                             long long M, int C, int ldx, int Kout, int ldw, int ldy, int tiles_m, int tiles_n,
+                                             const Addend &add, int splits, int per) {
+  static_assert(!SPLIT || OUT_F32, "split-K writes fp32 slabs");
+  constexpr int WGN = 2, MI = 2;
+  constexpr int BM = 128, BN = NI * 64;
+  constexpr int A_BYTES = BM * 128;
+  constexpr int NA = 4, NB = BN / 32;
+  const int tid = threadIdx.x, lane = tid & 63, w = tid >> 6;
+  long long lb = xcd_chunked_block(blockIdx.x, (long long)tiles_m * tiles_n * (SPLIT ? splits : 1));
+  int split = 0;
+  if (SPLIT) {
+    split = (int)(lb % splits);
+    lb /= splits;
+  }
+  const int tn = (int)(lb % tiles_n), tm = (int)(lb / tiles_n);
+  const long long m0 = (long long)tm * BM;
+  const int n0 = tn * BN;
+  const int nq = C >> 3, nt = (nq + 7) >> 3;
+  int tb = 0, te = nt;
+  if (SPLIT) {
+    tb = split * per;
+    te = tb + per < nt ? tb + per : nt;
+  }
+  const int lrow = lane >> 3, lpos = lane & 7;
+  const bf16_t *zsrc = zero_src();
+  const bf16_t *arow[NA], *brow[NB];
+#pragma unroll
+  for (int i = 0; i < NA; ++i) {
+    const long long m = m0 + w * 32 + i * 8 + lrow;
+    arow[i] = m < M ? x + (unsigned)m * (unsigned)ldx : nullptr;
+  }
+#pragma unroll
+  for (int i = 0; i < NB; ++i) {
+    const int co = n0 + w * (NB * 8) + i * 8 + lrow;
+    brow[i] = co < Kout ? wt + (size_t)co * ldw : nullptr;
+  }
+  f32x16 acc[MI][NI];
+#pragma unroll
+  for (int mi = 0; mi < MI; ++mi)
+#pragma unroll
+    for (int ni = 0; ni < NI; ++ni)
+#pragma unroll
+      for (int r = 0; r < 16; ++r) acc[mi][ni][r] = 0.f;
+  const int wm = w / WGN, wn = w % WGN;
+  const int l31 = lane & 31, lh = lane >> 5, rswz = (lane >> 1) & 7;
+  const unsigned char *pA = smem + (wm * 64 + l31) * 128, *pB = smem + A_BYTES + (wn * (NI * 32) + l31) * 128;
+  unsigned char *dA = smem + (w * 32) * 128, *dB = smem + A_BYTES + (w * (NB * 8)) * 128;
+  for (int t = tb; t < te; ++t) {
+    if (t != tb) __syncthreads();
+#pragma unroll
+    for (int i = 0; i < NA; ++i) {
+      const int q = t * 8 + (lpos ^ (((w * 32 + i * 8 + lrow) >> 1) & 7));
+      glds16(arow[i] && q < nq ? arow[i] + q * 8 : zsrc, dA + i * 1024);
+    }
+#pragma unroll
+    for (int i = 0; i < NB; ++i) {
+      const int q = t * 8 + (lpos ^ (((w * (NB * 8) + i * 8 + lrow) >> 1) & 7));
+      glds16(brow[i] && q < nq ? brow[i] + q * 8 : zsrc, dB + i * 1024);
+    }
+    wait_vmcnt<0>();
+    __builtin_amdgcn_s_barrier();
+#pragma unroll
+    for (int ks = 0; ks < 4; ++ks) {
+      const int pos = ((2 * ks + lh) ^ rswz) << 4;
+      bf16x8 a[MI], b[NI];
+#pragma unroll
+      for (int mi = 0; mi < MI; ++mi) a[mi] = *(const bf16x8 *)(pA + mi * 32 * 128 + pos);
+#pragma unroll
+      for (int ni = 0; ni < NI; ++ni) b[ni] = *(const bf16x8 *)(pB + ni * 32 * 128 + pos);
+#pragma unroll
+      for (int mi = 0; mi < MI; ++mi)
+#pragma unroll
+        for (int ni = 0; ni < NI; ++ni) acc[mi][ni] = __builtin_amdgcn_mfma_f32_32x32x16_bf16(a[mi], b[ni], acc[mi][ni], 0, 0, 0);
+    }
+  }
+  if (SPLIT)
+    igemm_epilogue<2, WGN, MI, NI, true>(acc, smem, tm, m0, n0, M, Kout, Kout, nullptr,
+                                         (float *)y + (size_t)split * (size_t)M * (size_t)Kout, nullptr);
+  else
+    igemm_epilogue<2, WGN, MI, NI, OUT_F32>(acc, smem, tm, m0, n0, M, Kout, ldy, bias, y, stat_partial, RowIdentity(), add);
 }
 
 template <int NI, bool OUT_F32, int DIR>
@@ -355,70 +470,112 @@
                                                          const float *__restrict__ bias, void *__restrict__ y,
                                                          float *__restrict__ stat_partial, long long M, int C, int ldx, int Kout,
                                                          int ldw, int ldy, int tiles_m, int tiles_n, Addend add) {
-  constexpr int WGN = 2, MI = 2;
-  constexpr int BM = 128, BN = NI * 64;
-  constexpr int A_BYTES = BM * 128;
-  constexpr int NA = 4, NB = BN / 32;
   extern __shared__ __attribute__((aligned(1024))) unsigned char smem[];
-  const int tid = threadIdx.x, lane = tid & 63, w = tid >> 6;
-  const long long lb = xcd_chunked_block(blockIdx.x, (long long)tiles_m * tiles_n);
-  const int tn = (int)(lb % tiles_n), tm = (int)(lb / tiles_n);
-  const long long m0 = (long long)tm * BM;
-  const int n0 = tn * BN;
-  const int nq = C >> 3, nt = (nq + 7) >> 3;
-  const int lrow = lane >> 3, lpos = lane & 7;
-  const bf16_t *zsrc = zero_src();
-  const bf16_t *arow[NA], *brow[NB];
-#pragma unroll
-  for (int i = 0; i < NA; ++i) {
-    const long long m = m0 + w * 32 + i * 8 + lrow;
-    arow[i] = m < M ? x + (unsigned)m * (unsigned)ldx : nullptr;
-  }
-#pragma unroll
-  for (int i = 0; i < NB; ++i) {
-    const int co = n0 + w * (NB * 8) + i * 8 + lrow;
-    brow[i] = co < Kout ? wt + (size_t)co * ldw : nullptr;
-  }
-  f32x16 acc[MI][NI];
-#pragma unroll
-  for (int mi = 0; mi < MI; ++mi)
-#pragma unroll
-    for (int ni = 0; ni < NI; ++ni)
-#pragma unroll
-      for (int r = 0; r < 16; ++r) acc[mi][ni][r] = 0.f;
-  const int wm = w / WGN, wn = w % WGN;
-  const int l31 = lane & 31, lh = lane >> 5, rswz = (lane >> 1) & 7;
-  const unsigned char *pA = smem + (wm * 64 + l31) * 128, *pB = smem + A_BYTES + (wn * (NI * 32) + l31) * 128;
-  unsigned char *dA = smem + (w * 32) * 128, *dB = smem + A_BYTES + (w * (NB * 8)) * 128;
-  for (int t = 0; t < nt; ++t) {
-    if (t) __syncthreads();
-#pragma unroll
-    for (int i = 0; i < NA; ++i) {
-      const int q = t * 8 + (lpos ^ (((w * 32 + i * 8 + lrow) >> 1) & 7));
-      glds16(arow[i] && q < nq ? arow[i] + q * 8 : zsrc, dA + i * 1024);
-    }
-#pragma unroll
-    for (int i = 0; i < NB; ++i) {
-      const int q = t * 8 + (lpos ^ (((w * (NB * 8) + i * 8 + lrow) >> 1) & 7));
-      glds16(brow[i] && q < nq ? brow[i] + q * 8 : zsrc, dB + i * 1024);
-    }
-    wait_vmcnt<0>();
-    __builtin_amdgcn_s_barrier();
-#pragma unroll
-    for (int ks = 0; ks < 4; ++ks) {
-      const int pos = ((2 * ks + lh) ^ rswz) << 4;
-      bf16x8 a[MI], b[NI];
-#pragma unroll
-      for (int mi = 0; mi < MI; ++mi) a[mi] = *(const bf16x8 *)(pA + mi * 32 * 128 + pos);
-#pragma unroll
-      for (int ni = 0; ni < NI; ++ni) b[ni] = *(const bf16x8 *)(pB + ni * 32 * 128 + pos);
-#pragma unroll
-      for (int mi = 0; mi < MI; ++mi)
-#pragma unroll
-        for (int ni = 0; ni < NI; ++ni) acc[mi][ni] = __builtin_amdgcn_mfma_f32_32x32x16_bf16(a[mi], b[ni], acc[mi][ni], 0, 0, 0);
-    }
-  }
-  igemm_epilogue<2, WGN, MI, NI, OUT_F32>(acc, smem, tm, m0, n0, M, Kout, ldy, bias, y, stat_partial, RowIdentity(), add);
+  conv_pw_body<NI, OUT_F32, false>(smem, x, wt, bias, y, stat_partial, M, C, ldx, Kout, ldw, ldy, tiles_m, tiles_n, add, 1, 0);
+}
+
+template <int NI, int DIR>
+__global__ __launch_bounds__(256, 4) void conv_pw_splitk_kernel(const bf16_t *__restrict__ x, const bf16_t *__restrict__ wt,
+                                                                float *__restrict__ slabs, long long M, int C, int ldx, int Kout,
+                                                                int ldw, int tiles_m, int tiles_n, int splits, int per) {
+  extern __shared__ __attribute__((aligned(1024))) unsigned char smem[];
+  conv_pw_body<NI, true, true>(smem, x, wt, nullptr, slabs, nullptr, M, C, ldx, Kout, ldw, Kout, tiles_m, tiles_n,
+                               Addend{nullptr, 0, 0, 0, 0}, splits, per);
+}
+
+template <bool OUT_F32>
+__global__ __launch_bounds__(256) void conv_splitk_reduce_kernel(const float *__restrict__ slabs, int splits, long long M, int Kout,
+                                                                 const float *__restrict__ bias, void *__restrict__ y, int ldy,
+                                                                 float *__restrict__ stat_partial, Addend add) {
+  __shared__ float sred[32][64][2];
+  const int tid = threadIdx.x, cx = tid & 7, ry = tid >> 3;
+  const int col = blockIdx.y * 64 + cx * 8;
+  const long long m0 = (long long)blockIdx.x * 128;
+  const bool col_ok = col < Kout;
+  const size_t slab = (size_t)M * (size_t)Kout;
+  float bv[8], s[8], s2[8];
+#pragma unroll
+  for (int j = 0; j < 8; ++j) {
+    bv[j] = (bias && col_ok) ? bias[col + j] : 0.f;
+    s[j] = s2[j] = 0.f;
+  }
+  for (int i = 0; i < 4; ++i) {
+    const long long m = m0 + ry + 32 * i;
+    if (m >= M || !col_ok) continue;
+    const float *p = slabs + (size_t)m * Kout + col;
+    float v[8];
+    {
+      const float4 a = *(const float4 *)p, b = *(const float4 *)(p + 4);
+      v[0] = a.x; v[1] = a.y; v[2] = a.z; v[3] = a.w; v[4] = b.x; v[5] = b.y; v[6] = b.z; v[7] = b.w;
+    }
+    for (int k = 1; k < splits; ++k) {
+      const float4 a = *(const float4 *)(p + k * slab), b = *(const float4 *)(p + k * slab + 4);
+      v[0] += a.x; v[1] += a.y; v[2] += a.z; v[3] += a.w; v[4] += b.x; v[5] += b.y; v[6] += b.z; v[7] += b.w;
+    }
+#pragma unroll
+    for (int j = 0; j < 8; ++j) {
+      s[j] += v[j];
+      s2[j] += v[j] * v[j];
+      v[j] += bv[j];
+    }
+    if (OUT_F32) {
+      float *dst = (float *)y + (size_t)m * ldy + col;
+      if ((((uintptr_t)dst) & 15) == 0) {
+        *(float4 *)dst = make_float4(v[0], v[1], v[2], v[3]);
+        *(float4 *)(dst + 4) = make_float4(v[4], v[5], v[6], v[7]);
+      } else {
+#pragma unroll
+        for (int j = 0; j < 8; ++j) dst[j] = v[j];
+      }
+      continue;
+    }
+    unsigned o[8];
+#pragma unroll
+    for (int j = 0; j < 8; ++j) o[j] = bf16_rne(v[j]);
+    if (add.p) {
+      const bf16_t *rs = nullptr;
+      if (add.sub == 2) {
+        const unsigned mu = (unsigned)m, hw = (unsigned)(add.H * add.W);
+        const unsigned n = mu / hw, rem = mu - n * hw;
+        const unsigned h = rem / (unsigned)add.W, w = rem - h * (unsigned)add.W;
+        if (((h | w) & 1u) == 0)
+          rs = add.p + ((size_t)((n * (unsigned)((add.H + 1) >> 1) + (h >> 1)) * (unsigned)((add.W + 1) >> 1) + (w >> 1)) * add.ld + col);
+      } else {
+        rs = add.p + ((size_t)m * add.ld + col);
+      }
+      if (rs) {
+        unsigned short r16[8];
+        if ((((uintptr_t)rs) & 15) == 0) {
+          *(uint4 *)r16 = *(const uint4 *)rs;
+        } else {
+#pragma unroll
+          for (int j = 0; j < 8; ++j) r16[j] = rs[j];
+        }
+#pragma unroll
+        for (int j = 0; j < 8; ++j) o[j] = bf16_rne(__uint_as_float(o[j] << 16) + __uint_as_float((unsigned)r16[j] << 16));
+      }
+    }
+    bf16_t *dst = (bf16_t *)y + (size_t)m * ldy + col;
+    if ((((uintptr_t)dst) & 15) == 0) {
+      *(uint4 *)dst = make_uint4(o[0] | (o[1] << 16), o[2] | (o[3] << 16), o[4] | (o[5] << 16), o[6] | (o[7] << 16));
+    } else {
+#pragma unroll
+      for (int j = 0; j < 8; ++j) dst[j] = (bf16_t)o[j];
+    }
+  }
+  if (!stat_partial) return;
+#pragma unroll
+  for (int j = 0; j < 8; ++j) {
+    sred[ry][cx * 8 + j][0] = s[j];
+    sred[ry][cx * 8 + j][1] = s2[j];
+  }
+  __syncthreads();
+  if (tid < 128) {
+    const int c = tid & 63, which = tid >> 6;
+    float t = 0.f;
+    for (int r = 0; r < 32; ++r) t += sred[r][c][which];
+    if (blockIdx.y * 64 + c < Kout) stat_partial[((size_t)blockIdx.x * 2 + which) * Kout + blockIdx.y * 64 + c] = t;
+  }
 }
 
 __global__ __launch_bounds__(256) void conv_weight_transpose_kernel(const bf16_t *__restrict__ w, bf16_t *__restrict__ wt,
@@ -560,6 +717,40 @@
   return c;
 }
 
+constexpr int kSplitMinSteps = 16, kSplitMinPer = 8, kSplitMax = 8;
+constexpr size_t kSplitSlabMax = (size_t)96 << 20;
+struct SplitChoice { int splits, per, nt; };
+
+SplitChoice choose_splitk(const ConvGeom &g, int out_f32, int cus) {
+  static const int knob = env_int("BFHIP_CONV_SPLITK", 1);
+  const int nt = (g.nq + 7) / 8;
+  const SplitChoice none = {1, nt, nt};
+  if (knob <= 0 || g.transposed == 2) return none;
+  const IgemmChoice c0 = choose_igemm(g, out_f32, cus);
+  if (!c0.pointwise && c0.shape == 2) return none;
+  const IgemmChoice c = choose_igemm(g, 1, cus);
+  const long long tiles = (long long)c.tiles_m * c.tiles_n;
+  long long want = knob;
+  if (knob == 1) {
+    const long long slots = (long long)(c.BN == 64 ? 3 : 2) * cus;
+    if (nt < kSplitMinSteps || tiles * 2 > slots) return none;
+    want = slots / tiles;
+    if (want > nt / kSplitMinPer) want = nt / kSplitMinPer;
+  }
+  if (want > kSplitMax) want = kSplitMax;
+  const size_t slab = (size_t)g.M * (size_t)g.Kout * 4;
+  if (want > (long long)(kSplitSlabMax / slab)) want = (long long)(kSplitSlabMax / slab);
+  if (want > nt) want = nt;
+  for (; want >= 2; --want) {
+    const int per = (int)((nt + want - 1) / want);
+    const int splits = (nt + per - 1) / per;
+    if (splits < 2) break;
+    if (knob == 1 && nt - (splits - 1) * per < kSplitMinPer) continue;
+    return SplitChoice{splits, per, nt};
+  }
+  return none;
+}
+
 struct IgemmArgs { const bf16_t *x, *wt; const float *bias; void *y; float *stat_partial; ConvGeom g; hipStream_t s; Addend add; };
 
 template <int NI, bool F32, int DIR>
@@ -584,10 +775,56 @@
 template <int NI, int ST>
 void launch_ig128(const IgemmArgs &a, const IgemmChoice &c, int f32) { f32 ? launch_ig<2, 2, 2, NI, ST, true>(a, c) : launch_ig<2, 2, 2, NI, ST, false>(a, c); }
 
+template <int NI, int ST>
+void launch_ig_split(const IgemmArgs &a, const IgemmChoice &c, const SplitChoice &k) {
+  const dim3 grid((unsigned)((long long)c.tiles_m * c.tiles_n * k.splits));
+  if (a.g.transposed)
+    launch_big_lds<conv_igemm_splitk_kernel<NI, ST, 1>>(80 * 1024, grid, dim3(256), c.lds, a.s, a.x, a.wt, (float *)a.y, a.g, c.tiles_m,
+                                                        c.tiles_n, k.splits, k.per);
+  else
+    launch_big_lds<conv_igemm_splitk_kernel<NI, ST, 0>>(80 * 1024, grid, dim3(256), c.lds, a.s, a.x, a.wt, (float *)a.y, a.g, c.tiles_m,
+                                                        c.tiles_n, k.splits, k.per);
+}
+template <int NI>
+void launch_pw_split(const IgemmArgs &a, const IgemmChoice &c, const SplitChoice &k) {
+  const dim3 grid((unsigned)((long long)c.tiles_m * c.tiles_n * k.splits));
+  if (a.g.transposed)
+    launch_big_lds<conv_pw_splitk_kernel<NI, 1>>(64 * 1024, grid, dim3(256), c.lds, a.s, a.x, a.wt, (float *)a.y, a.g.M, a.g.C, a.g.ldx,
+                                                 a.g.Kout, a.g.ldw, c.tiles_m, c.tiles_n, k.splits, k.per);
+  else
+    launch_big_lds<conv_pw_splitk_kernel<NI, 0>>(64 * 1024, grid, dim3(256), c.lds, a.s, a.x, a.wt, (float *)a.y, a.g.M, a.g.C, a.g.ldx,
+                                                 a.g.Kout, a.g.ldw, c.tiles_m, c.tiles_n, k.splits, k.per);
+}
+
+size_t splitk_workspace_bytes(const ConvGeom &g, const SplitChoice &k) {
+  return k.splits < 2 ? 0 : align_up((size_t)k.splits * (size_t)g.M * (size_t)g.Kout * 4, 256);
+}
+
 int launch_igemm(const void *x, const void *wt, const float *bias, void *y, float *stat_partial, const ConvGeom &g, int out_f32,
-                 hipStream_t s, const char *what, Addend add = Addend{nullptr, 0, 0, 0, 0}) {
+                 hipStream_t s, const char *what, Addend add = Addend{nullptr, 0, 0, 0, 0}, void *workspace = nullptr,
+                 size_t workspace_bytes = 0) {
   BFHIP_REQUIRE(!add.p || (takes_pointwise(g) && !out_f32),
                 "%s: an addend is only fused into the pointwise kernel (1x1, stride 1, no padding, bf16 output)", what);
+  if (workspace) {
+    const SplitChoice k = choose_splitk(g, out_f32, device_cus());
+    if (k.splits > 1) {
+      BFHIP_REQUIRE(workspace_bytes >= splitk_workspace_bytes(g, k) && ((uintptr_t)workspace % 16) == 0,
+                    "%s: split-K workspace too small or misaligned (bfhip_conv2d_split_workspace_bytes)", what);
+      const IgemmChoice c = choose_igemm(g, 1, device_cus());
+      const IgemmArgs a = {(const bf16_t *)x, (const bf16_t *)wt, nullptr, workspace, nullptr, g, s, Addend{nullptr, 0, 0, 0, 0}};
+      if (c.pointwise) c.BN == 128 ? launch_pw_split<2>(a, c, k) : launch_pw_split<1>(a, c, k);
+      else if (c.shape == 1) c.stages == 1 ? launch_ig_split<2, 1>(a, c, k) : launch_ig_split<2, 2>(a, c, k);
+      else c.stages == 1 ? launch_ig_split<1, 1>(a, c, k) : launch_ig_split<1, 2>(a, c, k);
+      const dim3 rgrid((unsigned)ceil_div(g.M, 128), (unsigned)ceil_div(g.Kout, 64));
+      if (out_f32)
+        hipLaunchKernelGGL(conv_splitk_reduce_kernel<true>, rgrid, dim3(256), 0, s, (const float *)workspace, k.splits, g.M, g.Kout, bias,
+                           y, g.ldy, stat_partial, add);
+      else
+        hipLaunchKernelGGL(conv_splitk_reduce_kernel<false>, rgrid, dim3(256), 0, s, (const float *)workspace, k.splits, g.M, g.Kout,
+                           bias, y, g.ldy, stat_partial, add);
+      return check_launch(what);
+    }
+  }
   const IgemmChoice c = choose_igemm(g, out_f32, device_cus());
   IgemmArgs a = {(const bf16_t *)x, (const bf16_t *)wt, bias, y, stat_partial, g, s, add};
   for (int k = 0; g.transposed == 2 && k <= g.ncls; ++k) a.g.cls[k].tile0 = c.tile0[k];
@@ -615,9 +852,9 @@
 
 BFHIP_EXPORT int bfhip_conv2d_stat_rows(int N, int OH, int OW) { return ceil_div((long long)N * OH * OW, 128); }
 
-BFHIP_EXPORT int bfhip_conv2d_fwd(const void *x, int ldx, const void *w, const float *bias, void *y, int ldy, int N, int H, int W,
-                                  int Cin, int Cout, int KH, int KW, int stride, int pad, int dil, int out_f32,
-                                  float *stat_partial, void *stream_) {
+static int conv2d_fwd_impl(const void *x, int ldx, const void *w, const float *bias, void *y, int ldy, int N, int H, int W, int Cin,
+                           int Cout, int KH, int KW, int stride, int pad, int dil, int out_f32, float *stat_partial, void *workspace,
+                           size_t workspace_bytes, void *stream_) {
   BFHIP_REQUIRE(bfhip_conv2d_supported(N, H, W, Cin, Cout, KH, KW, stride, pad, dil), "conv2d_fwd: unsupported geometry");
   BFHIP_REQUIRE(x && w && y, "conv2d_fwd: null pointer");
   BFHIP_REQUIRE(dma_operand_ok(x, ldx, Cin) && ((uintptr_t)w % 16) == 0 && ldy >= Cout, kOperandMsg, "conv2d_fwd");
@@ -626,17 +863,58 @@
   BFHIP_REQUIRE((long long)N * H * W * ldx < (1LL << 31), "conv2d_fwd: tensors of 2^31 elements or more are not supported");
   ProfScope ps;
   prof_begin(takes_pointwise(g) ? BFHIP_OP_CONV2D_PW_FWD : BFHIP_OP_CONV2D_FWD, (hipStream_t)stream_, &ps);
-  const int rc = launch_igemm(x, w, bias, y, stat_partial, g, out_f32, (hipStream_t)stream_, "conv2d_fwd");
+  const int rc = launch_igemm(x, w, bias, y, stat_partial, g, out_f32, (hipStream_t)stream_, "conv2d_fwd", Addend{nullptr, 0, 0, 0, 0},
+                              workspace, workspace_bytes);
   prof_end(&ps);
   return rc;
+}
+
+BFHIP_EXPORT int bfhip_conv2d_fwd(const void *x, int ldx, const void *w, const float *bias, void *y, int ldy, int N, int H, int W,
+                                  int Cin, int Cout, int KH, int KW, int stride, int pad, int dil, int out_f32,
+                                  float *stat_partial, void *stream_) {
+  return conv2d_fwd_impl(x, ldx, w, bias, y, ldy, N, H, W, Cin, Cout, KH, KW, stride, pad, dil, out_f32, stat_partial, nullptr, 0,
+                         stream_);
+}
+
+BFHIP_EXPORT int bfhip_conv2d_fwd_ws(const void *x, int ldx, const void *w, const float *bias, void *y, int ldy, int N, int H, int W,
+                                     int Cin, int Cout, int KH, int KW, int stride, int pad, int dil, int out_f32,
+                                     float *stat_partial, void *workspace, size_t workspace_bytes, void *stream_) {
+  return conv2d_fwd_impl(x, ldx, w, bias, y, ldy, N, H, W, Cin, Cout, KH, KW, stride, pad, dil, out_f32, stat_partial, workspace,
+                         workspace_bytes, stream_);
+}
+
+static ConvGeom query_geom(int dir, int N, int H, int W, int Cin, int Cout, int KH, int KW, int stride, int pad, int dil);
+
+BFHIP_EXPORT size_t bfhip_conv2d_split_workspace_bytes(int dir, int N, int H, int W, int Cin, int Cout, int KH, int KW, int stride,
+                                                       int pad, int dil, int out_f32) {
+  if ((dir != 0 && dir != 1) || !bfhip_conv2d_supported(N, H, W, Cin, Cout, KH, KW, stride, pad, dil)) return 0;
+  const ConvGeom g = query_geom(dir, N, H, W, Cin, Cout, KH, KW, stride, pad, dil);
+  if (dir ? g.H <= 0 || g.W <= 0 : g.OH <= 0 || g.OW <= 0) return 0;
+  return splitk_workspace_bytes(g, choose_splitk(g, out_f32, device_cus()));
+}
+
+BFHIP_EXPORT int bfhip_conv2d_split_choice(int dir, int N, int H, int W, int Cin, int Cout, int KH, int KW, int stride, int pad,
+                                           int dil, int out_f32, int32_t *out_host) {
+  BFHIP_REQUIRE(out_host && (dir == 0 || dir == 1), "conv2d_split_choice: bad arguments");
+  BFHIP_REQUIRE(bfhip_conv2d_supported(N, H, W, Cin, Cout, KH, KW, stride, pad, dil), "conv2d_split_choice: unsupported geometry");
+  const ConvGeom g = query_geom(dir, N, H, W, Cin, Cout, KH, KW, stride, pad, dil);
+  BFHIP_REQUIRE((dir ? g.H > 0 && g.W > 0 : g.OH > 0 && g.OW > 0), "conv2d_split_choice: empty output");
+  const SplitChoice k = choose_splitk(g, out_f32, device_cus());
+  for (int i = 0; i < 2 + 2 * kSplitMax; ++i) out_host[i] = 0;
+  out_host[0] = k.splits;
+  out_host[1] = k.nt;
+  for (int i = 0; i < k.splits && i < kSplitMax; ++i) {
+    out_host[2 + 2 * i] = i * k.per;
+    out_host[3 + 2 * i] = (i + 1) * k.per < k.nt ? (i + 1) * k.per : k.nt;
+  }
+  return BFHIP_OK;
 }
 
 BFHIP_EXPORT int bfhip_conv2d_launch_choice(int dir, int N, int H, int W, int Cin, int Cout, int KH, int KW, int stride, int pad,
                                             int dil, int out_f32, int32_t *out_host) {
   BFHIP_REQUIRE(out_host && (dir == 0 || dir == 1), "conv2d_launch_choice: bad arguments");
   BFHIP_REQUIRE(bfhip_conv2d_supported(N, H, W, Cin, Cout, KH, KW, stride, pad, dil), "conv2d_launch_choice: unsupported geometry");
-  const ConvGeom g = dir ? dgrad_geom(N, H, W, Cin, Cin, Cout, Cout, KH, KW, stride, pad, dil)
-                         : conv_geom_fwd(N, H, W, Cin, Cin, Cout, KH, KW, stride, pad, dil, Cout);
+  const ConvGeom g = query_geom(dir, N, H, W, Cin, Cout, KH, KW, stride, pad, dil);
   BFHIP_REQUIRE((dir ? g.H > 0 && g.W > 0 : g.OH > 0 && g.OW > 0), "conv2d_launch_choice: empty output");
   const IgemmChoice c = choose_igemm(g, out_f32, device_cus());
   const int32_t v[8] = {c.pointwise ? 1 : 0, c.pointwise ? c.BN : c.shape, c.stages, g.transposed, c.BM, c.BN, c.tiles_m, c.tiles_n};
@@ -644,13 +922,19 @@
   return BFHIP_OK;
 }
 
+static ConvGeom query_geom(int dir, int N, int H, int W, int Cin, int Cout, int KH, int KW, int stride, int pad, int dil) {
+  return dir ? dgrad_geom(N, H, W, Cin, Cin, Cout, Cout, KH, KW, stride, pad, dil)
+             : conv_geom_fwd(N, H, W, Cin, Cin, Cout, KH, KW, stride, pad, dil, Cout);
+}
+
 BFHIP_EXPORT size_t bfhip_conv2d_dgrad_workspace_bytes(int Cin, int Cout, int KH, int KW) {
   return align_up((size_t)Cin * KH * KW * Cout * 2, 256);
 }
 
 static int conv2d_dgrad_impl(const void *dy, int ldg, const void *w, void *dx, int ldx, int N, int H, int W, int Cin, int Cout,
                              int KH, int KW, int stride, int pad, int dil, int out_f32, void *workspace, size_t workspace_bytes,
-                             hipStream_t s, const void *addend = nullptr, int addend_stride = 1) {
+                             hipStream_t s, const void *addend = nullptr, int addend_stride = 1, void *split_ws = nullptr,
+                             size_t split_ws_bytes = 0) {
   BFHIP_REQUIRE(bfhip_conv2d_supported(N, H, W, Cin, Cout, KH, KW, stride, pad, dil), "conv2d_dgrad: unsupported geometry");
   BFHIP_REQUIRE(dy && dx && workspace, "conv2d_dgrad: null pointer");
   BFHIP_REQUIRE(workspace_bytes >= bfhip_conv2d_dgrad_workspace_bytes(Cin, Cout, KH, KW), "conv2d_dgrad: workspace too small");
@@ -664,7 +948,7 @@
     hipLaunchKernelGGL(conv_weight_transpose_kernel, dim3(ceil_div(Cin, 32), ceil_div(Cout, 32), KH * KW), dim3(256), 0, s,
                        (const bf16_t *)w, (bf16_t *)workspace, Cout, KH * KW, Cin);
   const int rc = launch_igemm(dy, workspace, nullptr, dx, nullptr, g, out_f32, s, "conv2d_dgrad",
-                              Addend{(const bf16_t *)addend, addend ? addend_stride : 0, Cin, H, W});
+                              Addend{(const bf16_t *)addend, addend ? addend_stride : 0, Cin, H, W}, split_ws, split_ws_bytes);
   prof_end(&ps);
   return rc;
 }
@@ -682,6 +966,14 @@
                                        int out_f32, void *stream_) {
   return conv2d_dgrad_impl(dy, ldg, nullptr, dx, ldx, N, H, W, Cin, Cout, KH, KW, stride, pad, dil, out_f32, (void *)wt,
                            bfhip_conv2d_dgrad_workspace_bytes(Cin, Cout, KH, KW), (hipStream_t)stream_, addend, addend_stride);
+}
+
+BFHIP_EXPORT int bfhip_conv2d_dgrad_wt_ws(const void *dy, int ldg, const void *wt, const void *addend, int addend_stride, void *dx,
+                                          int ldx, int N, int H, int W, int Cin, int Cout, int KH, int KW, int stride, int pad,
+                                          int dil, int out_f32, void *workspace, size_t workspace_bytes, void *stream_) {
+  return conv2d_dgrad_impl(dy, ldg, nullptr, dx, ldx, N, H, W, Cin, Cout, KH, KW, stride, pad, dil, out_f32, (void *)wt,
+                           bfhip_conv2d_dgrad_workspace_bytes(Cin, Cout, KH, KW), (hipStream_t)stream_, addend, addend_stride,
+                           workspace, workspace_bytes);
 }
 
 BFHIP_EXPORT int bfhip_conv2d_dgrad_fuses_addend(int KH, int KW, int stride, int pad, int out_f32) {
diff --git a/bevfusion-3d_object_detection_amd/csrc/torch_binding.cpp b/bevfusion-3d_object_detection_amd/csrc/torch_binding.cpp
--- a/bevfusion-3d_object_detection_amd/csrc/torch_binding.cpp
+++ b/bevfusion-3d_object_detection_amd/csrc/torch_binding.cpp
@@ -186,6 +186,26 @@
 
 inline Tensor empty_nhwc(int64_t N, int64_t C, int64_t H, int64_t W, const at::TensorOptions &opt) {
   return at::empty({N, H, W, C}, opt).permute({0, 3, 1, 2});
+}
+
+struct SplitWs { void *ptr = nullptr; size_t bytes = 0; };
+std::mutex g_split_mu;
+std::map<std::pair<int, void *>, Tensor> &g_split_ws = *new std::map<std::pair<int, void *>, Tensor>();
+
+SplitWs split_workspace(int dir, const Tensor &x, void *stream, int64_t N, int64_t H, int64_t W, int64_t Cin, int64_t Cout, int64_t KH,
+                        int64_t KW, int64_t stride, int64_t pad, int64_t dil) {
+  const size_t need = bfhip_conv2d_split_workspace_bytes(dir, (int)N, (int)H, (int)W, (int)Cin, (int)Cout, (int)KH, (int)KW, (int)stride,
+                                                         (int)pad, (int)dil, 0);
+  if (need == 0) return SplitWs();
+  std::lock_guard<std::mutex> lock(g_split_mu);
+  Tensor &buf = g_split_ws[std::make_pair((int)x.get_device(), stream)];
+  if (!buf.defined() || (size_t)buf.numel() < need) {
+    hipStreamCaptureStatus st = hipStreamCaptureStatusNone;
+    if (hipStreamIsCapturing((hipStream_t)stream, &st) != hipSuccess || st != hipStreamCaptureStatusNone) return SplitWs();
+    buf = Tensor();
+    buf = at::empty({(int64_t)std::max<size_t>(need, (size_t)32 << 20)}, x.options().dtype(at::kByte));
+  }
+  return SplitWs{buf.data_ptr(), (size_t)buf.numel()};
 }
 
 struct PendingWgrad {
@@ -339,9 +359,11 @@
         addend.size(2) == (addend_stride == 2 ? (H + 1) / 2 : H) && addend.size(3) == (addend_stride == 2 ? (W + 1) / 2 : W) &&
         addend.is_contiguous(at::MemoryFormat::ChannelsLast) && ((uintptr_t)addend.data_ptr()) % 16 == 0)
       fuse = bfhip_conv2d_dgrad_fuses_addend((int)KH, (int)KW, (int)stride, (int)pad, 0) != 0;
-    check(bfhip_conv2d_dgrad_wt(dy.data_ptr(), (int)nhwc_pitch(dy), wt.data_ptr(), fuse ? addend.data_ptr() : nullptr, addend_stride,
-                                dx.data_ptr(), (int)Cin, (int)N, (int)H, (int)W, (int)Cin, (int)Cout, (int)KH, (int)KW, (int)stride,
-                                (int)pad, (int)dil, 0, cur_stream(x)),
+    void *stream = cur_stream(x);
+    const SplitWs sw = split_workspace(1, x, stream, N, H, W, Cin, Cout, KH, KW, stride, pad, dil);
+    check(bfhip_conv2d_dgrad_wt_ws(dy.data_ptr(), (int)nhwc_pitch(dy), wt.data_ptr(), fuse ? addend.data_ptr() : nullptr, addend_stride,
+                                   dx.data_ptr(), (int)Cin, (int)N, (int)H, (int)W, (int)Cin, (int)Cout, (int)KH, (int)KW, (int)stride,
+                                   (int)pad, (int)dil, 0, sw.ptr, sw.bytes, stream),
           "conv2d_dgrad_wt");
     return fuse ? dx : add_grad(dx, addend, addend_stride);
   }
@@ -391,9 +413,11 @@
     Tensor b32;
     const bool has_bias = bias.has_value() && bias->defined();
     if (has_bias) b32 = bias->scalar_type() == at::kFloat ? *bias : bias->to(at::kFloat);
-    check(bfhip_conv2d_fwd(x.data_ptr(), (int)nhwc_pitch(x), w.data_ptr(), has_bias ? b32.data_ptr<float>() : nullptr, y.data_ptr(),
-                           (int)Cout, (int)N, (int)H, (int)W, (int)Cin, (int)Cout, (int)KH, (int)KW, (int)stride, (int)pad, (int)dil, 0,
-                           emit_stats ? partial.data_ptr<float>() : nullptr, cur_stream(x)),
+    void *stream = cur_stream(x);
+    const SplitWs sw = split_workspace(0, x, stream, N, H, W, Cin, Cout, KH, KW, stride, pad, dil);
+    check(bfhip_conv2d_fwd_ws(x.data_ptr(), (int)nhwc_pitch(x), w.data_ptr(), has_bias ? b32.data_ptr<float>() : nullptr, y.data_ptr(),
+                              (int)Cout, (int)N, (int)H, (int)W, (int)Cin, (int)Cout, (int)KH, (int)KW, (int)stride, (int)pad, (int)dil, 0,
+                              emit_stats ? partial.data_ptr<float>() : nullptr, sw.ptr, sw.bytes, stream),
           "conv2d_fwd");
     ctx->save_for_backward({x, weight, (wt.has_value() && wt->defined()) ? *wt : Tensor()});
     ctx->saved_data["geom"] = std::vector<int64_t>{stride, pad, dil, fork, dgrad_lib ? 1 : 0, has_bias ? 1 : 0,
diff --git a/include/bevfusion_hip.h b/include/bevfusion_hip.h
--- a/include/bevfusion_hip.h
+++ b/include/bevfusion_hip.h
@@ -246,6 +246,16 @@
 int bfhip_conv2d_dgrad_wt(const void *dy, int ldg, const void *wt, const void *addend, int addend_stride, void *dx, int ldx, int N,
                           int H, int W, int Cin, int Cout, int KH, int KW, int stride, int pad, int dil, int out_f32, void *stream);
 int bfhip_conv2d_dgrad_fuses_addend(int KH, int KW, int stride, int pad, int out_f32);
+size_t bfhip_conv2d_split_workspace_bytes(int dir, int N, int H, int W, int Cin, int Cout, int KH, int KW, int stride, int pad,
+                                          int dil, int out_f32);
+int bfhip_conv2d_split_choice(int dir, int N, int H, int W, int Cin, int Cout, int KH, int KW, int stride, int pad, int dil,
+                              int out_f32, int32_t *out_host);
+int bfhip_conv2d_fwd_ws(const void *x, int ldx, const void *w, const float *bias, void *y, int ldy, int N, int H, int W, int Cin,
+                        int Cout, int KH, int KW, int stride, int pad, int dil, int out_f32, float *stat_partial, void *workspace,
+                        size_t workspace_bytes, void *stream);
+int bfhip_conv2d_dgrad_wt_ws(const void *dy, int ldg, const void *wt, const void *addend, int addend_stride, void *dx, int ldx,
+                             int N, int H, int W, int Cin, int Cout, int KH, int KW, int stride, int pad, int dil, int out_f32,
+                             void *workspace, size_t workspace_bytes, void *stream);
 int bfhip_conv2d_wt_segment_bytes(void);
 int bfhip_conv2d_weight_transpose_batched(const void *segs_dev, int nseg, long long total_blocks, void *stream);
 int bfhip_split_bf16x3(const float *src, long long P, int C, void *chan, int order_chan, void *batch, int order_batch, void *stream);
```

Result: no change. 157.1 frames/s (median of 6 runs) (+0.3%).
